# davidepi/glaze

Hardware: AMD Instinct MI355X
Metric: Msamples/s + achieved HBM GB/s, Sponza 1080p, 1/2/4/8xMI355X (higher is better)
Workload: dtype f32; 1 GPU; Sponza-class synthetic atrium (262267 tris, 26 materials, 27 textures) as a .glaze V1 file (2853389 bytes) through parse, 1920x1080, path tracer depth 8, 143 steps = 17.9 spp; materials=26, textures=27, scene=Sponza-class synthetic atrium, width=1920, height=1080, depth=8, triangles=262267

## Files before the change

### glaze_amd/abi.py

```python
import ctypes as C
import os

NAME_MAX = 256

OK, E_IO, E_INVALID_INPUT, E_INVALID_DATA, E_ARG, E_DEVICE, E_UNSUPPORTED = 0, -1, -2, -3, -4, -5, -6

CAMERA_PERSPECTIVE, CAMERA_ORTHOGRAPHIC = 0, 1
MAT_FLAT, MAT_LAMBERT, MAT_MIRROR, MAT_GLASS, MAT_METAL, MAT_FROSTED, MAT_UBER = range(7)
LIGHT_OMNI, LIGHT_SUN, LIGHT_AREA, LIGHT_SKY = range(4)
TEX_GRAY, TEX_RGBA_SRGB, TEX_RGBA_NORM = 1, 2, 3
DIRECT, PATH_TRACE = 0, 1


class Vertex(C.Structure):
    _fields_ = [("vv", C.c_float * 3), ("vn", C.c_float * 3), ("vt", C.c_float * 2)]


class Mesh(C.Structure):
    _fields_ = [("id", C.c_uint16), ("material", C.c_uint16), ("index_offset", C.c_uint32), ("index_count", C.c_uint32)]


class Transform(C.Structure):
    _fields_ = [("m", C.c_float * 16)]

# ... 227 lines not shown
    "glz_renderer_restart": (C.c_int, [_P]),
    "glz_renderer_step": (C.c_int, [_P, C.c_uint32]),
    "glz_renderer_read_rgba8": (C.c_int, [_P, _P]),
    "glz_renderer_set_seed": (C.c_int, [_P, C.c_uint64]),
    "glz_renderer_set_depth": (C.c_int, [_P, C.c_uint32]),
    "glz_renderer_read_hdr": (C.c_int, [_P, _P]),
    "glz_renderer_read_result": (C.c_int, [_P, _P]),
    "glz_renderer_launch_constants": (C.c_int, [_P, C.c_uint32, _P, _P]),
    "glz_renderer_push_constants": (C.c_int, [_P, _P]),
    "glz_renderer_set_partition": (C.c_int, [_P, C.c_uint32, C.c_uint32]),
    "glz_renderer_set_chains": (C.c_int, [_P, C.c_uint32]),
    "glz_renderer_export_device": (C.c_int, [_P, C.c_int, _P]),
    "glz_renderer_packed_pixels": (C.c_uint64, [_P, C.c_uint32, C.c_uint32]),
    "glz_renderer_export_packed": (C.c_int, [_P, C.c_int, _P]),
    "glz_renderer_scatter_packed": (C.c_int, [_P, C.c_uint32, C.c_uint32, _P, _P]),
    "glz_renderer_scatter_packed_all": (C.c_int, [_P, C.c_uint32, _P, C.c_uint64, _P]),
    "glz_renderer_tonemap_device": (C.c_int, [_P, _P, _P]),
    "glz_renderer_enable_counters": (C.c_int, [_P, C.c_int]),
    "glz_renderer_get_stats": (C.c_int, [_P, _P]),
    "glz_debug_trace_closest": (C.c_int, [_P, _P, _P, C.c_uint64, C.c_float, _P, _P, _P, _P, _P]),
    "glz_debug_trace_any": (C.c_int, [_P, _P, _P, _P, C.c_uint64, C.c_float, _P]),
    "glz_debug_read_derivatives": (C.c_int64, [_P, _P, C.c_int64]),
    "glz_debug_read_rt_materials": (C.c_int64, [_P, _P, C.c_int64]),
    "glz_debug_read_rt_lights": (C.c_int64, [_P, _P, C.c_int64]),
    "glz_debug_read_sky": (C.c_int64, [_P, _P, C.c_int64]),
    "glz_debug_read_bvh": (C.c_int64, [_P, _P, C.c_int64, _P, C.c_int64]),
    "glz_debug_read_bvh8": (C.c_int64, [_P, _P, C.c_int64]),
    "glz_host_launch_constants": (C.c_int, [C.c_uint64, C.c_uint32, _P, _P]),
    "glz_host_push_constants": (C.c_int, [_P, C.c_uint32, C.c_uint32, _P]),
    "glz_host_chain_owner": (C.c_int, [C.c_uint32, C.c_uint32, C.c_uint32, C.c_uint32, C.c_uint32, _P]),
    "glz_host_build_sah": (C.c_int, [C.c_uint32, _P, _P, _P, _P]),
    "glz_host_srgb8_thresholds": (C.c_int, [_P]),
    "glz_debug_tonemap": (C.c_int, [_P, _P, C.c_uint64, _P]),
    "glz_debug_sample_texture": (C.c_int, [_P, C.c_uint32, _P, _P, C.c_uint64, _P]),
    "glz_debug_detmath": (C.c_int, [_P, C.c_int, _P, _P, _P, C.c_uint64]),
    "glz_debug_color_to_spec": (C.c_int, [_P, C.c_int, _P, C.c_uint64, _P]),
    "glz_debug_scene_set_spectra": (C.c_int, [_P, C.c_uint32, _P, _P]),
    "glz_debug_bsdf_value": (C.c_int,[_P, C.c_uint32, _P, _P, _P, _P, _P, C.c_uint64, _P, _P]),
    "glz_debug_bsdf_sample": (C.c_int, [_P, C.c_uint32, _P, _P, _P, _P, C.c_uint64, _P, _P, _P]),
    "glz_debug_light_sample": (C.c_int, [_P, C.c_uint32, _P, _P, C.c_uint64, C.c_float, _P, _P, _P, _P]),
    "glz_debug_read_texture_level": (C.c_int64, [_P, C.c_uint32, C.c_uint32, _P, C.c_int64, _P, _P]),
    "glz_host_mip_level": (C.c_int64, [_P, C.c_uint32, _P, C.c_int64, _P, _P]),
    "glz_renderer_set_texture_lod": (C.c_int, [_P, C.c_int]),
    "glz_debug_rccl_selftest": (C.c_int, [_P, C.c_uint64, _P]),
    "glz_instance_set_as_levels": (C.c_int, [_P, C.c_int]),
    "glz_renderer_set_devices": (C.c_int, [_P, _P, C.c_int]),
    "glz_renderer_set_launch_mode": (C.c_int, [_P, C.c_int]),
    "glz_renderer_set_node_width": (C.c_int, [_P, C.c_int]),
    "glz_renderer_node_width": (C.c_int, [_P]),
    "glz_renderer_launch_mode": (C.c_int, [_P]),
    "glz_renderer_device_count": (C.c_int, [_P]),
    "glz_renderer_device_scene_info": (C.c_int, [_P, C.c_int, _P]),
    "glz_rccl_version": (C.c_int, []),
    "glz_host_tile_owner": (C.c_int, [C.c_uint32, C.c_uint32, C.c_uint32, _P]),
    "glz_renderer_read_aov": (C.c_int, [_P, C.c_int, _P]),
    "glz_renderer_set_denoise": (C.c_int, [_P, _P]),
    "glz_renderer_read_denoised": (C.c_int, [_P, _P, _P]),
    "glz_renderer_set_despeckle": (C.c_int, [_P, C.c_int, _P]),
    "glz_renderer_despeckle": (C.c_int, [_P, _P]),
    "glz_renderer_read_despeckled": (C.c_int, [_P, _P, _P]),
    "glz_renderer_read_motion": (C.c_int, [_P, _P, _P, C.c_uint32, _P]),
    "glz_renderer_reproject": (C.c_int, [_P, _P, _P, C.c_uint32, _P, _P, _P, _P, _P]),
    "glz_renderer_read_motion_from": (C.c_int, [_P, _P, _P]),
    "glz_renderer_reproject_from": (C.c_int, [_P, _P, _P, _P, _P, _P, _P]),
    "glz_debug_motion_timing_from": (C.c_int, [_P, _P, _P]),
    "glz_debug_skin_timing": (C.c_int, [_P, _P, C.c_uint32, _P]),
    "glz_host_project_constants": (C.c_int, [_P, C.c_uint32, C.c_uint32, _P]),
    "glz_host_project_points": (C.c_int, [_P, C.c_uint32, C.c_uint32, _P, C.c_uint64, _P]),
    "glz_host_reproject": (C.c_int, [C.c_uint32, C.c_uint32, _P, _P, _P, _P, _P, _P]),
    "glz_debug_project_points": (C.c_int, [_P, _P, C.c_uint32, C.c_uint32, _P, C.c_uint64, _P]),
    "glz_debug_motion_timing": (C.c_int, [_P, _P, _P, C.c_uint32, _P]),
    "glz_debug_reproject": (C.c_int, [_P, C.c_uint32, C.c_uint32, _P, _P, _P, _P, _P, _P, _P]),
    "glz_host_despeckle": (C.c_int, [C.c_uint32, C.c_uint32, _P, _P, _P, _P, _P, C.c_int, _P]),
    "glz_debug_despeckle": (C.c_int, [_P, C.c_uint32, C.c_uint32, _P, _P, _P, _P, _P, C.c_int, _P, _P]),
    "glz_host_denoise": (C.c_int, [C.c_uint32, C.c_uint32, _P, _P, _P, _P, _P]),
    "glz_debug_denoise": (C.c_int, [_P, C.c_uint32, C.c_uint32, _P, _P, _P, _P, _P]),
    "glz_debug_camera_rays": (C.c_int, [_P, C.c_float, C.c_float, _P, _P]),
    "glz_debug_post_timing": (C.c_int, [_P, _P]),
    "glz_renderer_set_guide_mode": (C.c_int, [_P, C.c_int, C.c_uint32]),
    "glz_renderer_guide_mode": (C.c_int, [_P, _P]),
    "glz_debug_guide_chain": (C.c_int, [_P, C.c_uint32, _P, _P, _P]),
    "glz_host_traversal_offsets_fit": (C.c_int, [C.c_uint64] * 6),
    "glz_host_sky_row_pairs": (C.c_int, [_P, _P, C.c_uint64, _P]),
    "glz_host_conductor_finite": (C.c_int, [_P, _P, _P]),
    "glz_host_metal_spectra": (C.c_int, [C.c_uint32, _P, _P]),
}

_LIB = None


def library_path():
    return os.environ.get("GLAZE_HIP_LIB") or os.path.join(os.path.dirname(os.path.abspath(__file__)), "csrc", "libglaze_hip.so")


class GlazeLibraryMissing(ImportError):
    pass


def lib():
    global _LIB
    if _LIB is None:
        path = library_path()
        if not os.path.exists(path):
            raise GlazeLibraryMissing(
                "%s not found: build it with `make -C glaze_amd/csrc` (there is no CPU fallback for the render path)" % path)
        handle = C.CDLL(path)
        for name, (res, args) in PROTOTYPES.items():
            fn = getattr(handle, name)
            fn.restype = res
            fn.argtypes = args
        _LIB = handle
    return _LIB


class GlazeError(IOError):
    def __init__(self, status, message):
        super().__init__("%s (status %d)" % (message, status))
        self.status = status


def last_error():
    l = lib()
    msg = l.glz_last_error()
    return GlazeError(l.glz_last_status(), msg.decode("utf8", "replace") if msg else "unknown error")


def check(status):
    if status < 0:
        raise last_error()
    return status
```

### glaze_amd/csrc/abi_debug.cpp

```cpp
#include <algorithm>
#include <cstring>
#include <string>
#include <vector>

#include "abi_internal.h"
#include "denoise.h"
#include "reproject.h"
#include "skin.h"
#include "morph.h"
#include "normals.h"
#include "mipchain.h"
#include "rccl_dl.h"
#include "tile_map.h"

using namespace glz;
using namespace glz::abi;

namespace {
struct DebugCall {
  hipStream_t st;
  template <class T>
  const T* in(const T* host, size_t n) {
    return host ? static_cast<const T*>(buffer(host, n * sizeof(T), nullptr)) : nullptr;
  }
// ... 603 lines not shown
  const int dev = inst->i->device;
  ncclResult_t r = nc->CommInitAll(&comm, 1, &dev);
  if (r != ncclSuccess) return fail(GLZ_E_DEVICE, (std::string("ncclCommInitAll: ") + nc->GetErrorString(r)).c_str());
  r = nc->Reduce(send.ptr, recv.ptr, n, ncclFloat, ncclSum, 0, comm, st);
  bool ok = r == ncclSuccess;
  std::string msg = ok ? "" : std::string("ncclReduce: ") + nc->GetErrorString(r);
  if (ok) {
    ok = hip_ok(hipMemcpyAsync(back.data(), recv.ptr, n * 4, hipMemcpyDeviceToHost, st), "read back", e) && hip_ok(hipStreamSynchronize(st), "ncclReduce", e);
    if (!ok) msg = e.msg;
  }
  (void)nc->CommDestroy(comm);
  if (!ok) return fail(GLZ_E_DEVICE, msg.c_str());
  if (memcmp(host.data(), back.data(), n * 4) != 0) return fail(GLZ_E_DEVICE, "ncclReduce on a one-rank communicator changed the data");
  return GLZ_OK;
  GLZ_GUARD_END(GLZ_E_IO)
}

int glz_host_launch_constants(uint64_t seed, uint32_t launch, uint32_t* seed_out, float offset[2]) {
  GLZ_GUARD_BEGIN
  if (!seed_out || !offset) return fail(GLZ_E_ARG, "output is null");
  if (!host::launch_constants(seed, launch, seed_out, offset)) return fail(GLZ_E_IO, "WorkScheduler::peek disagrees with next()");
  return GLZ_OK;
  GLZ_GUARD_END(GLZ_E_IO)
}
int glz_host_push_constants(const glz_camera* camera, uint32_t width, uint32_t height, float out32[32]) {
  if (!camera || !out32 || width == 0 || height == 0 || camera->type > GLZ_CAMERA_ORTHOGRAPHIC) return fail(GLZ_E_ARG, "bad argument");
  host::push_constants(*camera, width, height, out32, out32 + 16);
  return GLZ_OK;
}
int glz_host_tile_owner(uint32_t width, uint32_t height, uint32_t world, uint16_t* owner_out) {
  if (!owner_out || world == 0 || world > 65535) return fail(GLZ_E_ARG, "bad argument");
  const TileMap m = make_tile_map(width, height, 0, world);
  for (uint32_t y = 0; y < height; ++y)
    for (uint32_t x = 0; x < width; ++x) owner_out[(size_t)y * width + x] = (uint16_t)tile_owner(tile_of_pixel(m, x, y), world);
  return GLZ_OK;
}
int glz_host_chain_owner(uint32_t width, uint32_t height, uint32_t rank, uint32_t world, uint32_t chains, uint16_t* owner_out) {
  if (world == 0 || rank >= world || chains > 16 || !width || !height) return fail(GLZ_E_ARG, "bad argument");
  const uint32_t S = Renderer::chains_for(width, height, rank, world, chains);
  const TileMap m = make_tile_map(width, height, rank, world);
  if (owner_out)
    for (uint32_t y = 0; y < height; ++y)
      for (uint32_t x = 0; x < width; ++x) {
        const uint32_t t = tile_of_pixel(m, x, y);
        owner_out[(size_t)y * width + x] = tile_owner(t, world) == rank ? (uint16_t)tile_chain(t, world, S) : (uint16_t)0xFFFF;
      }
  return (int)S;
}

int64_t glz_host_mip_level(const glz_texture* t, uint32_t level, uint8_t* out, int64_t cap, uint32_t* width, uint32_t* height) {
  GLZ_GUARD_BEGIN
  if (!t || !t->pixels || !t->width || !t->height || t->format < 1 || t->format > 3) return fail(GLZ_E_ARG, "bad texture");
  std::vector<host::MipLevel> given(1);
  given[0].width = t->width;
  given[0].height = t->height;
  given[0].pixels.assign(t->pixels, t->pixels + (size_t)t->width * t->height * (t->format == GLZ_TEX_GRAY ? 1 : 4));
  const std::vector<host::MipLevel> chain = host::build_mip_chain(t->format, std::move(given));
  if (level >= chain.size()) {
    if (width) *width = 0;
    if (height) *height = 0;
    return 0;
  }
  const host::MipLevel& m = chain[level];
  if (width) *width = m.width;
  if (height) *height = m.height;
  if (out && cap > 0) memcpy(out, m.pixels.data(), (size_t)std::min<int64_t>(cap, (int64_t)m.pixels.size()));
  return (int64_t)m.pixels.size();
  GLZ_GUARD_END(GLZ_E_IO)
}
int glz_host_traversal_offsets_fit(uint64_t n_nodes, uint64_t n_nodes8, uint64_t n_leaves, uint64_t n_instances, uint64_t grid_lanes, uint64_t overflow_depth) {
  const char* what = traversal_offsets_exceeded(TraversalSizes{n_nodes, n_nodes8, n_leaves, n_instances, grid_lanes, overflow_depth});
  return what ? fail(GLZ_E_INVALID_DATA, what) : GLZ_OK;
}
int glz_host_srgb8_thresholds(float thresholds_out[256]) {
  if (!thresholds_out) return fail(GLZ_E_ARG, "output is null");
  host::srgb8_thresholds(thresholds_out);
  return GLZ_OK;
}
int glz_host_sky_row_pairs(const float* marginal_values, const float* conditional_integrals, uint64_t n, float* pairs_out) {
  if (n != 0 && (!marginal_values || !conditional_integrals || !pairs_out)) return fail(GLZ_E_ARG, "glz_host_sky_row_pairs: null array");
  sky_row_pairs(marginal_values, conditional_integrals, (size_t)n, pairs_out);
  return GLZ_OK;
}
int glz_host_conductor_finite(const float ior[16], const float ior2abs2[16], int* flag_out) {
  if (!ior || !ior2abs2 || !flag_out) return fail(GLZ_E_ARG, "glz_host_conductor_finite: null argument");
  *flag_out = conductor_finite(ior, ior2abs2) ? 1 : 0;
  return GLZ_OK;
}
int glz_host_metal_spectra(uint32_t metal, float ior_out[16], float ior2abs2_out[16]) {
  if (!ior_out || !ior2abs2_out || !metal_spectra(metal, ior_out, ior2abs2_out)) return fail(GLZ_E_ARG, "glz_host_metal_spectra: no such metal, or a null output");
  return GLZ_OK;
}

}

int glz_host_build_sah(uint32_t n, const float* box_lo, const float* box_hi, int32_t* children_out, int32_t* parent_out) {
  GLZ_GUARD_BEGIN
  if (n < 2 || !box_lo || !box_hi || !children_out || !parent_out) return fail(GLZ_E_ARG, "glz_host_build_sah: bad argument");
  static_assert(sizeof(float4) == 16 && sizeof(int2) == 8, "layout");
  build_sah_host(n, reinterpret_cast<const float4*>(box_lo), reinterpret_cast<const float4*>(box_hi), reinterpret_cast<int2*>(children_out), parent_out);
  return GLZ_OK;
  GLZ_GUARD_END(GLZ_E_IO)
}
```

### glaze_amd/csrc/device/hit_vertex.h

```cpp
#pragma once
#include "device/shading.h"

namespace glz {
using namespace dev;

struct ShadeRecord { float4 va0, va1, vb0, vb1, vc0, vc1, dn, du; };
struct HitVertex {
  ShadeRecord rec;
  uint32_t xf_bits;
  vec3 point;
  vec2 uv;
  vec3 ng, ns, dpdu;
  MatScalars mat;
};

__device__ __forceinline__ ShadeRecord load_shade_record(const DeviceScene& S, uint32_t leaf) {
  const float4* rec = S.shade_tris + 8u * (size_t)leaf;
  return ShadeRecord{rec[0], rec[1], rec[2], rec[3], rec[4], rec[5], rec[6], rec[7]};
}
__device__ __forceinline__ vec3 hit_point(float4 a, float4 b, float4 c, float4 hr) {
  const float b0 = 1.0f - hr.y - hr.z, b1 = hr.y, b2 = hr.z;
  return (mk3(a.x, a.y, a.z) * b0 + mk3(b.x, b.y, b.z) * b1) + mk3(c.x, c.y, c.z) * b2;
}
__device__ __forceinline__ vec3 hit_point(const ShadeRecord& r, float4 hr) { return hit_point(r.va0, r.vb0, r.vc0, hr); }
struct HitIds { uint32_t material_id, xf; };
template <bool FLAG, class InstOf>
__device__ __forceinline__ HitIds hit_ids(const DeviceScene& S, const ShadeRecord& r, InstOf inst_of) {
  HitIds ids{__float_as_uint(r.dn.w), __float_as_uint(r.du.w)};
  if (!FLAG) ids.xf &= 0x7FFFFFFFu;
  if (S.two_level) {
    const RTInstance in = S.instances[inst_of()];
    ids.material_id = in.material_id;
    ids.xf = in.transform_id;
    if (FLAG) ids.xf = in.transform_id | (S.xf_identity[in.transform_id] ? 0x80000000u : 0u);
  }
  return ids;
}
template <class InstOf>
__device__ __forceinline__ HitVertex load_hit_vertex(const DeviceScene& S, float4 hr, InstOf inst_of) {
  HitVertex v;
  v.rec = load_shade_record(S, __float_as_uint(hr.w));
  const ShadeRecord& r = v.rec;
  const HitIds ids = hit_ids<true>(S, r, inst_of);
  const float b0 = 1.0f - hr.y - hr.z, b1 = hr.y, b2 = hr.z;
  v.point = hit_point(r, hr);
  v.uv = vec2{(r.va1.z * b0 + r.vb1.z * b1) + r.vc1.z * b2, (r.va1.w * b0 + r.vb1.w * b1) + r.vc1.w * b2};
  v.ng = mk3(r.dn.x, r.dn.y, r.dn.z), v.dpdu = mk3(r.du.x, r.du.y, r.du.z);
  v.ns = (mk3(r.va0.w, r.va1.x, r.va1.y) * b0 + mk3(r.vb0.w, r.vb1.x, r.vb1.y) * b1) + mk3(r.vc0.w, r.vc1.x, r.vc1.y) * b2;
  v.mat = load_material(S, ids.material_id);
  v.xf_bits = ids.xf;
  return v;
}
template <bool POINTS>
__device__ __forceinline__ void finish_hit_vertex(const DeviceScene& S, HitVertex& v, const TexFootprint& fp) {
  if (v.mat.normal != 0) {
    const vec4 tx = texture2d_lod(S, v.mat.normal, v.uv.x, v.uv.y, fp);
    Frame old;
    old.s = normalize3(v.dpdu);
    old.n = v.ns;
    old.t = normalize3(cross3(old.n, old.s));
    v.ns = normalize3(to_world(mk3(tx.x * 2.0f - 1.0f, tx.y * 2.0f - 1.0f, tx.z * 2.0f - 1.0f), old));
    v.ns = v.ns * gl_sign(dot3(v.ng, v.ns));
  }
  if (!(v.xf_bits >> 31)) {
    const float4* xq = reinterpret_cast<const float4*>(&S.transforms[v.xf_bits & 0x7FFFFFFFu]);
    const float4 m0 = xq[0], m1 = xq[1], m2 = xq[2], m3 = xq[3], w0 = xq[4], w1 = xq[5], w2 = xq[6];
    const float w2o[12] = {w0.x, w0.y, w0.z, w0.w, w1.x, w1.y, w1.z, w1.w, w2.x, w2.y, w2.z, w2.w};
    if (POINTS) {
      const float o2w[16] = {m0.x, m0.y, m0.z, m0.w, m1.x, m1.y, m1.z, m1.w, m2.x, m2.y, m2.z, m2.w, m3.x, m3.y, m3.z, m3.w};
      v.point = xform_point(o2w, v.point);
      v.dpdu = xform_point(o2w, v.dpdu);
    }
    v.ng = xform_tdir(w2o, v.ng);
    v.ns = xform_tdir(w2o, v.ns);
  }
}
__device__ __forceinline__ SurfacePoint hit_surface_point(const DeviceScene& S, const HitVertex& v, vec3 direction, const TexFootprint& fp) {
  SurfacePoint P;
  P.woW = -direction;
  P.uv = v.uv;
  P.frame = make_frame(v.dpdu, v.ns);
  P.mat = v.mat;
  fetch_material_textures(S, P, fp);
  return P;
}
}
```

### glaze_amd/csrc/device/intersect.h

```cpp
#pragma once
#include <hip/hip_runtime.h>

#include "device/math.h"
#include "device/shading.h"
#include "device/types.h"

namespace glz {
using namespace dev;

typedef float f32x2 __attribute__((ext_vector_type(2)));
struct SlabSel { uint32_t x, y, z; };
constexpr uint32_t kKeyDistanceMask = 0xFFFFFC00u, kKeyChild = 0x100u, kKeyChildMask = 0x300u;
constexpr uint32_t kSlabSelLo = 0x0305040Cu, kSlabSelHi = 0x0307060Cu, kSlabSelFlip = kSlabSelLo ^ kSlabSelHi, kSlabMagic = 0x47000000u;
__device__ __forceinline__ uint32_t slab_sel(float ig) { return ig < 0.0f ? kSlabSelHi : kSlabSelLo; }
constexpr int kKeysNearFirst = 0, kKeysFarFirst = 1, kKeysPerLane = 2;
template <int ORDER>
constexpr uint32_t kKeyMiss = ORDER == kKeysFarFirst ? 0u : 0xFFFFFFFFu;
template <bool CHECK_LINK = true, int ORDER = kKeysNearFirst>
__device__ __forceinline__ uint32_t box_key(uint32_t wx, uint32_t wy, uint32_t wz, uint32_t link, uint32_t k, SlabSel sel, vec3 ig, vec3 cgn, vec3 cgf,
                                            float tmin, float tmax, uint32_t flip = 0u) {
  const float nx = __uint_as_float(__builtin_amdgcn_perm(wx, kSlabMagic, sel.x)), fx = __uint_as_float(__builtin_amdgcn_perm(wx, kSlabMagic, sel.x ^ kSlabSelFlip));
  const float ny = __uint_as_float(__builtin_amdgcn_perm(wy, kSlabMagic, sel.y)), fy = __uint_as_float(__builtin_amdgcn_perm(wy, kSlabMagic, sel.y ^ kSlabSelFlip));
  const float nz = __uint_as_float(__builtin_amdgcn_perm(wz, kSlabMagic, sel.z)), fz = __uint_as_float(__builtin_amdgcn_perm(wz, kSlabMagic, sel.z ^ kSlabSelFlip));
  const f32x2 tx = __builtin_elementwise_fma(f32x2{nx, fx}, f32x2{ig.x, ig.x}, f32x2{cgn.x, cgf.x});
// ... 23 lines not shown
  const float i = 1.0f / d;
  return fabsf(i) <= 1e30f ? i : copysignf(1e30f, i);
}
__device__ __forceinline__ float grid_inv_dir_fast(float d) {
  const float i = __builtin_amdgcn_rcpf(d);
  return fabsf(i) <= 1e30f ? i : copysignf(1e30f, i);
}
__device__ __forceinline__ bool ray_is_finite(vec3 o, vec3 d) {
  const float s = ((o.x + o.y) + o.z) + ((d.x + d.y) + d.z);
  return s - s == 0.0f;
}

struct RayShear {
  bool z_is_x, z_is_y;
  float sx, sy, sz;
};
__device__ __forceinline__ RayShear ray_shear(vec3 d) {
  const float ax = fabsf(d.x), ay = fabsf(d.y), az = fabsf(d.z);
  RayShear r;
  r.z_is_x = (ax >= ay) & (ax >= az);
  r.z_is_y = !r.z_is_x & (ay >= az);
  const float dz = r.z_is_x ? d.x : (r.z_is_y ? d.y : d.z), dx = r.z_is_x ? d.y : (r.z_is_y ? d.z : d.x), dy = r.z_is_x ? d.z : (r.z_is_y ? d.x : d.y);
  r.sz = 1.0f / dz;
  r.sx = dx * r.sz;
  r.sy = dy * r.sz;
  return r;
}
constexpr float kDetNoise = 1.9073486e-6f;

struct QuadHit {
  float t[2], u[2], v[2];
  bool ok[2];
};
__device__ __forceinline__ vec3 shear_point(const RayShear& r, float px, float py, float pz, vec3 o) {
  const vec3 a = mk3(px, py, pz) - o;
  const float az = r.z_is_x ? a.x : (r.z_is_y ? a.y : a.z), ax = r.z_is_x ? a.y : (r.z_is_y ? a.z : a.x), ay = r.z_is_x ? a.z : (r.z_is_y ? a.x : a.y);
  return mk3(fmaf(-r.sx, az, ax), fmaf(-r.sy, az, ay), r.sz * az);
}
__device__ __forceinline__ bool triangle_finish(float U, float V, float W, float Az, float Bz, float Cz, float products, float tmin, float& t, float& u, float& v) {
  const float lo = fminf(fminf(U, V), W), hi = fmaxf(fmaxf(U, V), W);
  const float det = (U + V) + W;
  const float inv = 1.0f / det;
  u = V * inv;
  v = W * inv;
  t = fmaf(W, Cz, fmaf(V, Bz, U * Az)) * inv;
  return !((lo < 0.0f) & (hi > 0.0f)) & (fabsf(det) > products * kDetNoise) & (t > tmin);
}
__device__ __forceinline__ QuadHit ray_quad(const RayShear& rs, float4 r0, float4 r1, float4 r2, float4 r3, bool pair, vec3 o, float tmin) {
  QuadHit h;
  const vec3 S0 = shear_point(rs, r0.x, r0.y, r0.z, o), S2 = shear_point(rs, r2.x, r2.y, r2.z, o);
  const float pv = S0.x * S2.y, qv = S0.y * S2.x;
  {
    const vec3 S1 = shear_point(rs, r1.x, r1.y, r1.z, o);
    const float pu = S2.x * S1.y, qu = S2.y * S1.x, pw = S1.x * S0.y, qw = S1.y * S0.x;
    float U = pu - qu, V = pv - qv, W = pw - qw;
    if (__builtin_expect(__any((U == 0.0f) | (V == 0.0f) | (W == 0.0f)), 0)) {
      if (U == 0.0f) U = fmaf(S2.x, S1.y, -pu) - fmaf(S2.y, S1.x, -qu);
      if (V == 0.0f) V = fmaf(S0.x, S2.y, -pv) - fmaf(S0.y, S2.x, -qv);
      if (W == 0.0f) W = fmaf(S1.x, S0.y, -pw) - fmaf(S1.y, S0.x, -qw);
    }
    h.ok[0] = triangle_finish(U, V, W, S0.z, S1.z, S2.z, (fabsf(pu) + fabsf(pv)) + fabsf(pw), tmin, h.t[0], h.u[0], h.v[0]);
  }
  __builtin_amdgcn_sched_barrier(0);
  {
    const vec3 S3 = shear_point(rs, r3.x, r3.y, r3.z, o);
    const float pu = S3.x * S2.y, qu = S3.y * S2.x, pv2 = S0.x * S3.y, qv2 = S0.y * S3.x;
    float U = pu - qu, V = pv2 - qv2, W = qv - pv;
    if (__builtin_expect(__any(pair & ((U == 0.0f) | (V == 0.0f) | (W == 0.0f))), 0)) {
      if (U == 0.0f) U = fmaf(S3.x, S2.y, -pu) - fmaf(S3.y, S2.x, -qu);
      if (V == 0.0f) V = fmaf(S0.x, S3.y, -pv2) - fmaf(S0.y, S3.x, -qv2);
      if (W == 0.0f) W = fmaf(S2.x, S0.y, -qv) - fmaf(S2.y, S0.x, -pv);
    }
    h.ok[1] = triangle_finish(U, V, W, S0.z, S2.z, S3.z, (fabsf(pu) + fabsf(pv2)) + fabsf(qv), tmin, h.t[1], h.u[1], h.v[1]) & pair;
  }
  return h;
}

__device__ __forceinline__ bool alpha_test(const DeviceScene& S, uint32_t leaf, float u, float v) {
  const float w = 1.0f - u - v;
  const float4* rec = S.alpha_recs + 3u * (size_t)leaf;
  const float4 r0 = rec[0], r1 = rec[1], r2 = rec[2];
  const float tu = (r0.x * w + r0.z * u) + r1.x * v, tv = (r0.y * w + r0.w * u) + r1.y * v;
  const TexDesc t{__float_as_uint(r1.z), __float_as_uint(r1.w), __float_as_uint(r2.x), __float_as_uint(r2.y)};
  return !(bilinear_level(S, t, S.tex_pool, tu, tv).x < 0.5f);
}

__device__ __forceinline__ bool alpha_test_instance(const DeviceScene& S, uint32_t slot, uint32_t instance, float u, float v) {
  const float4* rec = S.shade_tris + 8u * (size_t)slot;
  const float4 a = rec[1], b = rec[3], c = rec[5];
  const uint32_t material_id = S.instances[instance].material_id;
  const float w = 1.0f - u - v;
  const float tu = (a.z * w + b.z * u) + c.z * v, tv = (a.w * w + b.w * u) + c.w * v;
  return !(texture_r(S, S.materials[material_id].opacity, vec2{tu, tv}) < 0.5f);
}

struct HitRecord {
  float t, u, v;
  uint32_t leaf;
  uint32_t inst;
  uint32_t world_id;
};
}
```

### glaze_amd/csrc/device/shade_pixel.h

```cpp
#pragma once
#include <hip/hip_runtime.h>

#include "device/hit_vertex.h"
#include "device/math.h"
#include "device/path_state.h"
#include "device/shading.h"
#include "device/types.h"
#include "kernels.h"

namespace glz {
using namespace dev;

struct SharedQueue {
  const LaunchArgs& A;
  __device__ __forceinline__ uint32_t slot(bool push) { return queue_slot(A.st.queue_count + A.shade_set * kQueueSetWords, A.map.n_local_pixels, push); }
};
#ifdef GLZ_SECTION_TIMES
#define GLZ_SHADE_STAMP(k) out.stamp(k)
#else
#define GLZ_SHADE_STAMP(k) do { } while (0)
#endif
__device__ __forceinline__ uint32_t pixel_rng(const FrameData& F, PixelId px) {
  return pcg(__float_as_uint((float)F.seed) ^ pcg(__float_as_uint((float)px.x) ^ pcg(__float_as_uint((float)px.y))));
}
__device__ __forceinline__ uint32_t light_pick(const FrameData& F, uint32_t& rng) {
  return (uint32_t)gl_min(rand01(rng) * (float)F.lights_no, (float)(F.lights_no - 1u));
}
struct DirectState {
  const LaunchArgs& A;
  static constexpr bool kDeferSkyTexel = false;
  __device__ __forceinline__ void stamp(int) {}
  __device__ __forceinline__ void ray_o(uint32_t lid, float4 v) { A.st.ray_o[lid] = v; }
  __device__ __forceinline__ void ray_d(uint32_t lid, float4 v) { A.st.ray_d[lid] = v; }
  __device__ __forceinline__ void imp(int q, uint32_t lid, float4 v) { A.st.imp[q][lid] = v; }
  __device__ __forceinline__ float4 read_imp(int q, uint32_t lid) const { return A.st.imp[q][lid]; }
  __device__ __forceinline__ float4 reset_origin(uint32_t, float4 ro) const { return ro; }
  __device__ __forceinline__ uint32_t seed_rng(const FrameData& F, PixelId px) const { return pixel_rng(F, px); }
  __device__ __forceinline__ uint32_t pick_light(const FrameData& F, uint32_t& rng) const { return light_pick(F, rng); }
  __device__ __forceinline__ void accumulate(uint32_t lid, vec3 c, bool add, bool update, float mark) { accumulate_shaded(A, lid, c, add && isfinite(c.x + c.y + c.z), update, mark); }
};
struct StagedState {
#ifdef GLZ_SECTION_TIMES
  unsigned long long sec[8] = {0, 0, 0, 0, 0, 0, 0, 0}, sec_last = 0;
  __device__ __forceinline__ void stamp(int k) {
    const unsigned long long now = __builtin_amdgcn_s_memtime();
    sec[k] += now - sec_last;
    sec_last = now;
  }
#else
  __device__ __forceinline__ void stamp(int) {}
#endif
  static constexpr bool kDeferSkyTexel = true;
  float4 ro, rd, im[4];
  uint32_t mask = 0;
  __device__ __forceinline__ void ray_o(uint32_t, float4 v) { ro = v; mask |= 1u; }
  __device__ __forceinline__ void ray_d(uint32_t, float4 v) { rd = v; mask |= 2u; }
  __device__ __forceinline__ void imp(int q, uint32_t, float4 v) { im[q] = v; mask |= 4u; }
  const LaunchArgs* A = nullptr;
  LdsNodePtr lds_imp = nullptr;
  static constexpr uint32_t kShadeBlockPixels = 256;
  __device__ __forceinline__ float4 read_imp(int q, uint32_t) const {
    const u32x4 v = lds_imp[q * kShadeBlockPixels];
    return make_float4(__uint_as_float(v.x), __uint_as_float(v.y), __uint_as_float(v.z), __uint_as_float(v.w));
  }
  __device__ __forceinline__ float4 reset_origin(uint32_t lid, float4) const { return A->st.ray_o[lid]; }
  typedef uint32_t u32x2 __attribute__((ext_vector_type(2)));
  typedef const __attribute__((address_space(3))) u32x2* LdsPickPtr;
  LdsPickPtr lds_pick = nullptr;
  __device__ __forceinline__ uint32_t seed_rng(const FrameData&, PixelId) const { return (*lds_pick).x; }
  __device__ __forceinline__ uint32_t pick_light(const FrameData&, uint32_t&) const { return (*lds_pick).y; }
  __device__ __forceinline__ void accumulate(uint32_t lid, vec3 cc, bool add, bool update, float mark) { accumulate_shaded(*A, lid, cc, add && isfinite(cc.x + cc.y + cc.z), update, mark); }
};
template <bool LOD, class Queue, class State>
__device__ __forceinline__ int shade_pixel_body(const LaunchArgs& A, const DeviceScene& S, const FrameData& F, uint32_t lid, PixelId px, float4 ro, float4 rd, float4 hr, Queue& queue,
                                                State& out, float& end_w) {
  const bool fresh = F.direct_only || ro.w == 0.0f;
  float bounce = F.direct_only ? 0.0f : ro.w;
  const vec3 direction = mk3(rd.x, rd.y, rd.z);
  auto load_importance = [&]() {
    asm volatile("" ::: "memory");
    Spec imp;
    if (fresh) {
      imp = spec_set(1.0f);
    } else {
#pragma unroll
      for (int q = 0; q < 4; ++q) {
        const float4 v = out.read_imp(q, lid);
        imp.w[4 * q] = v.x; imp.w[4 * q + 1] = v.y; imp.w[4 * q + 2] = v.z; imp.w[4 * q + 3] = v.w;
      }
    }
    return imp;
  };
  const uint32_t leaf = __float_as_uint(hr.w);
  if (leaf == 0xFFFFFFFFu) {
    uint32_t flags = 0;
    vec3 c = mk3(0.0f, 0.0f, 0.0f);
    if ((bounce == 0.0f || rd.w == 1.0f) && S.sky.tex_id > 0) {
      const vec3 w = normalize3(xform_dir(S.sky.world2obj, direction));
      const float phi = glz_atan2f(w.y, w.x), theta = glz_acosf(w.z);
      const vec3 texel = texture_rgb(S, S.sky.tex_id, vec2{phi * kInv2Pi, theta * kInvPi});
      c = spec_to_rgb(spec_mul(load_importance(), from_illuminant_color(texel)));
      flags = kFlagUpdate;
    }
    if (flags != 0) out.accumulate(lid, c, true, true, F.update_mark);
    end_w = rd.w;
    return F.direct_only ? 0 : 1;
  }
  HitVertex hv = load_hit_vertex(S, hr, [&]() { return A.st.hit_inst[lid]; });
  const MatScalars mat = hv.mat;
  GLZ_SHADE_STAMP(0);
  TexFootprint fp{kNoLod, 0.0f, 0.0f, 1u};
  float cone_w = 0.0f;
  if constexpr (LOD) {
    const auto& [va0, va1, vb0, vb1, vc0, vc1, dn, du_rec] = hv.rec;
    float cone_in = F.cone_width0;
    asm volatile("" : "+v"(cone_in));
    if (!fresh) cone_in = A.st.cone[lid];
    cone_w = cone_in + F.cone_spread * hr.x;
    vec3 e1 = mk3(vb0.x, vb0.y, vb0.z) - mk3(va0.x, va0.y, va0.z), e2 = mk3(vc0.x, vc0.y, vc0.z) - mk3(va0.x, va0.y, va0.z);
    vec3 n = mk3(dn.x, dn.y, dn.z);
    if (!(hv.xf_bits >> 31)) {
      const TransformPair* xf = &S.transforms[hv.xf_bits & 0x7FFFFFFFu];
      e1 = xform_dir(xf->o2w, e1);
      e2 = xform_dir(xf->o2w, e2);
      n = xform_tdir(xf->w2o, n);
    }
    const vec3 cr = cross3(e1, e2);
    const float area2 = sqrtf(dot3(cr, cr));
    const float uva2 = fabsf((vb1.z - va1.z) * (vc1.w - va1.w) - (vc1.z - va1.z) * (vb1.w - va1.w));
    const float nn = dot3(n, n), nd = dot3(n, direction);
    const float cosv = fabsf(nd) / sqrtf(nn);
    const float x = ((uva2 / area2) * (cone_w * cone_w)) / (cosv * cosv);
    if (x >= 1.17549435e-38f && x <= 3.4e38f) {
      fp.lod_base = 0.5f * glz_log2f(x);
      if (F.lod_mode == 2u) {
        float ratio = 1.0f / cosv;
        ratio = ratio < 16.0f ? ratio : 16.0f;
        const float taps = -glz_floorf(-ratio);
        const vec3 m = direction - n * (nd / nn);
        const float mm = dot3(m, m);
        if (taps > 1.0f && mm > 0.0f) {
          const float g11 = dot3(e1, e1), g12 = dot3(e1, e2), g22 = dot3(e2, e2), r1 = dot3(m, e1), r2 = dot3(m, e2);
          const float det = g11 * g22 - g12 * g12;
          const float ca = (r1 * g22 - r2 * g12) / det, cb = (r2 * g11 - r1 * g12) / det;
          const float len = (cone_w / cosv) / sqrtf(mm);
          const float du = (ca * (vb1.z - va1.z) + cb * (vc1.z - va1.z)) * len;
          const float dv = (ca * (vb1.w - va1.w) + cb * (vc1.w - va1.w)) * len;
          if (fabsf(du) <= 3.4e38f && fabsf(dv) <= 3.4e38f) {
            fp.du = du;
            fp.dv = dv;
            fp.taps = (uint32_t)taps;
            fp.lod_base = fp.lod_base - glz_log2f(taps);
          }
        }
      }
    }
  }
  finish_hit_vertex<true>(S, hv, fp);
  const vec3 point = hv.point, ns = hv.ns;
  uint32_t rng = out.seed_rng(F, px);
  const SurfacePoint P = hit_surface_point(S, hv, direction, fp);
  GLZ_SHADE_STAMP(1);
  float spec_flag;
  float imp_lum = 0.0f;
  bool have_lum = false;
  if (mat.is_specular == 0) {
    const uint32_t li = out.pick_light(F, rng);
    vec3 xi;
    xi.x = rand01(rng); xi.y = rand01(rng); xi.z = rand01(rng);
    LightSample ls;
    ls.pdf = 0.0f;
    sample_light<State::kDeferSkyTexel>(S, li, point, xi, F.scene_radius, ls);
    GLZ_SHADE_STAMP(2);
    vec3 c = mk3(0.0f, 0.0f, 0.0f);
    uint32_t flags = kFlagUpdate;
    vec3 sh_dir = mk3(0.0f, 0.0f, 0.0f);
    float sh_tmax = 0.0f;
    if (ls.pdf > 0.0f) {
      const float xi_b = rand01(rng);
      Spec value = spec_set(0.0f);
      const float bpdf = bsdf_eval(S, P, ls.wiW, xi_b, value);
      if (bpdf > 0.0f) {
        const float w_vis = 1.0f * (fabsf(dot3(ls.wiW, ns)) / ls.pdf);
        const float nl = (float)F.lights_no;
        const Spec emission = light_emission<State::kDeferSkyTexel>(S, ls);
        const Spec importance = load_importance();
        imp_lum = spec_luminance(importance);
        have_lum = true;
        Spec rad;
        GLZ_BINS {
          const float rl = value.w[i] * emission.w[i];
          rad.w[i] = ((rl * w_vis) * nl) * importance.w[i];
        }
        c = spec_to_rgb(rad);
        if (!isfinite(c.x + c.y + c.z)) c = mk3(0.0f, 0.0f, 0.0f);
        flags |= kFlagShadow;
        sh_dir = ls.wiW;
        sh_tmax = ls.distance - 1e-3f;
      }
    }
    if (!(flags & kFlagShadow)) {
      const Spec importance = load_importance();
      imp_lum = spec_luminance(importance);
      have_lum = true;
    }
    const bool push = (flags & kFlagShadow) != 0;
    GLZ_SHADE_STAMP(3);
    const uint32_t slot = queue.slot(push);
    if (push) {
      A.st.sh_o[slot] = make_float4(point.x, point.y, point.z, sh_tmax);
      A.st.sh_d[slot] = make_float4(sh_dir.x, sh_dir.y, sh_dir.z, __uint_as_float(lid));
      A.st.contrib[slot] = make_float4(c.x, c.y, c.z, __uint_as_float(flags));
    } else {
      out.accumulate(lid, c, false, true, F.update_mark);
    }
    spec_flag = 0.0f;
  } else {
    spec_flag = 1.0f;
  }
  if (F.direct_only) return 0;
  GLZ_SHADE_STAMP(4);
  float rr_scale = 1.0f;
  if (bounce > (float)(F.pt_steps / 2u)) {
    const float kill = gl_max(0.05f, 1.0f - (have_lum ? imp_lum : spec_luminance(load_importance())));
    if (rand01(rng) < kill) {
      end_w = spec_flag;
      return 2;
    }
    rr_scale = 1.0f / (1.0f - kill);
  }
  vec3 xi;
  xi.x = rand01(rng); xi.y = rand01(rng); xi.z = rand01(rng);
  Spec value = spec_set(0.0f);
  vec3 wiW = mk3(0.0f, 0.0f, 0.0f);
  const float pdf = bsdf_sample(S, P, xi, value, wiW);
  if (pdf == 0.0f) {
    end_w = spec_flag;
    return 2;
  }
  float weight = fabsf(dot3(wiW, ns));
  weight /= pdf;
  const Spec importance = spec_scale(load_importance(), rr_scale);
#pragma unroll
  for (int q = 0; q < 4; ++q)
    out.imp(q, lid, make_float4(importance.w[4 * q] * (value.w[4 * q] * weight), importance.w[4 * q + 1] * (value.w[4 * q + 1] * weight),
                                importance.w[4 * q + 2] * (value.w[4 * q + 2] * weight), importance.w[4 * q + 3] * (value.w[4 * q + 3] * weight)));
  bounce = bounce < (float)F.pt_steps ? bounce + 1.0f : 0.0f;
  GLZ_SHADE_STAMP(5);
  if constexpr (LOD) A.st.cone[lid] = cone_w;
  if (F.pregen && bounce == 0.0f) {
    end_w = spec_flag;
    return 2;
  }
  out.ray_o(lid, make_float4(point.x, point.y, point.z, bounce));
  out.ray_d(lid, make_float4(wiW.x, wiW.y, wiW.z, spec_flag));
  return 0;
}
template <bool LOD, class Queue, class State>
__device__ __forceinline__ void shade_pixel(const LaunchArgs& A, const DeviceScene& S, const FrameData& F, uint32_t lid, PixelId px, float4 ro, float4 rd, float4 hr, Queue& queue,
                                            State& out) {
  float end_w = 0.0f;
  const int ended = shade_pixel_body<LOD>(A, S, F, lid, px, ro, rd, hr, queue, out, end_w);
  if (ended != 0) {
    if (F.pregen) {
      vec3 co, cd;
      camera_ray(A, F, px, F.next_pixel_offset[0], F.next_pixel_offset[1], co, cd);
      out.ray_o(lid, make_float4(co.x, co.y, co.z, __uint_as_float(kPregenBounceBits)));
      out.ray_d(lid, make_float4(cd.x, cd.y, cd.z, end_w));
    } else {
      const float4 o = out.reset_origin(lid, ro);
      out.ray_o(lid, make_float4(o.x, o.y, o.z, 0.0f));
      if (ended == 2) out.ray_d(lid, make_float4(rd.x, rd.y, rd.z, end_w));
    }
  }
}

constexpr uint32_t kShadeLdsTableBytes = 8192;
constexpr uint32_t kPathTableBytes = 16384;
static_assert(sizeof(MatCompact) % 16 == 0 && sizeof(MetalSpectra) % 16 == 0 && sizeof(RTLight) % 16 == 0 && sizeof(TexDesc) % 16 == 0, "the tables are copied in 16-byte pieces");
struct SceneTables {
  uint32_t qm, qs, ql, qt;
  __host__ __device__ explicit SceneTables(const DeviceScene& s)
      : qm(s.n_materials * (uint32_t)(sizeof(MatCompact) / 16)), qs(s.n_metal_spectra * (uint32_t)(sizeof(MetalSpectra) / 16)), ql(s.n_rt_lights * (uint32_t)(sizeof(RTLight) / 16)), qt(s.n_textures * (uint32_t)(sizeof(TexDesc) / 16)) {}
  __host__ __device__ uint32_t bytes() const { return (qm + qs + ql + qt) * 16u; }
  __device__ __forceinline__ void stage(const DeviceScene& s, uint4* dst, uint32_t block) const {
    const uint4* gm = reinterpret_cast<const uint4*>(s.mat_compact);
    const uint4* gs = reinterpret_cast<const uint4*>(s.metal_spectra);
    const uint4* gl = reinterpret_cast<const uint4*>(s.lights);
    const uint4* gt = reinterpret_cast<const uint4*>(s.tex_desc);
    const uint32_t es = qm + qs, el = es + ql;
    for (uint32_t i = threadIdx.x; i < el + qt; i += block) dst[i] = i < qm ? gm[i] : (i < es ? gs[i - qm] : (i < el ? gl[i - es] : gt[i - el]));
  }
  __device__ __forceinline__ void use(DeviceScene& S, const uint4* copy) const {
    S.mat_compact = reinterpret_cast<const MatCompact*>(copy);
    S.metal_spectra = reinterpret_cast<const MetalSpectra*>(copy + qm);
    S.lights = reinterpret_cast<const RTLight*>(copy + qm + qs);
    S.tex_desc = reinterpret_cast<const TexDesc*>(copy + qm + qs + ql);
  }
};

typedef const __attribute__((address_space(4))) char* KernargPtr;
__device__ __forceinline__ KernargPtr reread_kernarg() {
  KernargPtr p = (KernargPtr)__builtin_amdgcn_kernarg_segment_ptr();
  asm volatile("" : "+s"(p));
  return p;
}
}
```

### glaze_amd/csrc/device/shading.h

```cpp
#pragma once
#include "glaze_abi.h"
#include "glz_tables.h"
#include "math.h"
#include "types.h"

namespace glz {
namespace dev {

struct Spec {
  float w[16];
};
#define GLZ_BINS _Pragma("unroll") for (int i = 0; i < 16; ++i)

GLZ_D Spec spec_set(float f) { Spec s; GLZ_BINS s.w[i] = f; return s; }
GLZ_D Spec spec_scale(const Spec& a, float f) { Spec r; GLZ_BINS r.w[i] = a.w[i] * f; return r; }
GLZ_D Spec spec_mul(const Spec& a, const Spec& b) { Spec r; GLZ_BINS r.w[i] = a.w[i] * b.w[i]; return r; }
GLZ_D Spec spec_div(const Spec& a, float f) { Spec r; GLZ_BINS r.w[i] = a.w[i] / f; return r; }
GLZ_D Spec spec_load(const Spectrum16& g) { Spec r; GLZ_BINS r.w[i] = g.w[i]; return r; }

__device__ static const float kCieX[16] = GLZ_DEV_CIE_X;
__device__ static const float kCieY[16] = GLZ_DEV_CIE_Y;
__device__ static const float kCieZ[16] = GLZ_DEV_CIE_Z;
__device__ static const float kSurf[7][16] = {GLZ_DEV_SURF_WHITE, GLZ_DEV_SURF_CYAN, GLZ_DEV_SURF_MAGENTA, GLZ_DEV_SURF_YELLOW,
                                              GLZ_DEV_SURF_RED, GLZ_DEV_SURF_GREEN, GLZ_DEV_SURF_BLUE};
__device__ static const float kIllum[7][16] = {GLZ_DEV_ILLUM_WHITE, GLZ_DEV_ILLUM_CYAN, GLZ_DEV_ILLUM_MAGENTA, GLZ_DEV_ILLUM_YELLOW,
                                               GLZ_DEV_ILLUM_RED, GLZ_DEV_ILLUM_GREEN, GLZ_DEV_ILLUM_BLUE};
enum { kWhite = 0, kCyan, kMagenta, kYellow, kRed, kGreen, kBlue };

GLZ_D float spec_weighted(const Spec& s, const float* __restrict__ c) {
  float lane[4];
#pragma unroll
  for (int j = 0; j < 4; ++j) lane[j] = ((s.w[j] * c[j] + s.w[4 + j] * c[4 + j]) + s.w[8 + j] * c[8 + j]) + s.w[12 + j] * c[12 + j];
  return ((lane[0] + lane[1]) + lane[2]) + lane[3];
}
GLZ_D float spec_luminance(const Spec& s) { return spec_weighted(s, kCieY) * 0.17557178f; }
GLZ_D vec3 spec_to_rgb(const Spec& s) {
  float X = spec_weighted(s, kCieX) * 0.17557178f;
  float Y = spec_weighted(s, kCieY) * 0.17557178f;
  float Z = spec_weighted(s, kCieZ) * 0.17557178f;
  vec3 r;
  r.x = (3.240479f * X - 1.537150f * Y) - 0.498535f * Z;
  r.y = (-0.969256f * X + 1.875991f * Y) + 0.041556f * Z;
  r.z = (0.055648f * X - 0.204043f * Y) + 1.057311f * Z;
  return r;
}

GLZ_D Spec rgb_to_spec(vec3 c, const float (*__restrict__ basis)[16], float scale) {
  int a, b;
  float k0, k1, k2;
  if (c.x <= c.y && c.x <= c.z) {
    k0 = c.x;
    a = kCyan;
    if (c.y <= c.z) { k1 = c.y - c.x; b = kBlue; k2 = c.z - c.y; } else { k1 = c.z - c.x; b = kGreen; k2 = c.y - c.z; }
  } else if (c.y <= c.x && c.y <= c.z) {
    k0 = c.y;
    a = kMagenta;
    if (c.x <= c.z) { k1 = c.x - c.y; b = kBlue; k2 = c.z - c.x; } else { k1 = c.z - c.y; b = kRed; k2 = c.x - c.z; }
  } else {
    k0 = c.z;
    a = kYellow;
    if (c.x <= c.y) { k1 = c.x - c.z; b = kGreen; k2 = c.y - c.x; } else { k1 = c.y - c.z; b = kRed; k2 = c.x - c.y; }
  }
  Spec r;
  GLZ_BINS r.w[i] = ((basis[kWhite][i] * k0 + basis[a][i] * k1) + basis[b][i] * k2) * scale;
  return r;
}
GLZ_D Spec from_surface_color(vec3 c) { return rgb_to_spec(c, kSurf, 0.94f); }
GLZ_D Spec from_illuminant_color(vec3 c) { return rgb_to_spec(c, kIllum, 0.86445f); }

struct vec4 {
  float x, y, z, w;
};
constexpr uint32_t kTexInline = 0x80u;
GLZ_D vec4 decode_texel(const DeviceScene& S, uint32_t format, uint32_t bits) {
  if (format == GLZ_TEX_GRAY) return vec4{(float)(bits & 0xFFu) / 255.0f, 0.0f, 0.0f, 1.0f};
  const uint32_t r = bits & 0xFFu, g = (bits >> 8) & 0xFFu, b = (bits >> 16) & 0xFFu, a = bits >> 24;
  if (format == GLZ_TEX_RGBA_SRGB) return vec4{S.srgb_lut[r], S.srgb_lut[g], S.srgb_lut[b], (float)a / 255.0f};
  return vec4{(float)r / 255.0f, (float)g / 255.0f, (float)b / 255.0f, (float)a / 255.0f};
}
GLZ_D uint32_t texel_address(const TexDesc& t, uint32_t format, uint32_t ux, uint32_t uy) {
  const uint32_t tiles_x = t.format >> 8;
  if (format == GLZ_TEX_GRAY) return t.offset + ((uy >> 3) * tiles_x + (ux >> 4)) * 128u + (uy & 7u) * 16u + (ux & 15u);
  return t.offset + (((uy >> 2) * tiles_x + (ux >> 3)) * 32u + (uy & 3u) * 8u + (ux & 7u)) * 4u;
}
GLZ_D uint32_t load_texel(const uint8_t* __restrict__ pool, const TexDesc& t, uint32_t format, uint32_t ux, uint32_t uy) {
  const uint32_t addr = texel_address(t, format, ux, uy);
  return format == GLZ_TEX_GRAY ? (uint32_t)pool[addr] : *reinterpret_cast<const uint32_t*>(pool + addr);
}
GLZ_D int wrap_coord(int i, int n) {
  int r = i % n;
  return r < 0 ? r + n : r;
}
GLZ_D int wrap_coord_far(float i, int n) {
  const uint32_t bits = __float_as_uint(i), m = (bits & 0x7FFFFFu) | 0x800000u;
  const int e = (int)((bits >> 23) & 0xFFu) - 150;
  if (e > 104) return 0;
  uint32_t r = 0;
#pragma unroll 1
  for (int k = 23; k >= -e; --k) {
    r = 2u * r + (k >= 0 ? (m >> k) & 1u : 0u);
    r = r >= (uint32_t)n ? r - (uint32_t)n : r;
  }
  return (int)((bits >> 31) && r != 0u ? (uint32_t)n - r : r);
}
GLZ_D float lerp_ab(float a, float b, float t) { return a + (b - a) * t; }
GLZ_D vec4 bilinear_level(const DeviceScene& S, const TexDesc& t, const uint8_t* __restrict__ pool, float u, float v) {
  const uint32_t format = t.format & 0x7Fu;
  float fu = u * (float)t.width - 0.5f, fv = v * (float)t.height - 0.5f;
  float iu = glz_floorf(fu), iv = glz_floorf(fv);
  float ax = fu - iu, ay = fv - iv;
  uint32_t ta, tb, tc, tdx;
  if (t.format & kTexInline) {
    ta = tb = tc = tdx = t.offset;
  } else {
    if (S.tex_counter) {
      S.tex_counter[0] += 1ull;
      S.tex_counter[1] += format == GLZ_TEX_GRAY ? 4ull : 16ull;
    }
    const int x0 = fabsf(iu) < 8388608.0f ? wrap_coord((int)iu, (int)t.width) : wrap_coord_far(iu, (int)t.width);
    const int y0 = fabsf(iv) < 8388608.0f ? wrap_coord((int)iv, (int)t.height) : wrap_coord_far(iv, (int)t.height);
    const int x1 = x0 + 1 == (int)t.width ? 0 : x0 + 1, y1 = y0 + 1 == (int)t.height ? 0 : y0 + 1;
    if (format != GLZ_TEX_GRAY && x1 == x0 + 1 && (x0 & 7) != 7) {
      const uint2 r0 = *reinterpret_cast<const uint2*>(pool + texel_address(t, format, (uint32_t)x0, (uint32_t)y0));
      const uint2 r1 = *reinterpret_cast<const uint2*>(pool + texel_address(t, format, (uint32_t)x0, (uint32_t)y1));
      ta = r0.x; tb = r0.y; tc = r1.x; tdx = r1.y;
    } else {
      ta = load_texel(pool, t, format, (uint32_t)x0, (uint32_t)y0);
      tb = load_texel(pool, t, format, (uint32_t)x1, (uint32_t)y0);
      tc = load_texel(pool, t, format, (uint32_t)x0, (uint32_t)y1);
      tdx = load_texel(pool, t, format, (uint32_t)x1, (uint32_t)y1);
    }
  }
  const vec4 a = decode_texel(S, format, ta), b = decode_texel(S, format, tb), c = decode_texel(S, format, tc), d = decode_texel(S, format, tdx);
  vec4 r;
  r.x = lerp_ab(lerp_ab(a.x, b.x, ax), lerp_ab(c.x, d.x, ax), ay);
  r.y = lerp_ab(lerp_ab(a.y, b.y, ax), lerp_ab(c.y, d.y, ax), ay);
  r.z = lerp_ab(lerp_ab(a.z, b.z, ax), lerp_ab(c.z, d.z, ax), ay);
  r.w = lerp_ab(lerp_ab(a.w, b.w, ax), lerp_ab(c.w, d.w, ax), ay);
  return r;
}
GLZ_D vec4 texture2d(const DeviceScene& S, uint32_t id, float u, float v) {
  const uint4 td = reinterpret_cast<const uint4*>(S.tex_desc)[id];
  return bilinear_level(S, TexDesc{td.x, td.y, td.z, td.w}, S.tex_pool, u, v);
}
constexpr float kNoLod = -1e30f;
struct TexFootprint { float lod_base; float du, dv; uint32_t taps; };
GLZ_D vec4 texture2d_lod(const DeviceScene& S, uint32_t id, float u, float v, const TexFootprint& fp) {
  const uint4 td = reinterpret_cast<const uint4*>(S.tex_desc)[id];
  const TexDesc t0{td.x, td.y, td.z, td.w};
  uint32_t first = 0, l0 = 0, levels_used = 1, probes = 1;
  float frac = 0.0f;
  if (fp.lod_base > -1e29f && S.tex_mip_base != nullptr && !(t0.format & kTexInline)) {
    const uint32_t b = S.tex_mip_base[id];
    const uint32_t levels = b >> 24;
    first = b & 0xFFFFFFu;
    float lam = fp.lod_base + 0.5f * glz_log2f((float)t0.width * (float)t0.height);
    lam = lam > 0.0f ? lam : 0.0f;
    const float top = (float)(levels - 1u);
    lam = lam < top ? lam : top;
    const float fl = glz_floorf(lam);
    l0 = (uint32_t)fl;
    frac = lam - fl;
    levels_used = frac > 0.0f ? 2u : 1u;
    probes = fp.taps;
  }
  vec4 sum{0.0f, 0.0f, 0.0f, 0.0f}, cur{0.0f, 0.0f, 0.0f, 0.0f};
  const uint32_t fetches = probes * levels_used;
#pragma unroll 1
  for (uint32_t k = 0; k < fetches; ++k) {
    const uint32_t probe = levels_used == 2u ? k >> 1 : k, upper = levels_used == 2u ? k & 1u : 0u;
    const uint32_t level = l0 + upper;
    TexDesc t = t0;
    const uint8_t* pool = S.tex_pool;
    if (level != 0u) {
      const uint4 md = reinterpret_cast<const uint4*>(S.tex_mip_desc)[first + level - 1u];
      t = TexDesc{md.x, md.y, md.z, md.w};
      pool = S.tex_mip_pool;
    }
    float uu = u, vv = v;
    if (probes > 1u) {
      const float s = ((float)probe + 0.5f) / (float)probes - 0.5f;
      uu = u + s * fp.du;
      vv = v + s * fp.dv;
    }
    const vec4 r = bilinear_level(S, t, pool, uu, vv);
    if (upper == 0u) {
      cur = r;
    } else {
      cur.x = lerp_ab(cur.x, r.x, frac); cur.y = lerp_ab(cur.y, r.y, frac); cur.z = lerp_ab(cur.z, r.z, frac); cur.w = lerp_ab(cur.w, r.w, frac);
    }
    if (upper + 1u == levels_used) {
      if (probe == 0u) {
        sum = cur;
      } else {
        sum.x += cur.x; sum.y += cur.y; sum.z += cur.z; sum.w += cur.w;
      }
    }
  }
  if (probes > 1u) {
    const float n = (float)probes;
    sum.x = sum.x / n; sum.y = sum.y / n; sum.z = sum.z / n; sum.w = sum.w / n;
  }
  return sum;
}
GLZ_D vec3 texture_rgb(const DeviceScene& S, uint32_t id, vec2 uv) {
  vec4 t = texture2d(S, id, uv.x, uv.y);
  return mk3(t.x, t.y, t.z);
}
GLZ_D float texture_r(const DeviceScene& S, uint32_t id, vec2 uv) { return texture2d(S, id, uv.x, uv.y).x; }

struct Frame {
  vec3 s, t, n;
};
GLZ_D Frame make_frame(vec3 dpdu, vec3 n) {
  Frame f;
  f.s = normalize3(dpdu - n * dot3(n, dpdu));
  f.t = cross3(n, f.s);
  f.n = n;
  return f;
}
GLZ_D vec3 to_world(vec3 v, const Frame& f) {
  return normalize3(mk3((f.s.x * v.x + f.t.x * v.y) + f.n.x * v.z, (f.s.y * v.x + f.t.y * v.y) + f.n.y * v.z,
                        (f.s.z * v.x + f.t.z * v.y) + f.n.z * v.z));
}
GLZ_D vec3 to_local(vec3 w, const Frame& f) {
  return normalize3(mk3(dot3(w, f.s), dot3(w, f.t), dot3(w, f.n)));
}

GLZ_D Spec fresnel_conductor(float c, const Spectrum16& ior, const Spectrum16& ior2abs2) {
  const float c2 = c * c, twoc = c * 2.0f;
  Spec r;
  GLZ_BINS {
    float e = ior.w[i] * twoc;
    float ep = e + c2, epp = e + 1.0f;
    float a = ior2abs2.w[i];
    float perp = (a - ep) / (a + ep);
    float tmp = a * c2;
    float par = (tmp - epp) / (tmp + epp);
    r.w[i] = (perp + par) / 2.0f;
  }
  return r;
}
GLZ_D float fresnel_dielectric(float costi, float etai, float etat) {
  float sin2ti = gl_max(0.0f, 1.0f - costi * costi);
  float sin2tt = etai * etai / (etat * etat) * sin2ti;
  if (sin2tt >= 1.0f) return 1.0f;
  float costt = sqrtf(gl_max(0.0f, 1.0f - sin2tt));
  float tt = etat * costt, ti = etat * costi, ii = etai * costi, it = etai * costt;
  float rparl = (ti - it) / (ti + it);
  float rperp = (ii - tt) / (ii + tt);
  return (rparl * rparl + rperp * rperp) / 2.0f;
}

GLZ_D vec2 ggx_sample_p22(float cost, vec2 r) {
  if (cost > 0.999f) {
    float rr = sqrtf(r.x / (1.0f - r.x));
    float phi = kTwoPi * r.y;
    return vec2{rr * glz_cosf(phi), rr * glz_sinf(phi)};
  }
  float cos2t = cost * cost;
  float sin2t = gl_max(0.0f, 1.0f - cos2t);
  float tan2t = check_inf(sin2t / cos2t);
  float tant = sqrtf(tan2t);
  float a2 = 1.0f / tan2t;
  float G1 = 2.0f / (1.0f + sqrtf(1.0f + 1.0f / a2));
  float A = 2.0f * r.x / G1 - 1.0f;
  float B = tant;
  float invA2m1 = A * A - 1.0f == 0.0f ? 1e10f : 1.0f / (A * A - 1.0f);
  float sq = sqrtf(gl_max(0.0f, B * B * invA2m1 * invA2m1 - (A * A - B * B) * invA2m1));
  float sx1 = B * invA2m1 - sq;
  float sx2 = B * invA2m1 + sq;
  float sx = (A < 0.0f || sx2 > 1.0f / tant) ? sx1 : sx2;
  float stepval = gl_step(0.5f, r.y);
  float s = gl_mix(1.0f, -1.0f, stepval);
  float u = gl_mix(2.0f * (r.y - 0.5f), 2.0f * (0.5f - r.y), stepval);
  float z = (u * (u * (u * -0.3657289f + 0.7902350f) - 0.4249658f) + 0.0001529f) /
            (u * (u * (u * (u * 0.1695078f - 0.3972035f) - 0.2325005f) + 1.0f) - 0.5398259f);
  float sy = s * z * sqrtf(1.0f + sx * sx);
  return vec2{sx, sy};
}
GLZ_D float ggx_d(vec3 wh, vec2 a) {
  float cos2t = wh.z * wh.z;
  float cos4t = cos2t * cos2t;
  float sin2t = gl_max(0.0f, 1.0f - cos2t);
  float tan2t = sin2t / cos2t;
  float cos2p = wh.x * wh.x / sin2t;
  float sin2p = wh.y * wh.y / sin2t;
  float e1 = sin2t == 0.0f ? 1.0f : 1.0f + ((cos2p / (a.x * a.x) + sin2p / (a.y * a.y)) * tan2t);
  float d = 1.0f / (kPi * a.x * a.y * cos4t * e1 * e1);
  return isinf(tan2t) ? 0.0f : d;
}
GLZ_D float ggx_lambda(vec3 v, vec2 a) {
// ... 12 lines not shown
}
GLZ_D vec3 ggx_sample_wh(vec3 wo, vec2 r, vec2 a) {
  float flip = gl_sign(wo.z);
  vec3 wi = flip * wo;
  vec3 ws = normalize3(mk3(wi.x * a.x, wi.y * a.y, wi.z));
  float cost = ws.z;
  vec2 slope = ggx_sample_p22(cost, r);
  float sin2t = gl_max(0.0f, 1.0f - cost * cost);
  float cosp = sin2t == 0.0f ? 1.0f : sqrtf(ws.x * ws.x / sin2t);
  float sinp = sin2t == 0.0f ? 0.0f : sqrtf(ws.y * ws.y / sin2t);
  float sx = cosp * slope.x - sinp * slope.y;
  float sy = sinp * slope.x + cosp * slope.y;
  return flip * normalize3(mk3(-a.x * sx, -a.y * sy, 1.0f));
}
GLZ_D vec2 anisotropic_alpha(float a, float anis) { return vec2{a * (1.0f + anis), a * (1.0f - anis)}; }

struct MatScalars {
  float diffuse_mul[3];
  uint32_t diffuse, roughness, metalness, opacity, normal, bsdf_index;
  float roughness_mul, metalness_mul, anisotropy, ior_dielectric;
  uint32_t is_specular;
  uint32_t spectra;
};
GLZ_D MatScalars load_material(const DeviceScene& S, uint32_t id) {
  const float4* q = reinterpret_cast<const float4*>(&S.mat_compact[id]);
  const float4 a = q[0], b = q[2], c = q[3], d = q[4];
  MatScalars r;
  r.diffuse_mul[0] = a.x; r.diffuse_mul[1] = a.y; r.diffuse_mul[2] = a.z;
  r.diffuse = __float_as_uint(b.x); r.roughness = __float_as_uint(b.y); r.metalness = __float_as_uint(b.z); r.opacity = __float_as_uint(b.w);
  r.normal = __float_as_uint(c.x); r.bsdf_index = __float_as_uint(c.y); r.roughness_mul = c.z; r.metalness_mul = c.w;
  r.anisotropy = d.x; r.ior_dielectric = d.y; r.is_specular = __float_as_uint(d.z);
  r.spectra = __float_as_uint(a.w);
  return r;
}
GLZ_D const MetalSpectra& material_spectra(const DeviceScene& S, const MatScalars& m) { return S.metal_spectra[m.spectra & ~kSpectraConductorFinite]; }

struct SurfacePoint {
  vec3 woW;
  vec2 uv;
  Frame frame;
  MatScalars mat;
  vec3 tint;
  float rough_tex;
  float metal_tex;
};

GLZ_D void dielectric_etas(const MatScalars& m, float woz, float& etai, float& etat) {
  float outside = gl_step(0.0f, woz);
  etai = gl_mix(m.ior_dielectric, kDefaultIor, outside);
  etat = gl_mix(kDefaultIor, m.ior_dielectric, outside);
}

struct Lobe {
  float d, g, pdf, costi, cwo, cwi;
};
GLZ_D Lobe reflect_lobe(vec3 wo, vec3 wi, vec3 wh, vec2 a) {
  Lobe L;
  float owh = dot3(wo, wh), iwh = dot3(wi, wh);
  L.costi = dot3(wi, gl_sign(dot3(wh, mk3(0.0f, 0.0f, 1.0f))) * wh);
  L.cwo = fabsf(wo.z);
  L.cwi = fabsf(wi.z);
  L.d = gl_step(0.0f, wo.z) * ggx_d(wh, a);
  L.g = gl_step(0.0f, owh) * gl_step(0.0f, iwh) * ggx_g(wo, wi, a);
  L.pdf = ggx_pdf(L.d, a, wo, wh) / (4.0f * owh);
  return L;
}

GLZ_D float oren_nayar(float roughness, vec3 wo, vec3 wi) {
  float sigma = roughness * 0.5f;
  float s2 = sigma * sigma;
  float A = 1.0f - s2 / (2.0f * (s2 + 0.33f));
  float B = 0.45f * s2 / (s2 + 0.09f);
  float sinto = sqrtf(gl_max(0.0f, 1.0f - wo.z * wo.z));
  float sinti = sqrtf(gl_max(0.0f, 1.0f - wi.z * wi.z));
  float sinpi = wi.y / sinti, cospi = wi.x / sinti;
  float sinpo = wo.y / sinto, cospo = wo.x / sinto;
  float maxcos = gl_max(0.0f, cospi * cospo + sinpi * sinpo);
  float sel = gl_step(fabsf(wo.z), fabsf(wi.z));
  float sinalpha = gl_mix(sinto, sinti, sel);
  float tanbeta = gl_mix(sinti / fabsf(wi.z), sinto / fabsf(wo.z), sel);
  return kInvPi * (A + B * maxcos * sinalpha * tanbeta);
}

GLZ_D void fetch_material_textures(const DeviceScene& S, SurfacePoint& P, const TexFootprint& fp) {
  const uint32_t kind = P.mat.bsdf_index;
  P.tint = mk3(0.0f, 0.0f, 0.0f);
  P.rough_tex = P.metal_tex = 0.0f;
  if (kind == kBsdfLambert || kind == kBsdfUber) {
    const vec4 tx = texture2d_lod(S, P.mat.diffuse, P.uv.x, P.uv.y, fp);
    P.tint = mk3(tx.x, tx.y, tx.z) * mk3(P.mat.diffuse_mul[0], P.mat.diffuse_mul[1], P.mat.diffuse_mul[2]);
  }
  if (kind == kBsdfMetal || kind == kBsdfFrosted || kind == kBsdfUber) P.rough_tex = texture2d_lod(S, P.mat.roughness, P.uv.x, P.uv.y, fp).x;
  if (kind == kBsdfUber) P.metal_tex = texture2d_lod(S, P.mat.metalness, P.uv.x, P.uv.y, fp).x;
}
GLZ_D vec3 diffuse_tint(const DeviceScene&, const SurfacePoint& P) { return P.tint; }

GLZ_D void uber_specular_value(const DeviceScene& S, const MatScalars& m, float c, float fd, float metalness, float term, Spec& value) {
  if ((m.spectra & kSpectraConductorFinite) != 0u && metalness == 0.0f && fabsf(c) <= 2.0f) {
    const float v = gl_mix(fd, 0.0f, metalness) * term;
    GLZ_BINS value.w[i] = v;
    return;
  }
  const Spec fc = fresnel_conductor(c, material_spectra(S, m).ior, material_spectra(S, m).fresnel);
  GLZ_BINS value.w[i] = gl_mix(fd, fc.w[i], metalness) * term;
}

GLZ_D float bsdf_eval(const DeviceScene& S, const SurfacePoint& P, vec3 wiW, float xi, Spec& value) {
  const MatScalars& m = P.mat;
  const uint32_t kind = m.bsdf_index;
  if (kind == kBsdfMirror || kind == kBsdfGlass) return 0.0f;
  const vec3 wo = to_local(P.woW, P.frame), wi = to_local(wiW, P.frame);
  if (kind == kBsdfLambert) {
    float same = gl_step(0.0f, wo.z * wi.z);
    value = from_surface_color(diffuse_tint(S, P) * kInvPi);
    return same * fabsf(wi.z) * kInvPi;
  }
  if (kind == kBsdfMetal) {
    vec3 wh = normalize3(wo + wi);
    if (!(wo.z * wi.z > 0.0f)) return 0.0f;
    Spec F = fresnel_conductor(dot3(wi, wh), material_spectra(S, m).ior, material_spectra(S, m).fresnel);
    vec2 a = anisotropic_alpha(P.rough_tex * m.roughness_mul, m.anisotropy);
    float d = ggx_d(wh, a);
    float g = ggx_g(wo, wi, a);
    float term = d * g / (4.0f * fabsf(wo.z) * fabsf(wi.z));
    float pdf = ggx_pdf(d, a, wo, wh) / (4.0f * dot3(wo, wh));
    value = spec_scale(F, term);
    return check_nan(pdf);
  }
  if (kind == kBsdfFrosted) {
    vec2 a = anisotropic_alpha(P.rough_tex * m.roughness_mul, m.anisotropy);
    float etai, etat;
    dielectric_etas(m, wo.z, etai, etat);
    float eta = etai / etat;
    if (wo.z * wi.z > 0.0f) {
      vec3 wh = normalize3(wo + wi);
      Lobe L = reflect_lobe(wo, wi, wh, a);
      float f = fresnel_dielectric(L.costi, etai, etat);
      value = spec_set(L.d * L.g * f / (4.0f * L.cwo * L.cwi));
      return check_nan(L.pdf);
    }
    vec3 wh = normalize3(wo + eta * wi);
    wh = wh * gl_sign(wo.z);
    float owh = dot3(wo, wh), iwh = dot3(wi, wh);
    float f = fresnel_dielectric(owh, etai, etat);
    float cwo = fabsf(wo.z), cwi = fabsf(wi.z);
    float denom = owh + eta * iwh;
    float d = ggx_d(wh, a);
    float g = ggx_g(wo, wi, a);
    float pdf = ggx_pdf(d, a, wo, wh) * fabsf(eta * eta * iwh) / (denom * denom);
    value = spec_set(d * g * (1.0f - f) * fabsf(iwh) * fabsf(owh) / (denom * denom * cwo * cwi));
    return check_nan(pdf);
  }
  float roughness = P.rough_tex * m.roughness_mul;
  float same = gl_step(0.0f, wo.z * wi.z);
  if (xi < 0.5f) {
    vec2 a = anisotropic_alpha(roughness * m.roughness_mul, m.anisotropy);
    vec3 wh = normalize3(wo + wi);
    float metalness = P.metal_tex * m.metalness_mul;
    float etai, etat;
    dielectric_etas(m, wo.z, etai, etat);
    Lobe L = reflect_lobe(wo, wi, wh, a);
    float fd = fresnel_dielectric(L.costi, etai, etat);
    float term = L.d * L.g / (4.0f * L.cwo * L.cwi);
    uber_specular_value(S, m, L.costi, fd, metalness, term, value);
    return check_nan(same * 0.5f * L.pdf);
  }
  value = from_surface_color(diffuse_tint(S, P) * oren_nayar(roughness, wo, wi));
  return check_nan(same * 0.5f * fabsf(wi.z) * kInvPi);
}

GLZ_D vec3 cosine_hemisphere(float rx, float ry, float woz) {
  float t = kTwoPi * rx;
  float r = sqrtf(ry);
  vec3 wi;
  wi.x = r * glz_cosf(t);
  wi.y = r * glz_sinf(t);
  wi.z = sqrtf(gl_max(0.0f, 1.0f - wi.x * wi.x - wi.y * wi.y));
  wi.z *= gl_sign(woz);
  return wi;
}

GLZ_D float bsdf_sample(const DeviceScene& S, const SurfacePoint& P, vec3 xi, Spec& value, vec3& wiW) {
  const MatScalars& m = P.mat;
  const uint32_t kind = m.bsdf_index;
  const vec3 wo = to_local(P.woW, P.frame);
  if (kind == kBsdfLambert) {
    vec3 wi = cosine_hemisphere(xi.x, xi.y, wo.z);
    wiW = normalize3(to_world(wi, P.frame));
    value = from_surface_color(diffuse_tint(S, P) * kInvPi);
    return fabsf(wi.z) * kInvPi;
  }
  if (kind == kBsdfMirror) {
    Spec F = fresnel_conductor(wo.z, material_spectra(S, m).ior, material_spectra(S, m).fresnel);
    wiW = normalize3(to_world(mk3(-wo.x, -wo.y, wo.z), P.frame));
    value = spec_div(F, fabsf(wo.z));
    return 1.0f;
  }
  if (kind == kBsdfGlass) {
    float outside = gl_step(0.0f, wo.z);
    float etai = gl_mix(m.ior_dielectric, kDefaultIor, outside);
    float etat = gl_mix(kDefaultIor, m.ior_dielectric, outside);
    float costi = gl_mix(fabsf(wo.z), wo.z, outside);
    float F = fresnel_dielectric(costi, etai, etat);
    vec3 wi;
    float pdf, e;
    if (xi.z < F) {
      wi = mk3(-wo.x, -wo.y, wo.z);
      e = F / fabsf(wi.z);
      pdf = F;
    } else {
      wi = gl_refract(wo, mk3(0.0f, 0.0f, gl_sign(wo.z)), etai / etat);
      e = (1.0f - F) * (etai * etai) / (etat * etat * fabsf(wi.z));
      pdf = 1.0f - F;
    }
    value = spec_set(1.0f * e);
    wiW = to_world(wi, P.frame);
    return pdf;
  }
  if (kind == kBsdfMetal) {
    vec2 a = anisotropic_alpha(P.rough_tex * m.roughness_mul, m.anisotropy);
    vec3 wh = normalize3(ggx_sample_wh(wo, vec2{xi.x, xi.y}, a));
    vec3 wi = -normalize3(gl_reflect(wo, wh));
    if (!(wo.z * wi.z > 0.0f)) return 0.0f;
    float d = ggx_d(wh, a);
    float g = ggx_g(wo, wi, a);
    float gp = ggx_pdf(d, a, wo, wh);
    Spec F = fresnel_conductor(dot3(wi, wh), material_spectra(S, m).ior, material_spectra(S, m).fresnel);
    float term = d * g / (4.0f * fabsf(wo.z) * fabsf(wi.z));
    float pdf = gp / (4.0f * dot3(wo, wh));
    value = spec_scale(F, term);
    wiW = normalize3(to_world(wi, P.frame));
    return check_nan(pdf);
  }
  if (kind == kBsdfFrosted) {
    vec2 a = anisotropic_alpha(P.rough_tex * m.roughness_mul, m.anisotropy);
    vec3 wh = normalize3(ggx_sample_wh(wo, vec2{xi.x, xi.y}, a));
    float etai, etat;
    dielectric_etas(m, wo.z, etai, etat);
    float eta = etai / etat;
    vec3 wi;
    float pdf;
    if (xi.z < 0.5f) {
      wi = -normalize3(gl_reflect(wo, wh));
      Lobe L = reflect_lobe(wo, wi, wh, a);
      float f = fresnel_dielectric(L.costi, etai, etat);
      value = spec_set(L.d * L.g * f / (4.0f * L.cwo * L.cwi));
      pdf = check_nan(0.5f * L.pdf);
    } else {
      wi = normalize3(gl_refract(wo, wh, eta));
      float owh = dot3(wo, wh), iwh = dot3(wi, wh);
      float f = fresnel_dielectric(owh, etai, etat);
      float cwo = fabsf(wo.z), cwi = fabsf(wi.z);
      float denom = owh + eta * iwh;
      float d = ggx_d(wh, a);
      float g = ggx_g(wo, wi, a);
      float p = ggx_pdf(d, a, wo, wh) * fabsf(eta * eta * iwh) / (denom * denom);
      value = spec_set(d * g * (1.0f - f) * fabsf(iwh) * fabsf(owh) / (denom * denom * cwo * cwi));
      pdf = owh * iwh < 0.0f ? check_nan(0.5f * p) : 0.0f;
    }
    wiW = normalize3(to_world(wi, P.frame));
    return pdf;
  }
  float roughness = P.rough_tex * m.roughness_mul;
  vec3 wi;
  float pdf;
  if (xi.z < 0.5f) {
    vec2 a = anisotropic_alpha(roughness * m.roughness_mul, m.anisotropy);
    vec3 wh = normalize3(ggx_sample_wh(wo, vec2{xi.x, xi.y}, a));
    float metalness = P.metal_tex * m.metalness_mul;
    float etai, etat;
    dielectric_etas(m, wo.z, etai, etat);
    wi = -normalize3(gl_reflect(wo, wh));
    Lobe L = reflect_lobe(wo, wi, wh, a);
    float fd = fresnel_dielectric(L.costi, etai, etat);
    float term = L.d * L.g / (4.0f * L.cwo * L.cwi);
    uber_specular_value(S, m, L.costi, fd, metalness, term, value);
    pdf = check_nan(0.5f * L.pdf);
  } else {
    wi = cosine_hemisphere(xi.x, xi.y, wo.z);
    value = from_surface_color(diffuse_tint(S, P) * oren_nayar(roughness, wo, wi));
    pdf = 0.5f * fabsf(wi.z) * kInvPi;
  }
  wiW = normalize3(to_world(wi, P.frame));
  return pdf;
}

struct LightSample {
  vec3 wiW;
  float pdf;
  float distance;
  uint32_t kind;
  const RTLight* light;
  float k;
  vec3 rgb;
  vec2 uv;
};
constexpr uint32_t kLightSampleEmpty = 0xFFFFFFFFu;

GLZ_D float sq_dist(vec3 a, vec3 b) {
  return ((a.x - b.x) * (a.x - b.x) + (a.y - b.y) * (a.y - b.y)) + (a.z - b.z) * (a.z - b.z);
}

template <class Fetch>
GLZ_D float sample_cdf(float xi, int size, Fetch fetch, uint32_t& offset_out) {
  int first = 0, len = size;
  while (len > 0) {
    int half = len >> 1, middle = first + half;
    if (fetch(middle) <= xi) {
      first = middle + 1;
      len -= half + 1;
    } else {
      len = half;
    }
  }
  int off = first - 1;
  off = off < 0 ? 0 : (off > size - 2 ? size - 2 : off);
  float cur = fetch(off), next = fetch(off + 1);
  float du = xi - cur;
  if (next - cur > 0.0f) du /= next - cur;
  offset_out = (uint32_t)off;
  return ((float)off + du) / (float)size;
}

template <bool DEFER_SKY_TEXEL = true>
GLZ_D void sample_light(const DeviceScene& S, uint32_t light_index, vec3 p, vec3 xi, float scene_radius, LightSample& out) {
  const RTLight* L = &S.lights[light_index];
  const uint32_t kind = L->shader;
  if (S.tex_counter) {
    if (kind == kLightOmni || kind == kLightSun || kind == kLightArea) S.tex_counter[2] += 1ull; else S.tex_counter[3] += 1ull;
  }
  out.kind = kind;
  out.light = L;
  out.k = 1.0f;
  out.rgb = mk3(0.0f, 0.0f, 0.0f);
  out.uv = vec2{0.0f, 0.0f};
  if (kind == kLightOmni) {
    vec3 lp = mk3(L->pos[0], L->pos[1], L->pos[2]);
    out.wiW = normalize3(lp - p);
    float d2 = sq_dist(lp, p);
    out.distance = sqrtf(d2);
    out.pdf = 1.0f;
    out.k = d2 / L->intensity;
    return;
  }
  if (kind == kLightSun) {
    out.wiW = mk3(-L->dir[0], -L->dir[1], -L->dir[2]);
    out.pdf = 1.0f;
    out.distance = 2.0f * scene_radius + 1.0f;
    return;
  }
  if (kind == kLightArea) {
    const RTInstance in = S.instances[L->instance_id];
    const uint32_t ntri = in.index_count / 3u;
    uint32_t tri = (uint32_t)gl_min(xi.x * (float)in.index_count / 3.0f, (float)(ntri - 1u));
    tri += in.index_offset / 3u;
    const uint32_t i0 = S.indices[tri * 3u], i1 = S.indices[tri * 3u + 1u], i2 = S.indices[tri * 3u + 2u];
    const float4 a = S.vertices[2u * i0], b = S.vertices[2u * i1], c = S.vertices[2u * i2];
    const float area = 0.5f * 3.0f;
    float su = sqrtf(xi.y);
    float ru = 1.0f - su, rv = xi.z * su;
    vec3 rp = (ru * mk3(a.x, a.y, a.z) + rv * mk3(b.x, b.y, b.z)) + (1.0f - ru - rv) * mk3(c.x, c.y, c.z);
    rp = xform_point(S.transforms[in.transform_id].o2w, rp);
    out.wiW = normalize3(p - rp);
    float d2 = sq_dist(rp, p);
    out.distance = sqrtf(d2);
    const MatCompact* m = &S.mat_compact[in.material_id];
    out.rgb = mk3(m->diffuse_mul[0], m->diffuse_mul[1], m->diffuse_mul[2]);
    out.k = d2 / L->intensity;
    out.pdf = (1.0f / (float)ntri) * (1.0f / area);
    return;
  }
  uint32_t row;
  const float* cdf = S.sky_cdf;
  float v = sample_cdf(xi.y, (int)S.sky_header.marginal_cdf_count, [&](int i) { return cdf[i]; }, row);
  const float2 of_row = S.sky_rows[row];
  float v_pdf = of_row.x / S.sky_header.marginal_integral;
  const float cdf00 = S.sky_header.cond_cdf00;
  const int cond_size = (int)S.sky_header.conditional_cdf_count;
  int cond_off = (cond_size > 0 && cdf00 <= xi.x ? cond_size : 0) - 1;
  cond_off = cond_off < 0 ? 0 : (cond_off > cond_size - 2 ? cond_size - 2 : cond_off);
  float u = ((float)cond_off + (xi.x - cdf00)) / (float)cond_size;
  float u_pdf = S.sky_header.cond_value00 / of_row.y;
  float pdf = u_pdf * v_pdf;
  float theta = v * kPi;
  float sint = glz_sinf(theta);
  if (pdf > 0.0f && sint != 0.0f) {
    float phi = u * kTwoPi;
    float cost = glz_cosf(theta), cosp = glz_cosf(phi), sinp = glz_sinf(phi);
    out.pdf = pdf / (2.0f * kPi * kPi * sint);
    out.wiW = normalize3(xform_dir(S.sky.obj2world, mk3(sint * cosp, sint * sinp, cost)));
    out.distance = 2.0f * scene_radius + 1.0f;
    out.uv = vec2{u, v};
    if (!DEFER_SKY_TEXEL || S.tex_counter) out.rgb = texture_rgb(S, S.sky.tex_id, out.uv) * S.sky.intensity;
  } else {
    out.pdf = 0.0f;
    out.kind = kLightSampleEmpty;
  }
}

template <bool DEFER_SKY_TEXEL = true>
GLZ_D Spec light_emission(const DeviceScene& S, const LightSample& ls) {
  Spec e;
  if (ls.kind == kLightOmni) {
    GLZ_BINS e.w[i] = ls.light->color.w[i] / ls.k;
  } else if (ls.kind == kLightSun) {
    GLZ_BINS e.w[i] = ls.light->color.w[i] * ls.light->intensity;
  } else if (ls.kind == kLightArea) {
    e = spec_div(from_surface_color(ls.rgb), ls.k);
  } else {
    e = from_illuminant_color(!DEFER_SKY_TEXEL || S.tex_counter || ls.kind == kLightSampleEmpty ? ls.rgb : texture_rgb(S, S.sky.tex_id, ls.uv) * S.sky.intensity);
  }
  return e;
}

}
}
```

### glaze_amd/csrc/device/types.h

```cpp
#pragma once
#include <hip/hip_runtime.h>
#include <stdint.h>

namespace glz {

struct Spectrum16 {
  float w[16];
};

struct FrameData {
  uint32_t seed;
  uint32_t lights_no;
  float pixel_offset[2];
  float scene_radius;
  float update_mark;
  float scene_size[2];
  float scene_centre[4];
  uint32_t camera_persp;
  uint32_t pt_steps;
  uint32_t direct_only;
  uint32_t lod_mode;
  float cone_spread;
  float cone_width0;
  float next_pixel_offset[2];
// ... 87 lines not shown
  kBsdfLambert = 4, kBsdfMirror = 6, kBsdfGlass = 8, kBsdfMetal = 10, kBsdfFrosted = 12, kBsdfUber = 14
};

struct TexDesc {
  uint32_t offset;
  uint32_t width, height;
  uint32_t format;
};

struct TransformPair {
  float o2w[16];
  float w2o[16];
};

constexpr uint32_t kTriNonOpaque = 0x80000000u;
constexpr uint32_t kTriHasPartner = 0x40000000u;
constexpr uint32_t kTriPrimMask = 0x3FFFFFFFu;
constexpr float kPairAreaRatio = 0.85f;
struct alignas(16) BvhNode4 {
  uint32_t w[16];
};
struct alignas(128) BvhNode8 {
  uint32_t w[32];
};
constexpr int kBvhEmptyChild = 0x7FFFFFFF;
constexpr int kBvhTopNodes = 21;
constexpr int kBvhTopFlag = 0x40000000;
constexpr uint32_t kBvhGridMax = 32767u;
inline BvhNode4 childless_node4() {
  BvhNode4 nd{};
  for (int k = 0; k < 4; ++k) {
    nd.w[3 * k] = nd.w[3 * k + 1] = nd.w[3 * k + 2] = kBvhGridMax;
    nd.w[12 + k] = (uint32_t)kBvhEmptyChild;
  }
  return nd;
}
struct BvhGrid {
  float lo[3];
  float cell[3];
  float inv_cell[3];
};

struct alignas(16) TlasInstance {
  float w2o[12];
  BvhGrid grid;
  float slack;
  uint32_t node_base;
  float w2o_norm;
  float o2w[16];
  uint32_t tri_base;
  uint32_t world_base;
  uint32_t instance;
  uint32_t non_opaque;
  uint32_t quad_base;
  uint32_t _pad[3];
};
static_assert(sizeof(TlasInstance) == 192, "TlasInstance is 12 x 16 bytes");

struct alignas(16) BvhTri {
  float v0[3]; uint32_t world_id;
  float v1[3]; uint32_t instance;
  float v2[3]; uint32_t prim_flags;
};
static_assert(sizeof(BvhTri) == 48, "BvhTri is 48 bytes");

constexpr uint32_t kQuadSwapped = 0x20000000u;
constexpr uint32_t kQuadPrimMask = 0x1FFFFFFFu;
struct alignas(64) BvhQuad {
  float q0[3]; uint32_t world_id;
  float q1[3]; uint32_t instance;
  float q2[3]; uint32_t prim_flags;
  float q3[3]; uint32_t slot;
};
static_assert(sizeof(BvhQuad) == 64, "BvhQuad is 64 bytes");

struct SkyHeader {
  uint32_t marginal_cdf_count;
  uint32_t conditional_integral_offset;
  uint32_t conditional_cdf_count;
  float marginal_integral;
  float cond_cdf00;
  float cond_value00;
};

struct DeviceScene {
  const float4* vertices;
  const uint32_t* indices;
  const RTInstance* instances;
  const RTMaterial* materials;
  const MatCompact* mat_compact;
  const MetalSpectra* metal_spectra;
  const RTLight* lights;
  const TransformPair* transforms;
  const float4* derivatives;
  const TexDesc* tex_desc;
  const uint8_t* tex_pool;
  const TexDesc* tex_mip_desc;
  const uint32_t* tex_mip_base;
  const uint8_t* tex_mip_pool;
  const float* srgb_lut;
  const BvhNode4* bvh_nodes;
  const BvhNode4* bvh_top;
  const BvhNode8* bvh_nodes8;
  BvhGrid bvh_grid;
  const BvhTri* bvh_tris;
  const BvhQuad* bvh_quads;
  const float4* shade_tris;
  const float4* alpha_recs;
  const BvhNode4* tlas_nodes;
  const TlasInstance* tlas_instances;
  const uint32_t* xf_identity;
  uint32_t two_level;
  uint32_t has_non_opaque;
  uint32_t n_world_tris;
  uint32_t n_textures;
  uint32_t n_materials;
  uint32_t n_metal_spectra;
  uint32_t n_rt_lights;
  RTSky sky;
  SkyHeader sky_header;
  const float* sky_marginal;
  const float* sky_cdf;
  const float2* sky_rows;
  const float* sky_cond_values;
  const float* sky_cond_cdf;
  unsigned long long* tex_counter;
  uint32_t sky_w, sky_h;
};

}
```

### glaze_amd/csrc/kernels_debug.hip

```cpp
#include "device/shading.h"
#include "device/trace_wave.h"
#include "device/trace_wave_tl.h"
#include "launch_geometry.h"

namespace glz {
using namespace dev;

struct DebugSource {
  const float* __restrict__ o3;
  const float* __restrict__ d3;
  const float* __restrict__ tmax_arr;
  float tmin_all;
  __device__ __forceinline__ bool load(uint32_t i, vec3& o, vec3& d, float& tmin, float& tmax) {
    o = mk3(o3[3 * i], o3[3 * i + 1], o3[3 * i + 2]);
    d = mk3(d3[3 * i], d3[3 * i + 1], d3[3 * i + 2]);
    tmin = tmin_all;
    tmax = tmax_arr ? tmax_arr[i] : INFINITY;
    return true;
  }
};
struct DebugClosestSink {
  const DeviceScene& S;
  float* t; uint32_t* tri; uint32_t* inst; float* u; float* v;
  __device__ __forceinline__ void store(uint32_t i, const HitRecord& h) {
// ... 33 lines not shown
  __shared__ float s_top_ray[9 * kBlock];
  stage_top(S, s_top);
  TraceTally tally;
  DebugSource src{o, d, tmax, tmin};
  DebugAnySink sink{out};
  if (S.two_level) trace_wave_tl<true, false>(S, src, sink, &s_stack[threadIdx.x], wave_aux(s_aux, threadIdx.x >> 6), wave_links(s_aux, threadIdx.x >> 6), &s_top_ray[threadIdx.x], (LdsNodePtr)s_top, overflow, overflow_depth, n, wave_index(), wave_count(), tally);
  else trace_wave<true, false>(S, src, sink, &s_stack[threadIdx.x], wave_aux(s_aux, threadIdx.x >> 6), wave_links(s_aux, threadIdx.x >> 6), (LdsNodePtr)s_top, overflow, overflow_depth, n, wave_index(), wave_count(), tally);
}

__global__ void __launch_bounds__(kBlock) k_debug_sample_texture(DeviceScene S, uint32_t id, const float2* __restrict__ uv, const float4* __restrict__ fp,
                                                                 uint32_t n, float4* __restrict__ out) {
  const uint32_t i = blockIdx.x * kBlock + threadIdx.x;
  if (i >= n) return;
  S.tex_counter = nullptr;
  const float2 c = uv[i];
  vec4 r;
  if (fp) {
    const float4 f = fp[i];
    r = texture2d_lod(S, id, c.x, c.y, TexFootprint{f.x, f.y, f.z, (uint32_t)f.w});
  } else {
    r = texture2d(S, id, c.x, c.y);
  }
  out[i] = make_float4(r.x, r.y, r.z, r.w);
}
__global__ void __launch_bounds__(kBlock) k_debug_detmath(int fn, const float* __restrict__ x, const float* __restrict__ y, uint32_t n, float* __restrict__ out) {
  const uint32_t i = blockIdx.x * kBlock + threadIdx.x;
  if (i >= n) return;
  const float a = x[i];
  float r;
  switch (fn) {
    case 0: r = glz_sinf(a); break;
    case 1: r = glz_cosf(a); break;
    case 2: r = glz_acosf(a); break;
    case 3: r = glz_atan2f(y[i], a); break;
    case 4: r = glz_log2f(a); break;
    default: r = glz_floorf(a); break;
  }
  out[i] = r;
}
__global__ void __launch_bounds__(kBlock) k_debug_color_to_spec(int illuminant, const float* __restrict__ rgb3, uint32_t n, float* __restrict__ out16) {
  const uint32_t t = blockIdx.x * kBlock + threadIdx.x;
  if (t >= n) return;
  const vec3 c = mk3(rgb3[3 * t], rgb3[3 * t + 1], rgb3[3 * t + 2]);
  const Spec s = illuminant ? from_illuminant_color(c) : from_surface_color(c);
  GLZ_BINS out16[16 * t + i] = s.w[i];
}

__device__ __forceinline__ SurfacePoint debug_surface_point(const DeviceScene& S, uint32_t material, vec3 wo, const float* __restrict__ uv2,
                                                            const float* __restrict__ frame9) {
  SurfacePoint P;
  P.woW = wo;
  P.uv = vec2{uv2[0], uv2[1]};
  P.frame.s = frame9 ? mk3(frame9[0], frame9[1], frame9[2]) : mk3(1.0f, 0.0f, 0.0f);
  P.frame.t = frame9 ? mk3(frame9[3], frame9[4], frame9[5]) : mk3(0.0f, 1.0f, 0.0f);
  P.frame.n = frame9 ? mk3(frame9[6], frame9[7], frame9[8]) : mk3(0.0f, 0.0f, 1.0f);
  P.mat = load_material(S, material);
  fetch_material_textures(S, P, TexFootprint{kNoLod, 0.0f, 0.0f, 1u});
  return P;
}
__global__ void __launch_bounds__(kBlock) k_debug_bsdf_value(DeviceScene S, uint32_t material, const float* __restrict__ wo3, const float* __restrict__ wi3,
                                                             const float* __restrict__ uv2, const float* __restrict__ rand1, const float* __restrict__ frame9,
                                                             uint32_t n, float* __restrict__ value16, float* __restrict__ pdf) {
  const uint32_t t = blockIdx.x * kBlock + threadIdx.x;
  if (t >= n) return;
  S.tex_counter = nullptr;
  const SurfacePoint P = debug_surface_point(S, material, mk3(wo3[3 * t], wo3[3 * t + 1], wo3[3 * t + 2]), uv2, frame9);
  Spec value = spec_set(0.0f);
  pdf[t] = bsdf_eval(S, P, mk3(wi3[3 * t], wi3[3 * t + 1], wi3[3 * t + 2]), rand1[t], value);
  GLZ_BINS value16[16 * t + i] = value.w[i];
}
__global__ void __launch_bounds__(kBlock) k_debug_bsdf_sample(DeviceScene S, uint32_t material, const float* __restrict__ wo3, const float* __restrict__ uv2,
                                                              const float* __restrict__ rand3, const float* __restrict__ frame9, uint32_t n,
                                                              float* __restrict__ wi3, float* __restrict__ value16, float* __restrict__ pdf) {
  const uint32_t t = blockIdx.x * kBlock + threadIdx.x;
  if (t >= n) return;
  S.tex_counter = nullptr;
  const SurfacePoint P = debug_surface_point(S, material, mk3(wo3[3 * t], wo3[3 * t + 1], wo3[3 * t + 2]), uv2, frame9);
  Spec value = spec_set(0.0f);
  vec3 wi = mk3(0.0f, 0.0f, 0.0f);
  pdf[t] = bsdf_sample(S, P, mk3(rand3[3 * t], rand3[3 * t + 1], rand3[3 * t + 2]), value, wi);
  wi3[3 * t] = wi.x; wi3[3 * t + 1] = wi.y; wi3[3 * t + 2] = wi.z;
  GLZ_BINS value16[16 * t + i] = value.w[i];
}
__global__ void __launch_bounds__(kBlock) k_debug_light_sample(DeviceScene S, uint32_t light, const float* __restrict__ pos3, const float* __restrict__ rand3,
                                                               uint32_t n, float scene_radius, float* __restrict__ wi3, float* __restrict__ dist,
                                                               float* __restrict__ pdf, float* __restrict__ emission16) {
  const uint32_t t = blockIdx.x * kBlock + threadIdx.x;
  if (t >= n) return;
  S.tex_counter = nullptr;
  LightSample ls;
  ls.wiW = mk3(0.0f, 0.0f, 0.0f);
  ls.pdf = 0.0f;
  ls.distance = 0.0f;
  sample_light(S, light, mk3(pos3[3 * t], pos3[3 * t + 1], pos3[3 * t + 2]), mk3(rand3[3 * t], rand3[3 * t + 1], rand3[3 * t + 2]), scene_radius, ls);
  const Spec e = light_emission(S, ls);
  wi3[3 * t] = ls.wiW.x; wi3[3 * t + 1] = ls.wiW.y; wi3[3 * t + 2] = ls.wiW.z;
  dist[t] = ls.distance;
  pdf[t] = ls.pdf;
  GLZ_BINS emission16[16 * t + i] = e.w[i];
}

hipError_t launch_debug_closest(hipStream_t st, const DeviceScene& scene, const float* o, const float* d, uint32_t n, float tmin, float* t,
                                uint32_t* tri, uint32_t* inst, float* u, float* v, uint32_t* overflow, uint32_t overflow_depth) {
  if (n == 0) return hipSuccess;
  hipLaunchKernelGGL(k_debug_closest, persistent_grid(k_debug_closest, n), dim3(kBlock), 0, st, scene, o, d, n, tmin, t, tri, inst, u, v, overflow, overflow_depth);
  return hipGetLastError();
}
hipError_t launch_debug_any(hipStream_t st, const DeviceScene& scene, const float* o, const float* d, const float* tmax, uint32_t n, float tmin,
                            uint8_t* hit, uint32_t* overflow, uint32_t overflow_depth) {
  if (n == 0) return hipSuccess;
  hipLaunchKernelGGL(k_debug_any, persistent_grid(k_debug_any, n), dim3(kBlock), 0, st, scene, o, d, tmax, n, tmin, hit, overflow, overflow_depth);
  return hipGetLastError();
}

hipError_t launch_debug_sample_texture(hipStream_t st, const DeviceScene& scene, uint32_t id, const float* uv2, const float* fp4, uint32_t n, float* rgba) {
  return launch_per_item(st, k_debug_sample_texture, n, scene, id, reinterpret_cast<const float2*>(uv2), reinterpret_cast<const float4*>(fp4), n,
                         reinterpret_cast<float4*>(rgba));
}
hipError_t launch_debug_detmath(hipStream_t st, int fn, const float* x, const float* y, uint32_t n, float* out) {
  return launch_per_item(st, k_debug_detmath, n, fn, x, y, n, out);
}
hipError_t launch_debug_color_to_spec(hipStream_t st, int illuminant, const float* rgb3, uint32_t n, float* out16) {
  return launch_per_item(st, k_debug_color_to_spec, n, illuminant, rgb3, n, out16);
}
hipError_t launch_debug_bsdf_value(hipStream_t st, const DeviceScene& scene, uint32_t material, const float* wo3, const float* wi3, const float* uv2,
                                   const float* rand1, const float* frame9, uint32_t n, float* value16, float* pdf) {
  return launch_per_item(st, k_debug_bsdf_value, n, scene, material, wo3, wi3, uv2, rand1, frame9, n, value16, pdf);
}
hipError_t launch_debug_bsdf_sample(hipStream_t st, const DeviceScene& scene, uint32_t material, const float* wo3, const float* uv2, const float* rand3,
                                    const float* frame9, uint32_t n, float* wi3, float* value16, float* pdf) {
  return launch_per_item(st, k_debug_bsdf_sample, n, scene, material, wo3, uv2, rand3, frame9, n, wi3, value16, pdf);
}
hipError_t launch_debug_light_sample(hipStream_t st, const DeviceScene& scene, uint32_t light, const float* pos3, const float* rand3, uint32_t n,
                                     float scene_radius, float* wi3, float* dist, float* pdf, float* emission16) {
  return launch_per_item(st, k_debug_light_sample, n, scene, light, pos3, rand3, n, scene_radius, wi3, dist, pdf, emission16);
}
}
```

### glaze_amd/csrc/kernels_post.hip

```cpp
#include "denoise.h"
#include "device/hit_vertex.h"
#include "device/path_state.h"
#include "device/shading.h"
#include "device/trace_wave.h"
#include "device/trace_wave_tl.h"
#include "launch_geometry.h"
#include "reproject.h"

namespace glz {
using namespace dev;

struct CentreSource {
  const LaunchArgs& A;
  __device__ __forceinline__ bool load(uint32_t i, vec3& origin, vec3& direction, float& tmin, float& tmax) {
    if (i >= A.map.n_local_pixels) return false;
    const PixelId px = pixel_of(A.map, i);
    if (!px.active) return false;
    camera_ray(A, A.frame, px, 0.5f, 0.5f, origin, direction);
    tmin = 0.0001f;
    tmax = INFINITY;
    return true;
  }
};
template <bool BY_PIXEL>
struct HitSink {
  const LaunchArgs& A;
  float4* hit;
  uint32_t* inst;
  __device__ __forceinline__ void store(uint32_t i, const HitRecord& h) {
    const PixelId px = pixel_of(A.map, i);
    const size_t p = BY_PIXEL ? (size_t)px.y * A.map.width + px.x : i;
    const bool is_hit = h.leaf != 0xFFFFFFFFu;
    hit[p] = pack_hit(h);
    inst[p] = is_hit ? (A.scene.two_level ? h.inst : A.scene.bvh_tris[h.leaf].instance) : 0xFFFFFFFFu;
  }
};
__global__ void __launch_bounds__(kBlock) k_first_hit(const LaunchArgs A, float4* hit, uint32_t* inst) {
  __shared__ int s_stack[kLdsStack * kBlock];
  __shared__ alignas(1024) int s_aux[kAuxPerBlock];
  __shared__ uint4 s_top[kBvhTopNodes * 4];
  __shared__ float s_top_ray[9 * kBlock];
  stage_top(A.scene, s_top);
  TraceTally tally;
  CentreSource src{A};
  HitSink<true> sink{A, hit, inst};
  const uint32_t n = A.map.n_local_pixels;
  if (A.scene.two_level) trace_wave_tl<false, false>(A.scene, src, sink, &s_stack[threadIdx.x], wave_aux(s_aux, threadIdx.x >> 6), wave_links(s_aux, threadIdx.x >> 6), &s_top_ray[threadIdx.x], (LdsNodePtr)s_top, A.st.overflow, A.st.overflow_depth, n, wave_index(), wave_count(), tally);
  else trace_wave<false, false>(A.scene, src, sink, &s_stack[threadIdx.x], wave_aux(s_aux, threadIdx.x >> 6), wave_links(s_aux, threadIdx.x >> 6), (LdsNodePtr)s_top, A.st.overflow, A.st.overflow_depth, n, wave_index(), wave_count(), tally);
}

struct GuideVertex {
  vec3 n, albedo;
  bool go_on;
  vec3 point, wiW;
};
template <bool CHAIN>
__device__ __forceinline__ GuideVertex guide_vertex(const DeviceScene& S, float4 hr, uint32_t hit_inst, vec3 direction) {
  const TexFootprint fp{kNoLod, 0.0f, 0.0f, 1u};
  HitVertex hv = load_hit_vertex(S, hr, [&]() { return hit_inst; });
  finish_hit_vertex<CHAIN>(S, hv, fp);
  const MatScalars& mat = hv.mat;
  GuideVertex v;
  v.n = normalize3(hv.ns);
  if (dot3(v.n, direction) > 0.0f) v.n = -v.n;
  if (!(post::finite1(v.n.x) && post::finite1(v.n.y) && post::finite1(v.n.z))) v.n = mk3(0.0f, 0.0f, 0.0f);
  v.albedo = mk3(1.0f, 1.0f, 1.0f);
  if (mat.bsdf_index == kBsdfLambert || mat.bsdf_index == kBsdfUber) {
    const vec4 tx = texture2d_lod(S, mat.diffuse, hv.uv.x, hv.uv.y, fp);
    v.albedo = mk3(tx.x, tx.y, tx.z) * mk3(mat.diffuse_mul[0], mat.diffuse_mul[1], mat.diffuse_mul[2]);
  }
  v.go_on = false;
  v.point = hv.point;
  v.wiW = mk3(0.0f, 0.0f, 0.0f);
  if (CHAIN && mat.is_specular != 0) {
    const SurfacePoint P = hit_surface_point(S, hv, direction, fp);
    Spec value = spec_set(0.0f);
    const float pdf = bsdf_sample(S, P, mk3(0.0f, 0.0f, 0x1.fffffep-1f), value, v.wiW);
    v.go_on = pdf != 0.0f && post::finite1(v.wiW.x) && post::finite1(v.wiW.y) && post::finite1(v.wiW.z);
  }
  return v;
}

__device__ __forceinline__ void store_miss_planes(float4* __restrict__ aov0, float4* __restrict__ aov1, uint32_t p) {
  aov0[p] = make_float4(0.0f, 0.0f, 0.0f, INFINITY);
  aov1[p] = make_float4(1.0f, 1.0f, 1.0f, __uint_as_float(0xFFFFFFFFu));
}
__device__ __forceinline__ vec3 centre_ray_direction(const LaunchArgs& A, uint32_t p) {
  PixelId px;
  px.x = p % A.map.width;
  px.y = p / A.map.width;
  px.active = true;
  vec3 origin, direction;
  camera_ray(A, A.frame, px, 0.5f, 0.5f, origin, direction);
  return direction;
}
__global__ void __launch_bounds__(kBlock) k_first_hit_attributes(const LaunchArgs A, const float4* __restrict__ hit, const uint32_t* __restrict__ inst,
                                                                 float4* __restrict__ aov0, float4* __restrict__ aov1) {
  const uint32_t p = blockIdx.x * kBlock + threadIdx.x;
  if (p >= A.map.width * A.map.height) return;
  const float4 hr = hit[p];
  if (__float_as_uint(hr.w) == 0xFFFFFFFFu) {
    store_miss_planes(aov0, aov1, p);
    return;
  }
  DeviceScene S = A.scene;
  S.tex_counter = nullptr;
  const uint32_t hit_inst = inst[p];
  const GuideVertex v = guide_vertex<false>(S, hr, hit_inst, centre_ray_direction(A, p));
  aov0[p] = make_float4(v.n.x, v.n.y, v.n.z, hr.x);
  aov1[p] = make_float4(v.albedo.x, v.albedo.y, v.albedo.z, __uint_as_float(hit_inst));
}

__device__ __forceinline__ uint32_t list_slot(uint32_t* count, bool push) {
  const unsigned long long m = __ballot(push);
  uint32_t slot = 0;
  if (push) {
    const int lane = threadIdx.x & 63;
    const int leader = __ffsll((long long)m) - 1;
    uint32_t base = 0;
    if (lane == leader) base = atomicAdd(count, (uint32_t)__popcll(m));
    base = __shfl(base, leader);
    slot = base + (uint32_t)__popcll(m & ((1ull << lane) - 1ull));
  }
  return slot;
}
template <bool FIRST>
__device__ __forceinline__ void guide_continue_ray(const LaunchArgs& A, const DeviceScene& S, uint32_t i, bool live, bool may_push, const float4* __restrict__ hit,
                                                   const uint32_t* __restrict__ inst, const float4* __restrict__ in_o, const float4* __restrict__ in_d,
                                                   float4* __restrict__ out_o, float4* __restrict__ out_d, uint32_t* out_count, float4* __restrict__ aov0,
                                                   float4* __restrict__ aov1) {
  bool push = false;
  uint32_t p = 0;
  float depth = 0.0f;
  vec3 point = mk3(0.0f, 0.0f, 0.0f), wiW = mk3(0.0f, 0.0f, 0.0f);
  if (live) {
    const float4 hr = hit[i];
    vec3 direction;
    float before = 0.0f;
    if (FIRST) {
      p = i;
      direction = centre_ray_direction(A, p);
    } else {
      const float4 ro = in_o[i], rd = in_d[i];
      p = __float_as_uint(rd.w);
      direction = mk3(rd.x, rd.y, rd.z);
      before = ro.w;
    }
    if (__float_as_uint(hr.w) == 0xFFFFFFFFu) {
      if (FIRST) store_miss_planes(aov0, aov1, p);
    } else {
      const uint32_t hit_inst = inst[i];
      const GuideVertex v = guide_vertex<true>(S, hr, hit_inst, direction);
      depth = FIRST ? hr.x : before + hr.x;
      aov0[p] = make_float4(v.n.x, v.n.y, v.n.z, depth);
      aov1[p] = make_float4(v.albedo.x, v.albedo.y, v.albedo.z, __uint_as_float(hit_inst));
      push = may_push && v.go_on;
      point = v.point;
      wiW = v.wiW;
// ... 289 lines not shown
```

### glaze_amd/csrc/kernels_render.hip

```cpp
#include "device/path_state.h"
#include "device/shade_pixel.h"
#include "device/trace_wave.h"
#include "device/trace_wave_tl.h"
#include "launch_geometry.h"
#include "symbol_readers.h"

namespace glz {
using namespace dev;

constexpr uint32_t kSkyLdsFloats = 1088;

constexpr uint32_t kShadeBlock = 256, kShadeWavesPerBlock = kShadeBlock / 64;
#ifdef GLZ_SECTION_TIMES
static __device__ unsigned long long g_shade_sections[16 * 4096];
#endif
__host__ __device__ inline bool shade_tables_fit(const DeviceScene& s) { return SceneTables(s).bytes() <= kShadeLdsTableBytes; }
__host__ __device__ inline bool shade_sky_fits(const DeviceScene& s) { return s.sky_header.marginal_cdf_count > 1u && s.sky_header.marginal_cdf_count <= kSkyLdsFloats; }
template <class T>
__device__ __forceinline__ const T* in_memory(const T* p) { return (const T*)(const __attribute__((address_space(1))) T*)p; }
template <bool COUNT, bool LOD, bool TABLES, bool SKY>
__global__ void __launch_bounds__(kShadeBlock, GLZ_SHADE_WAVES) k_shade(const LaunchArgs A) {
#ifdef GLZ_SECTION_TIMES
  unsigned long long ks[4] = {0, 0, 0, 0}, ks_last = __builtin_amdgcn_s_memtime();
#define GLZ_KS(k) do { const unsigned long long now_ = __builtin_amdgcn_s_memtime(); ks[k] += now_ - ks_last; ks_last = now_; } while (0)
#else
#define GLZ_KS(k) do { } while (0)
#endif
  __shared__ alignas(16) float s_lut[256];
  __shared__ uint4 s_pool[kShadeBlock * 4 + kSkyLdsFloats / 4 + kShadeLdsTableBytes / 16];
  uint4* s_imp = s_pool;
  float* s_sky = reinterpret_cast<float*>(s_pool + kShadeBlock * 4);
  uint4* s_tables = s_pool + kShadeBlock * 4 + kSkyLdsFloats / 4;
  static_assert(6u * kShadeBlock <= kShadeBlock * 4 + kSkyLdsFloats / 4 + kShadeLdsTableBytes / 16, "the staging area of the path state fits the pool");
  __shared__ uint32_t s_bin[kShadeWavesPerBlock * 64];
  __shared__ uint16_t s_perm[kShadeBlock];
  __shared__ float4 s_hit[kShadeBlock];
  __shared__ float s_bounce[kShadeBlock];
  __shared__ uint2 s_pick[kShadeBlock];
  static_assert(kShadeBlock == 256, "pixel_of_block");
  const uint32_t n_sky = A.scene.sky_header.marginal_cdf_count;
  if (threadIdx.x < 64u) reinterpret_cast<float4*>(s_lut)[threadIdx.x] = reinterpret_cast<const float4*>(A.scene.srgb_lut)[threadIdx.x];
  if (SKY)
    for (uint32_t i = threadIdx.x; i < (n_sky + 3u) / 4u; i += kShadeBlock) s_pool[kShadeBlock * 4 + i] = reinterpret_cast<const uint4*>(A.scene.sky_marginal)[i];
  s_bin[threadIdx.x] = 0;
  const SceneTables tables(A.scene);
  if (TABLES) tables.stage(A.scene, s_tables, kShadeBlock);
  __syncthreads();
  GLZ_KS(0);
  DeviceScene S = A.scene;
  unsigned long long tex_tally[4] = {0ull, 0ull, 0ull, 0ull};
  S.tex_counter = COUNT ? tex_tally : nullptr;
  S.srgb_lut = s_lut;
  S.sky_cdf = SKY ? s_sky : in_memory(S.sky_cdf);
  S.sky_rows = in_memory(S.sky_rows);
  if (TABLES) {
    tables.use(S, s_tables);
  } else {
    S.mat_compact = in_memory(S.mat_compact);
    S.metal_spectra = in_memory(S.metal_spectra);
    S.lights = in_memory(S.lights);
    S.tex_desc = in_memory(S.tex_desc);
  }
  const FrameData& F = A.frame;
  uint32_t key = 63u;
  {
    const uint32_t lid0 = blockIdx.x * kShadeBlock + threadIdx.x;
    const PixelId px0 = pixel_of_block(A.map, blockIdx.x, threadIdx.x);
    if (px0.active) {
      const float4 h0 = A.st.hit[lid0];
#pragma unroll
      for (int q = 0; q < 4; ++q) s_imp[q * kShadeBlock + threadIdx.x] = *reinterpret_cast<const uint4*>(&A.st.imp[q][lid0]);
      s_hit[threadIdx.x] = h0;
      s_bounce[threadIdx.x] = A.st.ray_o[lid0].w;
      const uint32_t leaf0 = __float_as_uint(h0.w);
      key = 0u;
      if (leaf0 != 0xFFFFFFFFu) {
        const MatCompact* m0 = &S.mat_compact[S.two_level ? S.instances[A.st.hit_inst[lid0]].material_id : __float_as_uint(S.shade_tris[8u * (size_t)leaf0 + 6u].w)];
        uint32_t light = 4u, rng0 = pixel_rng(F, px0), li0 = 0u;
        if (m0->is_specular == 0) {
          li0 = light_pick(F, rng0);
          if (F.lights_no != 0u) light = S.lights[li0].shader;
        }
        s_pick[threadIdx.x] = make_uint2(rng0, li0);
        key = 1u + (m0->bsdf_index < 6u ? m0->bsdf_index : 5u) * 5u + (light < 4u ? light : 4u);
      }
    }
  }
  GLZ_KS(1);
  uint32_t rank = 0;
  {
    const uint32_t wv = threadIdx.x >> 6, ln = threadIdx.x & 63u;
    unsigned long long todo = __ballot(true);
    while (todo != 0ull) {
      const uint32_t k = (uint32_t)__shfl((int)key, __ffsll((long long)todo) - 1);
      const unsigned long long m = __ballot(key == k);
      if (key == k) {
        rank = (uint32_t)__popcll(m & ((1ull << ln) - 1ull));
        if (rank == 0u) s_bin[wv * 64u + k] = (uint32_t)__popcll(m);
      }
      todo &= ~m;
    }
  }
  __syncthreads();
  if (threadIdx.x < 64) {
    uint32_t c[kShadeWavesPerBlock];
    uint32_t cnt = 0;
#pragma unroll
    for (uint32_t w = 0; w < kShadeWavesPerBlock; ++w) {
      c[w] = s_bin[w * 64u + threadIdx.x];
      cnt += c[w];
    }
    uint32_t incl = cnt;
#pragma unroll
    for (int off = 1; off < 64; off <<= 1) {
      const uint32_t up = __shfl_up(incl, off);
      if ((int)threadIdx.x >= off) incl += up;
    }
    uint32_t at = incl - cnt;
#pragma unroll
    for (uint32_t w = 0; w < kShadeWavesPerBlock; ++w) {
      s_bin[w * 64u + threadIdx.x] = at;
      at += c[w];
    }
  }
  __syncthreads();
  {
    const uint32_t pos = s_bin[(threadIdx.x >> 6) * 64u + key] + rank;
    s_perm[pos] = (uint16_t)threadIdx.x;
  }
  __syncthreads();
  GLZ_KS(2);
  const uint32_t lid = blockIdx.x * kShadeBlock + s_perm[threadIdx.x];
  const PixelId px = pixel_of_block(A.map, blockIdx.x, s_perm[threadIdx.x]);
  StagedState staged;
  if (px.active) {
    const float4 ro = make_float4(0.0f, 0.0f, 0.0f, s_bounce[s_perm[threadIdx.x]]), rd = A.st.ray_d[lid], hr = s_hit[s_perm[threadIdx.x]];
    const LaunchArgs& A2 = *(const LaunchArgs*)reread_kernarg();
    SharedQueue queue{A2};
    staged.A = &A2;
    staged.lds_imp = (LdsNodePtr)(reinterpret_cast<u32x4*>(s_imp) + s_perm[threadIdx.x]);
    staged.lds_pick = (StagedState::LdsPickPtr)(reinterpret_cast<StagedState::u32x2*>(s_pick) + s_perm[threadIdx.x]);
#ifdef GLZ_SECTION_TIMES
    staged.sec_last = __builtin_amdgcn_s_memtime();
#endif
    shade_pixel<LOD>(A2, S, A2.frame, lid, px, ro, rd, hr, queue, staged);
  }
#ifdef GLZ_SECTION_TIMES
  ks_last = __builtin_amdgcn_s_memtime();
#endif
  {
    __syncthreads();
    float4* stage = reinterpret_cast<float4*>(s_pool);
    const uint32_t p = s_perm[threadIdx.x];
    s_bin[p] = staged.mask;
    if (staged.mask & 1u) stage[p] = staged.ro;
    if (staged.mask & 2u) stage[kShadeBlock + p] = staged.rd;
    if (staged.mask & 4u) {
#pragma unroll
      for (int q = 0; q < 4; ++q) stage[(2u + q) * kShadeBlock + p] = staged.im[q];
    }
    __syncthreads();
    const LaunchArgs& A3 = *(const LaunchArgs*)reread_kernarg();
    const uint32_t m = s_bin[threadIdx.x], at = blockIdx.x * kShadeBlock + threadIdx.x;
    if (m & 1u) A3.st.ray_o[at] = stage[threadIdx.x];
    if (m & 2u) A3.st.ray_d[at] = stage[kShadeBlock + threadIdx.x];
    if (m & 4u) {
#pragma unroll
      for (int q = 0; q < 4; ++q) A3.st.imp[q][at] = stage[(2u + q) * kShadeBlock + threadIdx.x];
    }
  }
  if (COUNT) flush_tex_tallies(A.counters->shade_tex, tex_tally);
#ifdef GLZ_SECTION_TIMES
  if (!COUNT) {
    GLZ_KS(3);
    unsigned long long v[10] = {ks[0], ks[1], ks[2], staged.sec[0], staged.sec[1], staged.sec[2], staged.sec[3], staged.sec[4], staged.sec[5], ks[3]};
    const uint32_t w = blockIdx.x * kShadeWavesPerBlock + (threadIdx.x >> 6);
#pragma unroll
    for (int k = 0; k < 10; ++k) {
      unsigned int lo = (unsigned int)v[k], hi = (unsigned int)(v[k] >> 32);
      for (int off = 32; off > 0; off >>= 1) {
        const unsigned int lo2 = __shfl_xor(lo, off), hi2 = __shfl_xor(hi, off);
        const unsigned long long a = ((unsigned long long)hi << 32) | lo, b = ((unsigned long long)hi2 << 32) | lo2;
        if (b > a) { lo = lo2; hi = hi2; }
      }
      if ((threadIdx.x & 63u) == 0u && w < 4096u) g_shade_sections[16u * w + k] += ((unsigned long long)hi << 32) | lo;
    }
    if ((threadIdx.x & 63u) == 0u && w < 4096u) g_shade_sections[16u * w + 15u] += 1ull;
  }
#endif
}

template <bool COUNT, int ALPHA>
__global__ void __launch_bounds__(kBlock, GLZ_TRACE_WAVES) k_trace(const LaunchArgs A) {
  __shared__ int s_stack[kLdsStack * kBlock];
  __shared__ alignas(1024) int s_aux[kAuxPerBlock];
  __shared__ uint4 s_top[kBvhTopNodes * 4];
  static_assert(kBvhTopNodes * 4 <= kBlock, "stage_top copies one 16-byte piece per thread");
  GLZ_WAVE_STAMP(0);
  stage_top(A.scene, s_top);
  int* aux = wave_aux(s_aux, threadIdx.x >> 6);
  int* links = wave_links(s_aux, threadIdx.x >> 6);
  clear_next_queue_set(A);
  unsigned long long tex_tally[4] = {0ull, 0ull, 0ull, 0ull};
  DeviceScene counted_scene;
  if (COUNT) {
    counted_scene = A.scene;
    counted_scene.tex_counter = tex_tally;
  }
  const DeviceScene& TS = COUNT ? counted_scene : A.scene;
  uint32_t split_closest = A.do_closest, split_shadow = A.do_shadow, split_wave_c = wave_index(), split_waves_c = wave_count(), split_wave_s = 0, split_waves_s = 0;
  bool split = false;
  if (!COUNT && A.do_closest && A.do_shadow) {
    const uint32_t* counts0 = A.st.queue_count + (A.shade_set ^ 1u) * kQueueSetWords;
    uint32_t n_sh = 0;
#pragma unroll
    for (uint32_t k = 0; k < kQueueShards; ++k) n_sh += counts0[k * kCounterStride];
    const uint32_t gc = (A.map.n_local_pixels + 63u) / 64u, gs = (n_sh + 63u) / 64u, nw = wave_count();
    if (gc + gs > nw && gs > 0u) {
      split = true;
      uint32_t ws = (uint32_t)(((unsigned long long)nw * gs * GLZ_TRACE_SPLIT_NUM) / ((unsigned long long)gc * GLZ_TRACE_SPLIT_DEN + (unsigned long long)gs * GLZ_TRACE_SPLIT_NUM));
      ws = ws < 1u ? 1u : (ws > nw - 1u ? nw - 1u : ws);
      const uint32_t w = wave_index();
      const uint32_t s_before = (uint32_t)(((unsigned long long)w * ws) / nw), s_after = (uint32_t)(((unsigned long long)(w + 1u) * ws) / nw);
// ... 231 lines not shown
```

### glaze_amd/csrc/shading_tables.cpp

```cpp
#include "shading_tables.h"

#include <cmath>
#include <cstring>
#include <utility>

#include "host_math.h"
#include "instance_boxes.h"

namespace glz {

static uint32_t sbt_callable_index(uint8_t mtype) {
  switch (mtype) {
    case GLZ_MAT_FLAT:
    case GLZ_MAT_LAMBERT: return kBsdfLambert;
    case GLZ_MAT_MIRROR: return kBsdfMirror;
    case GLZ_MAT_GLASS: return kBsdfGlass;
    case GLZ_MAT_METAL: return kBsdfMetal;
    case GLZ_MAT_FROSTED: return kBsdfFrosted;
    default: return kBsdfUber;
  }
}

bool metal_spectra(uint32_t metal, float* ior_out, float* ior2abs2_out) {
  if (metal >= GLZ_METAL_COUNT) return false;
// ... 8 lines not shown
bool conductor_finite(const float* ior, const float* ior2abs2) {
  const double big = 1152921504606846976.0;
  for (int i = 0; i < 16; ++i) {
    const double n = ior[i], a = ior2abs2[i];
    if (!std::isfinite(n) || !std::isfinite(a) || std::fabs(n) > big || std::fabs(a) > big) return false;
    const double need = (std::fabs(a) + 4.0 * std::fabs(n) + 5.0) / 1024.0;
    double lo = std::fmin(a + 4.0 * n + 4.0, a - 4.0 * n + 4.0);
    if (std::fabs(n) <= 2.0) lo = std::fmin(lo, a - n * n);
    if (!(lo >= need)) return false;
    lo = std::fmin(4.0 * a + 4.0 * n + 1.0, 4.0 * a - 4.0 * n + 1.0);
    if (a != 0.0 && std::fabs(n) <= 2.0 * std::fabs(a)) lo = std::fmin(lo, 1.0 - n * n / a);
    if (!(lo >= need)) return false;
  }
  return true;
}

bool ShadingTables::build_materials(hipStream_t st, const std::vector<glz_material>& materials, Error& err) {
  h_materials.clear();
  for (const glz_material& m : materials) {
    RTMaterial r{};
    for (int i = 0; i < 3; ++i) {
      r.diffuse_mul[i] = (float)m.diffuse_mul[i] / 255.0f;
      r.emissive_col[i] = m.has_emissive ? (float)m.emissive_col[i] / 255.0f : 0.0f;
    }
    r.diffuse_mul[3] = r.emissive_col[3] = 1.0f;
    metal_spectra(m.metal < GLZ_METAL_COUNT ? m.metal : 0, r.metal_ior.w, r.metal_fresnel.w);
    r.diffuse = m.diffuse;
    r.roughness = m.roughness;
    r.metalness = m.metalness;
    r.opacity = m.opacity;
    r.normal = m.normal;
    r.bsdf_index = sbt_callable_index(m.mtype);
    r.roughness_mul = m.roughness_mul;
    r.metalness_mul = m.metalness_mul;
    r.anisotropy = m.anisotropy;
    r.ior_dielectric = m.ior;
    r.is_specular = (m.mtype == GLZ_MAT_MIRROR || m.mtype == GLZ_MAT_GLASS) ? 1u : 0u;
    r.is_emissive = m.has_emissive ? 1u : 0u;
    h_materials.push_back(r);
  }
  return upload_materials(st, err);
}

bool ShadingTables::debug_set_spectra(hipStream_t st, uint32_t material, const float* ior, const float* ior2abs2, Error& err) {
  if (material >= h_materials.size()) return err.fail(GLZ_E_ARG, "no such material");
  memcpy(h_materials[material].metal_ior.w, ior, 64);
  memcpy(h_materials[material].metal_fresnel.w, ior2abs2, 64);
  return upload_materials(st, err);
}

bool ShadingTables::upload_materials(hipStream_t st, Error& err) {
  h_mat_compact.clear();
  h_metal_spectra.clear();
  std::vector<uint32_t> finite;
  for (const RTMaterial& r : h_materials) {
    MetalSpectra sp;
    sp.ior = r.metal_ior;
    sp.fresnel = r.metal_fresnel;
    size_t slot = 0;
    while (slot < h_metal_spectra.size() && memcmp(&h_metal_spectra[slot], &sp, sizeof(sp)) != 0) ++slot;
    if (slot == h_metal_spectra.size()) {
      h_metal_spectra.push_back(sp);
      finite.push_back(conductor_finite(sp.ior.w, sp.fresnel.w) ? kSpectraConductorFinite : 0u);
    }
    h_mat_compact.push_back(compact_material(r, (uint32_t)slot | finite[slot]));
  }
  DeviceBuffer<RTMaterial> materials_new;
  DeviceBuffer<MetalSpectra> spectra_new;
  DeviceBuffer<MatCompact> compact_new;
  if (!hip_ok(materials_new.upload(h_materials.data(), h_materials.size(), st), "upload materials", err)) return false;
  if (!hip_ok(spectra_new.upload(h_metal_spectra.data(), h_metal_spectra.size(), st), "upload metal spectra", err)) return false;
  if (!hip_ok(compact_new.upload(h_mat_compact.data(), h_mat_compact.size(), st), "upload compact materials", err)) return false;
  if (!hip_ok(hipStreamSynchronize(st), "materials upload", err)) return false;
  d_materials_ = std::move(materials_new);
  d_metal_spectra_ = std::move(spectra_new);
  d_mat_compact_ = std::move(compact_new);
  return true;
}

void sky_row_pairs(const float* marginal_values, const float* conditional_integrals, size_t n, float* pairs_out) {
  for (size_t y = 0; y < n; ++y) {
    pairs_out[2 * y] = marginal_values[y];
    pairs_out[2 * y + 1] = conditional_integrals[y];
  }
}

bool ShadingTables::has_non_opaque() const {
  for (const RTMaterial& m : h_materials)
    if (m.opacity != 0u) return true;
  return false;
}

bool ShadingTables::build_lights_and_sky(hipStream_t st, const SceneData& data, size_t n_instances, Error& err) {
  std::vector<glz_light> ordered;
  const glz_light* sky = nullptr;
  for (const glz_light& l : data.lights) {
    if (l.ltype > GLZ_LIGHT_SKY) return err.fail(GLZ_E_INVALID_DATA, "Invalid enum value for LightType");
    if (l.ltype == GLZ_LIGHT_SKY) { if (!sky) sky = &l; }
    else ordered.push_back(l);
  }
  const bool has_sky = sky != nullptr;
  if (sky) ordered.push_back(*sky);
  lights_no = (uint32_t)ordered.size();
  h_lights.clear();
  for (const glz_light& l : ordered) {
    RTLight r{};
    memcpy(r.color.w, l.color, 64);
    float dx = l.direction[0], dy = l.direction[1], dz = l.direction[2];
    if (dx == 0.0f && dy == 0.0f && dz == 0.0f) dy = -1.0f;
    r.pos[0] = l.position[0]; r.pos[1] = l.position[1]; r.pos[2] = l.position[2];
    r.dir[0] = dx; r.dir[1] = dy; r.dir[2] = dz;
    r.shader = l.ltype;
    r.instance_id = 0xFFFFFFFFu;
    r.intensity = l.intensity;
    r.delta = (l.ltype == GLZ_LIGHT_OMNI || l.ltype == GLZ_LIGHT_SUN) ? 1u : 0u;
    if (l.ltype == GLZ_LIGHT_AREA) {
      const uint16_t material_id = (uint16_t)l.resource_id;
      std::vector<uint32_t> ids;
      for (size_t i = 0; i < data.instances.size(); ++i) {
        const glz_mesh* found = mesh_by_id(data, data.instances[i].mesh_id);
        if (found && found->material == material_id) ids.push_back((uint32_t)(uint16_t)i);
      }
      if (ids.empty()) ids.push_back(0);
      for (uint32_t id : ids) {
        if (id >= n_instances) return err.fail(GLZ_E_INVALID_DATA, "area light refers to a missing instance");
        r.instance_id = id;
        h_lights.push_back(r);
      }
    } else {
      h_lights.push_back(r);
    }
  }
  if (h_lights.empty()) {
    RTLight r{};
    r.instance_id = 0xFFFFFFFFu;
    r.intensity = 1.0f;
    r.delta = 1u;
    h_lights.push_back(r);
  }
  if (!hip_ok(d_lights_.upload(h_lights.data(), h_lights.size(), st), "upload lights", err)) return false;

  glz_light dflt{};
  dflt.intensity = 1.0f;
  const glz_light& sl = has_sky ? ordered.back() : dflt;
  if (sl.resource_id >= data.textures.size()) return err.fail(GLZ_E_INVALID_DATA, "sky light references a missing texture");
  float rot32[16];
  host::sky_rotation(sl.yaw_deg, sl.pitch_deg, sl.roll_deg).to_f32(rot32);
  host::Mat4d inv;
  if (!host::invert(host::Mat4d::from_f32(rot32), inv)) inv = host::Mat4d::identity();
  memcpy(h_sky.obj2world, rot32, 64);
  inv.to_f32(h_sky.world2obj);
  h_sky.tex_id = sl.resource_id;
  h_sky.intensity = sl.intensity;
  if (sky_distribution_tex_ != h_sky.tex_id) {
    const TextureData& map = data.textures[h_sky.tex_id];
    const uint32_t W = map.info.width, H = map.info.height;
    const size_t bpp = map.info.format == GLZ_TEX_GRAY ? 1 : 4;
    std::vector<float> values((size_t)W * H);
    const float pi = 3.14159265358979323846f;
    for (uint32_t y = 0; y < H; ++y) {
      const float sint = sinf(pi * ((float)y + 0.5f) / (float)H);
      const uint8_t* row = map.level0.data() + (size_t)y * W * bpp;
      for (uint32_t x = 0; x < W; ++x) {
        const uint8_t* p = row + x * bpp;
        const float r = (float)p[0] / 255.0f, g = (float)p[bpp > 1 ? 1 : 0] / 255.0f, b = (float)p[bpp > 1 ? 2 : 0] / 255.0f;
        values[(size_t)y * W + x] = host::illuminant_luminance(r, g, b) * sint;
      }
    }
    std::vector<float> cond_cdf, integrals(H), marginal_cdf;
    cond_cdf.reserve((size_t)(W + 1) * H);
    for (uint32_t y = 0; y < H; ++y) integrals[y] = host::distribution1d(values.data() + (size_t)y * W, W, cond_cdf);
    h_sky_header.marginal_integral = host::distribution1d(integrals.data(), H, marginal_cdf);
    h_sky_header.marginal_cdf_count = H + 1;
    h_sky_header.conditional_integral_offset = H + (H + 1);
    h_sky_header.conditional_cdf_count = W + 1;
    h_sky_marginal = marginal_cdf;
    h_sky_marginal.insert(h_sky_marginal.end(), integrals.begin(), integrals.end());
    h_sky_marginal.insert(h_sky_marginal.end(), integrals.begin(), integrals.end());
    h_sky_header.cond_cdf00 = cond_cdf.empty() ? 0.0f : cond_cdf[0];
    h_sky_header.cond_value00 = values.empty() ? 0.0f : values[0];
    h_sky_rows.resize(2 * (size_t)H);
    sky_row_pairs(h_sky_marginal.data() + h_sky_header.marginal_cdf_count, h_sky_marginal.data() + h_sky_header.conditional_integral_offset, H, h_sky_rows.data());
    if (!hip_ok(d_sky_rows_.upload(reinterpret_cast<const float2*>(h_sky_rows.data()), H, st), "upload sky rows", err)) return false;
    if (!hip_ok(d_sky_marginal_.upload(h_sky_marginal.data(), h_sky_marginal.size(), st), "upload sky marginal", err)) return false;
    if (!hip_ok(d_sky_cond_values_.upload(values.data(), values.size(), st), "upload sky values", err)) return false;
    if (!hip_ok(d_sky_cond_cdf_.upload(cond_cdf.data(), cond_cdf.size(), st), "upload sky cdf", err)) return false;
    if (!hip_ok(hipStreamSynchronize(st), "sky upload", err)) return false;
    sky_w_ = W;
    sky_h_ = H;
    sky_distribution_tex_ = h_sky.tex_id;
  }
  return hip_ok(hipStreamSynchronize(st), "lights upload", err);
}

void ShadingTables::describe(DeviceScene& dev) const {
  dev.materials = d_materials_.ptr;
  dev.mat_compact = d_mat_compact_.ptr;
  dev.metal_spectra = d_metal_spectra_.ptr;
  dev.n_metal_spectra = (uint32_t)d_metal_spectra_.count;
  dev.n_materials = (uint32_t)d_materials_.count;
  dev.has_non_opaque = has_non_opaque() ? 1u : 0u;
  dev.lights = d_lights_.ptr;
  dev.n_rt_lights = (uint32_t)d_lights_.count;
  dev.sky = h_sky;
  dev.sky_header = h_sky_header;
  dev.sky_marginal = d_sky_marginal_.ptr;
  dev.sky_cdf = d_sky_marginal_.ptr;
  dev.sky_rows = d_sky_rows_.ptr;
  dev.sky_cond_values = d_sky_cond_values_.ptr;
  dev.sky_cond_cdf = d_sky_cond_cdf_.ptr;
  dev.sky_w = sky_w_;
  dev.sky_h = sky_h_;
}

}
```

### glaze_amd/csrc/shading_tables.h

```cpp
#pragma once
#include <vector>

#include "hip_util.h"
#include "kernels.h"
#include "parser.h"

namespace glz {

void sky_row_pairs(const float* marginal_values, const float* conditional_integrals, size_t n, float* pairs_out);

bool conductor_finite(const float* ior, const float* ior2abs2);
bool metal_spectra(uint32_t metal, float* ior_out, float* ior2abs2_out);

class ShadingTables {
 public:
  bool build_materials(hipStream_t st, const std::vector<glz_material>& materials, Error& err);
  bool debug_set_spectra(hipStream_t st, uint32_t material, const float* ior, const float* ior2abs2, Error& err);
  bool build_lights_and_sky(hipStream_t st, const SceneData& data, size_t n_instances, Error& err);
  void forget_sky_distribution() { sky_distribution_tex_ = 0xFFFFFFFFu; }
  bool has_non_opaque() const;
  const RTMaterial* materials() const { return d_materials_.ptr; }
  void describe(DeviceScene& dev) const;

  std::vector<RTMaterial> h_materials;
  std::vector<MatCompact> h_mat_compact;
  std::vector<MetalSpectra> h_metal_spectra;
  std::vector<RTLight> h_lights;
  std::vector<float> h_sky_marginal;
  std::vector<float> h_sky_rows;
  SkyHeader h_sky_header{};
  RTSky h_sky{};
  uint32_t lights_no = 0;

 private:
  bool upload_materials(hipStream_t st, Error& err);
  DeviceBuffer<RTMaterial> d_materials_;
  DeviceBuffer<MatCompact> d_mat_compact_;
  DeviceBuffer<MetalSpectra> d_metal_spectra_;
  DeviceBuffer<RTLight> d_lights_;
  DeviceBuffer<float> d_sky_marginal_, d_sky_cond_values_, d_sky_cond_cdf_;
  DeviceBuffer<float2> d_sky_rows_;
  uint32_t sky_distribution_tex_ = 0xFFFFFFFFu;
  uint32_t sky_w_ = 0, sky_h_ = 0;
};

}
```

### glaze_amd/csrc/textures.cpp

```cpp
#include "textures.h"

#include <algorithm>
#include <cstring>
#include <thread>

#include "mipchain.h"

namespace glz {

struct Tiling {
  uint32_t tw, th, bpp, tiles_x, tiles_y;
  Tiling(uint32_t format, uint32_t w, uint32_t h) {
    const bool gray = format == GLZ_TEX_GRAY;
    tw = gray ? 16u : 8u, th = gray ? 8u : 4u, bpp = gray ? 1u : 4u;
    tiles_x = (w + tw - 1) / tw, tiles_y = (h + th - 1) / th;
  }
  size_t bytes() const { return (size_t)tiles_x * tiles_y * 128u; }
};
static TexDesc append_tiled(std::vector<uint8_t>& pool, uint32_t format, uint32_t w, uint32_t h, const uint8_t* px) {
  const Tiling t(format, w, h);
  pool.resize((pool.size() + 127) & ~size_t(127));
  const size_t base = pool.size();
  pool.resize(base + t.bytes(), 0);
  for (uint32_t y = 0; y < h; ++y)
    for (uint32_t x = 0; x < w; ++x) {
      const size_t dst = base + ((size_t)(y / t.th) * t.tiles_x + x / t.tw) * 128u + ((size_t)(y % t.th) * t.tw + x % t.tw) * t.bpp;
      memcpy(&pool[dst], &px[((size_t)y * w + x) * t.bpp], t.bpp);
    }
  return TexDesc{(uint32_t)base, w, h, format | (t.tiles_x << 8)};
}

bool Textures::copy_of(const glz_texture* textures, uint32_t n, std::vector<TextureData>& out, Error& err) {
  if (n == 0 || !textures) return err.fail(GLZ_E_ARG, "the texture list must keep at least the default texture");
  std::vector<TextureData> fresh(n);
  for (uint32_t i = 0; i < n; ++i) {
    const glz_texture& t = textures[i];
    const size_t bytes = (size_t)t.width * t.height * (t.format == GLZ_TEX_GRAY ? 1 : 4);
    if (!t.pixels || !bytes || t.format < 1 || t.format > 3) return err.fail(GLZ_E_INVALID_DATA, "texture has inconsistent dimensions");
    fresh[i].info = t;
    fresh[i].level0.assign(t.pixels, t.pixels + bytes);
  }
  out.swap(fresh);
  for (auto& t : out) t.info.pixels = t.level0.data();
  return true;
}

bool Textures::upload(hipStream_t st, const std::vector<TextureData>& textures, Error& err) {
  std::vector<TexDesc> desc(textures.size());
  std::vector<uint8_t> pool;
  for (size_t i = 0; i < textures.size(); ++i) {
    const TextureData& t = textures[i];
    const size_t bytes = (size_t)t.info.width * t.info.height * (t.info.format == GLZ_TEX_GRAY ? 1 : 4);
    if (t.level0.size() < bytes || t.info.width == 0 || t.info.height == 0 || t.info.format < 1 || t.info.format > 3)
      return err.fail(GLZ_E_INVALID_DATA, "texture has inconsistent dimensions");
    const Tiling tiling(t.info.format, t.info.width, t.info.height);
    if (pool.size() + tiling.bytes() > 0xFFFFFFFFull || tiling.tiles_x >= (1u << 24)) return err.fail(GLZ_E_UNSUPPORTED, "texture pool larger than 4 GiB");
    if (t.info.width == 1 && t.info.height == 1) {
      uint32_t bits = 0;
      memcpy(&bits, t.level0.data(), tiling.bpp);
      desc[i] = TexDesc{bits, 1u, 1u, t.info.format | 0x80u | (1u << 8)};
      continue;
    }
    desc[i] = append_tiled(pool, t.info.format, t.info.width, t.info.height, t.level0.data());
  }
  mips_ready_ = false;
  h_mips_.clear();
  if (!hip_ok(d_desc_.upload(desc.data(), desc.size(), st), "upload texture descriptors", err)) return false;
  if (!hip_ok(d_pool_.upload(pool.data(), pool.size(), st), "upload texture pool", err)) return false;
  return hip_ok(hipStreamSynchronize(st), "texture upload", err);
}

bool Textures::ensure_mips(hipStream_t st, std::vector<TextureData>& textures, Error& err) {
  if (mips_ready_) return true;
  const size_t nt = textures.size();
  h_mips_.assign(nt, {});
  std::vector<std::vector<host::MipLevel>> chains(nt);
  std::vector<std::string> decode_errs(nt);
  auto build_one = [&](size_t i) {
    TextureData& t = textures[i];
    if (!t.decode_more_levels(decode_errs[i])) return;
    std::vector<host::MipLevel> given(1);
    given[0].width = t.info.width;
    given[0].height = t.info.height;
    given[0].pixels = t.level0;
    for (size_t l = 0; l < t.more_levels.size(); ++l) {
      host::MipLevel m;
      m.width = t.more_dims[2 * l];
      m.height = t.more_dims[2 * l + 1];
      m.pixels = t.more_levels[l];
      given.push_back(std::move(m));
    }
    chains[i] = host::build_mip_chain(t.info.format, std::move(given));
  };
  const unsigned workers = (unsigned)std::min<size_t>(nt, std::max(1u, std::min(16u, std::thread::hardware_concurrency())));
  if (workers <= 1) {
    for (size_t i = 0; i < nt; ++i) build_one(i);
  } else {
    std::vector<std::thread> pool;
    std::vector<std::string> failed(workers);
    for (unsigned w = 0; w < workers; ++w)
      pool.emplace_back([&, w] {
        try {
          for (size_t i = w; i < nt; i += workers) build_one(i);
        } catch (const std::exception& ex) {
          failed[w] = ex.what();
        }
      });
    for (auto& th : pool) th.join();
    for (auto& f : failed)
      if (!f.empty()) return err.fail(GLZ_E_IO, "mip chain: " + f);
  }
  for (size_t i = 0; i < nt; ++i)
    if (!decode_errs[i].empty()) return err.fail(GLZ_E_INVALID_DATA, "Corrupted image: " + decode_errs[i]);
  std::vector<uint8_t> pool;
  std::vector<TexDesc> desc;
  std::vector<uint32_t> base(nt, 0);
  for (size_t i = 0; i < nt; ++i) {
    const uint32_t levels = (uint32_t)chains[i].size();
    base[i] = (uint32_t)desc.size() | (levels << 24);
    for (uint32_t l = 1; l < levels; ++l) {
      const host::MipLevel& m = chains[i][l];
      desc.push_back(append_tiled(pool, textures[i].info.format, m.width, m.height, m.pixels.data()));
      h_mips_[i].push_back(m.pixels);
    }
    if (pool.size() > 0xFFFFFFF0ull || desc.size() >= (1u << 24)) return err.fail(GLZ_E_UNSUPPORTED, "mip pool larger than 4 GiB");
  }
  if (!hip_ok(d_mip_desc_.upload(desc.data(), desc.size(), st), "upload mip descriptors", err)) return false;
  if (!hip_ok(d_mip_pool_.upload(pool.data(), pool.size(), st), "upload mip pool", err)) return false;
  if (!hip_ok(d_mip_base_.upload(base.data(), base.size(), st), "upload mip table", err)) return false;
  if (!hip_ok(hipStreamSynchronize(st), "mip upload", err)) return false;
  mips_ready_ = true;
  return true;
}

const std::vector<uint8_t>* Textures::mip_level(uint32_t texture, uint32_t level) const {
  if (!mips_ready_ || texture >= h_mips_.size() || level == 0 || level - 1 >= h_mips_[texture].size()) return nullptr;
  return &h_mips_[texture][level - 1];
}

// ... 12 lines not shown
```

### include/glaze_abi.h

```cpp
#ifndef GLAZE_ABI_H
#define GLAZE_ABI_H

#include <stddef.h>
#include <stdint.h>

#ifdef __cplusplus
extern "C" {
#endif

#define GLZ_OK 0
#define GLZ_E_IO (-1)
#define GLZ_E_INVALID_INPUT (-2)
#define GLZ_E_INVALID_DATA (-3)
#define GLZ_E_ARG (-4)
#define GLZ_E_DEVICE (-5)
#define GLZ_E_UNSUPPORTED (-6)


typedef struct glz_vertex {
  float vv[3];
  float vn[3];
  float vt[2];
} glz_vertex;

// ... 331 lines not shown
int glz_renderer_scatter_packed_all(glz_renderer*, uint32_t world, const void* dev_packed_rgba32f, uint64_t stride_pixels, void* dev_frame_rgba32f);
int glz_renderer_set_chains(glz_renderer*, uint32_t n);
#define GLZ_LAUNCH_AUTO 0
#define GLZ_LAUNCH_TWO_KERNELS 1
#define GLZ_LAUNCH_PATH 2
int glz_renderer_set_launch_mode(glz_renderer*, int mode);
int glz_renderer_launch_mode(glz_renderer*);
int glz_renderer_set_node_width(glz_renderer*, int width);
int glz_renderer_node_width(glz_renderer*);
int glz_renderer_set_devices(glz_renderer*, const int* hip_devices, int n);
int glz_renderer_device_count(glz_renderer*);
int glz_renderer_device_scene_info(glz_renderer*, int i, glz_scene_info* out);
int glz_rccl_version(void);
int glz_renderer_tonemap_device(glz_renderer*, const void* dev_result_rgba32f, uint8_t* rgba8_out);

typedef struct glz_render_stats {
  uint64_t launches;
  uint64_t samples;
  double   render_ms;
  double   trace_closest_ms, shade_ms, trace_shadow_ms, other_ms;
  uint64_t closest_rays, shadow_rays;
  uint64_t closest_nodes, closest_tris, shadow_nodes, shadow_tris, hits;
  uint64_t fresh_paths;
  uint64_t phase[12];
  uint64_t tex_fetches, tex_bytes, alpha_tex_bytes, light_samples, sky_samples;
} glz_render_stats;
int glz_renderer_enable_counters(glz_renderer*, int flags);
int glz_renderer_get_stats(glz_renderer*, glz_render_stats* out);

int glz_debug_trace_closest(glz_scene*, const float* origins3, const float* dirs3, uint64_t n, float tmin,
                            float* t_out, uint32_t* tri_out, uint32_t* inst_out, float* u_out, float* v_out);
int glz_debug_trace_any(glz_scene*, const float* origins3, const float* dirs3, const float* tmax, uint64_t n,
                        float tmin, uint8_t* hit_out);
int64_t glz_debug_read_derivatives(glz_scene*, float* out12, int64_t cap_triangles);
int64_t glz_debug_read_rt_materials(glz_scene*, void* out, int64_t cap_bytes);
int64_t glz_debug_read_rt_lights(glz_scene*, void* out, int64_t cap_bytes);
int64_t glz_debug_read_sky(glz_scene*, float* out, int64_t cap_floats);
int64_t glz_debug_read_bvh(glz_scene*, void* nodes_out, int64_t cap_nodes, void* tris_out, int64_t cap_tris);
int64_t glz_debug_read_bvh8(glz_scene*, void* nodes_out, int64_t cap_nodes);
int64_t glz_debug_read_leaf_records(glz_scene*, void* out, int64_t cap_records);

int64_t glz_debug_read_tlas_instances(glz_scene*, void* out, int64_t cap_bytes);
int64_t glz_debug_instance_boxes(glz_scene*, int on_device, uint64_t budget, float* lo4, float* hi4);
float glz_debug_box_kernel_ms(glz_scene*);
int64_t glz_debug_read_texture_level(glz_scene*, uint32_t texture, uint32_t level, uint8_t* out, int64_t cap, uint32_t* width, uint32_t* height);
int glz_debug_project_points(glz_instance*, const glz_camera* camera, uint32_t width, uint32_t height, const float* points3, uint64_t n, float* out3);
int glz_debug_reproject(glz_instance*, uint32_t w, uint32_t h, const float* motion, const float* prev_color, const float* prev_aov0, const float* prev_aov1,
                        const glz_reproject_params* params_or_null, float* out, float* kernel_ms_out);
int glz_debug_motion_timing(glz_renderer*, const glz_camera* prev_camera, const glz_transform* prev_transforms, uint32_t n_prev_transforms, float* kernel_ms_out);
int glz_debug_motion_timing_from(glz_renderer*, const glz_previous_state*, float* kernel_ms_out);
int glz_debug_skin_timing(glz_renderer*, const glz_pose* pose, uint32_t reps, float* kernel_ms_out);
int glz_debug_morph_timing(glz_renderer*, const glz_animation* one, uint32_t reps, float* kernel_ms_out, uint64_t* bytes_out);
int glz_debug_normals_timing(glz_renderer*, int id, uint32_t reps, float ms_out[2], uint64_t bytes_out[2]);
int glz_debug_tonemap(glz_instance*, const float* rgba32f, uint64_t n_pixels, uint8_t* rgba8_out);
int glz_debug_sample_texture(glz_scene*, uint32_t texture, const float* uv2, const float* footprint4_or_null, uint64_t n, float* rgba_out);
int glz_debug_detmath(glz_instance*, int fn, const float* x, const float* y, float* out, uint64_t n);
int glz_debug_color_to_spec(glz_instance*, int illuminant, const float* rgb3, uint64_t n, float* out16);
int glz_debug_bsdf_value(glz_scene*, uint32_t material_id, const float* wo3, const float* wi3, const float* uv2, const float* rand1,
                         const float* frame9_or_null, uint64_t n, float* value16_out, float* pdf_out);
int glz_debug_bsdf_sample(glz_scene*, uint32_t material_id, const float* wo3, const float* uv2, const float* rand3, const float* frame9_or_null,
                          uint64_t n, float* wi3_out, float* value16_out, float* pdf_out);
int glz_debug_light_sample(glz_scene*, uint32_t light_index, const float* pos3, const float* rand3, uint64_t n, float scene_radius,
                           float* wi3_out, float* dist_out, float* pdf_out, float* emission16_out);
int glz_debug_scene_set_spectra(glz_scene*, uint32_t material_id, const float ior[16], const float ior2abs2[16]);

int glz_debug_denoise(glz_instance*, uint32_t w, uint32_t h, const float* result, const float* aov0, const float* aov1,
                      const glz_denoise_params*, float* out);
int glz_debug_despeckle(glz_instance*, uint32_t w, uint32_t h, const float* result, const float* aov0, const float* aov1,
                        const glz_despeckle_params*, const glz_denoise_params*, int with_filter, float* out, float* kernel_ms_out);
#define GLZ_POST_TIMING_SLOTS (3 + GLZ_DENOISE_MAX_ITERATIONS)
int glz_debug_post_timing(glz_renderer*, float ms_out[GLZ_POST_TIMING_SLOTS]);
int glz_debug_camera_rays(glz_renderer*, float off_x, float off_y, float* origins3, float* dirs3);

int glz_debug_guide_chain(glz_renderer*, uint32_t segment, float* origins3, float* dirs3, uint8_t* alive);

int glz_debug_rccl_selftest(glz_instance*, uint64_t n_floats, int* version_out);

int glz_host_launch_constants(uint64_t seed, uint32_t launch, uint32_t* seed_out, float offset[2]);
int glz_host_push_constants(const glz_camera* camera, uint32_t width, uint32_t height, float out32[32]);
int glz_host_tile_owner(uint32_t width, uint32_t height, uint32_t world, uint16_t* owner_out);
int glz_host_chain_owner(uint32_t width, uint32_t height, uint32_t rank, uint32_t world, uint32_t chains, uint16_t* owner_out);
int glz_host_srgb8_thresholds(float thresholds_out[256]);
int glz_host_sky_row_pairs(const float* marginal_values, const float* conditional_integrals, uint64_t n, float* pairs_out);
int glz_host_conductor_finite(const float ior[16], const float ior2abs2[16], int* flag_out);
int glz_host_metal_spectra(uint32_t metal, float ior_out[16], float ior2abs2_out[16]);
int glz_host_traversal_offsets_fit(uint64_t n_nodes, uint64_t n_nodes8, uint64_t n_leaves, uint64_t n_instances, uint64_t grid_lanes,
                                   uint64_t overflow_depth);
int64_t glz_host_mip_level(const glz_texture* texture, uint32_t level, uint8_t* out, int64_t cap, uint32_t* width, uint32_t* height);
int glz_host_build_sah(uint32_t n, const float* box_lo, const float* box_hi, int32_t* children_out, int32_t* parent_out);
int glz_host_denoise(uint32_t w, uint32_t h, const float* result, const float* aov0, const float* aov1,
                     const glz_denoise_params*, float* out);
int glz_host_despeckle(uint32_t w, uint32_t h, const float* result, const float* aov0, const float* aov1,
                       const glz_despeckle_params*, const glz_denoise_params*, int with_filter, float* out);
int glz_host_project_constants(const glz_camera* camera, uint32_t width, uint32_t height, float out32[32]);
int glz_host_project_points(const glz_camera* camera, uint32_t width, uint32_t height, const float* points3, uint64_t n, float* out3);
int glz_host_reproject(uint32_t w, uint32_t h, const float* motion, const float* prev_color, const float* prev_aov0, const float* prev_aov1,
                       const glz_reproject_params* params_or_null, float* out);
int64_t glz_host_instance_boxes(const glz_scene_desc* desc, uint64_t budget, float* lo4, float* hi4);
int glz_host_skin(const glz_vertex* bind, const uint16_t* joints, const float* weights, uint64_t n, const glz_transform* bones, uint32_t n_bones,
                  glz_vertex* out);
int glz_host_morph(const glz_vertex* base, uint64_t n, const glz_morph_target* targets, uint32_t n_targets, const float* weights, glz_vertex* out);
int glz_host_vertex_normals(const glz_vertex* vertices, uint64_t n_vertices, const uint32_t* indices, uint64_t n_indices, const glz_mesh* meshes, uint64_t n_meshes,
                            uint32_t first_vertex, uint32_t n, const uint32_t* groups_or_null, glz_vertex* out);
int glz_host_weld_groups(const glz_vertex* vertices, uint64_t n, uint32_t* groups_out);

#ifdef __cplusplus
}
#endif
#endif
```

Before: 3213 Msamples/s.

## Bracket sky CDF search, shortcut pow2 texel wrap, reuse Lambert eval in shading

```diff
diff --git a/glaze_amd/abi.py b/glaze_amd/abi.py
--- a/glaze_amd/abi.py
+++ b/glaze_amd/abi.py
@@ -333,6 +333,9 @@
     "glz_debug_guide_chain": (C.c_int, [_P, C.c_uint32, _P, _P, _P]),
     "glz_host_traversal_offsets_fit": (C.c_int, [C.c_uint64] * 6),
     "glz_host_sky_row_pairs": (C.c_int, [_P, _P, C.c_uint64, _P]),
+    "glz_host_sky_bracket_table": (C.c_int, [_P, C.c_uint64, _P]),
+    "glz_host_sky_cdf_search": (C.c_int, [_P, C.c_uint64, _P, _P, C.c_uint64, _P, _P]),
+    "glz_host_texel_wrap": (C.c_int, [_P, C.c_uint64, C.c_int32, _P]),
     "glz_host_conductor_finite": (C.c_int, [_P, _P, _P]),
     "glz_host_metal_spectra": (C.c_int, [C.c_uint32, _P, _P]),
 }
diff --git a/glaze_amd/csrc/abi_debug.cpp b/glaze_amd/csrc/abi_debug.cpp
--- a/glaze_amd/csrc/abi_debug.cpp
+++ b/glaze_amd/csrc/abi_debug.cpp
@@ -709,6 +709,29 @@
   sky_row_pairs(marginal_values, conditional_integrals, (size_t)n, pairs_out);
   return GLZ_OK;
 }
+int glz_host_sky_bracket_table(const float* cdf, uint64_t size, uint16_t* table_out) {
+  if (!table_out || (size != 0 && !cdf) || size > 0xFFFFFFFFull) return fail(GLZ_E_ARG, "glz_host_sky_bracket_table: null array, or a cdf of 2^32 entries");
+  sky_bracket_table(cdf, (uint32_t)size, table_out);
+  return GLZ_OK;
+}
+int glz_host_sky_cdf_search(const float* cdf, uint64_t size, const uint16_t* bracket_or_null, const float* xi, uint64_t n, float* sample_out, uint32_t* offset_out) {
+  if (size < 2 || size > 0x7FFFFFFFull || !cdf) return fail(GLZ_E_ARG, "glz_host_sky_cdf_search: a cdf has two entries at least");
+  if (n != 0 && (!xi || !sample_out || !offset_out)) return fail(GLZ_E_ARG, "glz_host_sky_cdf_search: null array");
+  if (bracket_or_null && bracket_or_null[0] != kSkyBracketFallback)
+    for (uint32_t b = 0; b <= kSkyBracketBuckets; ++b)
+      if (bracket_or_null[b] > size || (b != 0 && bracket_or_null[b] < bracket_or_null[b - 1])) return fail(GLZ_E_ARG, "glz_host_sky_cdf_search: the bracket table does not fit the cdf");
+  for (uint64_t i = 0; i < n; ++i) sample_out[i] = sky_cdf_search(cdf, (uint32_t)size, xi[i], bracket_or_null, &offset_out[i]);
+  return GLZ_OK;
+}
+int glz_host_texel_wrap(const int32_t* i, uint64_t count, int32_t n, int32_t* index_out) {
+  if (n <= 0 || (count != 0 && (!i || !index_out))) return fail(GLZ_E_ARG, "glz_host_texel_wrap: a size below 1, or a null array");
+  const bool pow2 = (n & (n - 1)) == 0;
+  for (uint64_t k = 0; k < count; ++k) {
+    const int32_t r = i[k] % n;
+    index_out[k] = pow2 ? (i[k] & (n - 1)) : (r < 0 ? r + n : r);
+  }
+  return GLZ_OK;
+}
 int glz_host_conductor_finite(const float ior[16], const float ior2abs2[16], int* flag_out) {
   if (!ior || !ior2abs2 || !flag_out) return fail(GLZ_E_ARG, "glz_host_conductor_finite: null argument");
   *flag_out = conductor_finite(ior, ior2abs2) ? 1 : 0;
diff --git a/glaze_amd/csrc/device/hit_vertex.h b/glaze_amd/csrc/device/hit_vertex.h
--- a/glaze_amd/csrc/device/hit_vertex.h
+++ b/glaze_amd/csrc/device/hit_vertex.h
@@ -51,10 +51,10 @@
   v.xf_bits = ids.xf;
   return v;
 }
-template <bool POINTS>
+template <bool POINTS, bool SHORT = true>
 __device__ __forceinline__ void finish_hit_vertex(const DeviceScene& S, HitVertex& v, const TexFootprint& fp) {
   if (v.mat.normal != 0) {
-    const vec4 tx = texture2d_lod(S, v.mat.normal, v.uv.x, v.uv.y, fp);
+    const vec4 tx = texture2d_lod<SHORT>(S, v.mat.normal, v.uv.x, v.uv.y, fp);
     Frame old;
     old.s = normalize3(v.dpdu);
     old.n = v.ns;
@@ -75,13 +75,14 @@
     v.ns = xform_tdir(w2o, v.ns);
   }
 }
+template <bool SHORT = true>
 __device__ __forceinline__ SurfacePoint hit_surface_point(const DeviceScene& S, const HitVertex& v, vec3 direction, const TexFootprint& fp) {
   SurfacePoint P;
   P.woW = -direction;
   P.uv = v.uv;
   P.frame = make_frame(v.dpdu, v.ns);
   P.mat = v.mat;
-  fetch_material_textures(S, P, fp);
+  fetch_material_textures<SHORT>(S, P, fp);
   return P;
 }
 }
diff --git a/glaze_amd/csrc/device/intersect.h b/glaze_amd/csrc/device/intersect.h
--- a/glaze_amd/csrc/device/intersect.h
+++ b/glaze_amd/csrc/device/intersect.h
@@ -129,7 +129,7 @@
   const float4 r0 = rec[0], r1 = rec[1], r2 = rec[2];
   const float tu = (r0.x * w + r0.z * u) + r1.x * v, tv = (r0.y * w + r0.w * u) + r1.y * v;
   const TexDesc t{__float_as_uint(r1.z), __float_as_uint(r1.w), __float_as_uint(r2.x), __float_as_uint(r2.y)};
-  return !(bilinear_level(S, t, S.tex_pool, tu, tv).x < 0.5f);
+  return !(bilinear_level<false>(S, t, S.tex_pool, tu, tv).x < 0.5f);
 }
 
 __device__ __forceinline__ bool alpha_test_instance(const DeviceScene& S, uint32_t slot, uint32_t instance, float u, float v) {
@@ -138,7 +138,7 @@
   const uint32_t material_id = S.instances[instance].material_id;
   const float w = 1.0f - u - v;
   const float tu = (a.z * w + b.z * u) + c.z * v, tv = (a.w * w + b.w * u) + c.w * v;
-  return !(texture_r(S, S.materials[material_id].opacity, vec2{tu, tv}) < 0.5f);
+  return !(texture_r<false>(S, S.materials[material_id].opacity, vec2{tu, tv}) < 0.5f);
 }
 
 struct HitRecord {
diff --git a/glaze_amd/csrc/device/shade_pixel.h b/glaze_amd/csrc/device/shade_pixel.h
--- a/glaze_amd/csrc/device/shade_pixel.h
+++ b/glaze_amd/csrc/device/shade_pixel.h
@@ -29,7 +29,11 @@
 struct DirectState {
   const LaunchArgs& A;
   static constexpr bool kDeferSkyTexel = false;
+  static constexpr bool kHandLambert = false;
   __device__ __forceinline__ void stamp(int) {}
+  __device__ __forceinline__ const uint16_t* sky_bracket(const DeviceScene& S) const {
+    return reinterpret_cast<const uint16_t*>(S.sky_marginal + sky_bracket_offset(S.sky_header.marginal_cdf_count));
+  }
   __device__ __forceinline__ void ray_o(uint32_t lid, float4 v) { A.st.ray_o[lid] = v; }
   __device__ __forceinline__ void ray_d(uint32_t lid, float4 v) { A.st.ray_d[lid] = v; }
   __device__ __forceinline__ void imp(int q, uint32_t lid, float4 v) { A.st.imp[q][lid] = v; }
@@ -51,6 +55,9 @@
   __device__ __forceinline__ void stamp(int) {}
 #endif
   static constexpr bool kDeferSkyTexel = true;
+  static constexpr bool kHandLambert = true;
+  const uint16_t* lds_sky_bracket = nullptr;
+  __device__ __forceinline__ const uint16_t* sky_bracket(const DeviceScene&) const { return lds_sky_bracket; }
   float4 ro, rd, im[4];
   uint32_t mask = 0;
   __device__ __forceinline__ void ray_o(uint32_t, float4 v) { ro = v; mask |= 1u; }
@@ -162,15 +169,15 @@
   const SurfacePoint P = hit_surface_point(S, hv, direction, fp);
   GLZ_SHADE_STAMP(1);
   float spec_flag;
-  float imp_lum = 0.0f;
-  bool have_lum = false;
+  Spec lambert_value = spec_set(0.0f);
+  bool have_lambert = false;
   if (mat.is_specular == 0) {
     const uint32_t li = out.pick_light(F, rng);
     vec3 xi;
     xi.x = rand01(rng); xi.y = rand01(rng); xi.z = rand01(rng);
     LightSample ls;
     ls.pdf = 0.0f;
-    sample_light<State::kDeferSkyTexel>(S, li, point, xi, F.scene_radius, ls);
+    sample_light<State::kDeferSkyTexel>(S, li, point, xi, F.scene_radius, ls, out.sky_bracket(S));
     GLZ_SHADE_STAMP(2);
     vec3 c = mk3(0.0f, 0.0f, 0.0f);
     uint32_t flags = kFlagUpdate;
@@ -180,13 +187,15 @@
       const float xi_b = rand01(rng);
       Spec value = spec_set(0.0f);
       const float bpdf = bsdf_eval(S, P, ls.wiW, xi_b, value);
+      if (State::kHandLambert && mat.bsdf_index == kBsdfLambert) {
+        lambert_value = value;
+        have_lambert = true;
+      }
       if (bpdf > 0.0f) {
         const float w_vis = 1.0f * (fabsf(dot3(ls.wiW, ns)) / ls.pdf);
         const float nl = (float)F.lights_no;
         const Spec emission = light_emission<State::kDeferSkyTexel>(S, ls);
         const Spec importance = load_importance();
-        imp_lum = spec_luminance(importance);
-        have_lum = true;
         Spec rad;
         GLZ_BINS {
           const float rl = value.w[i] * emission.w[i];
@@ -199,11 +208,6 @@
         sh_tmax = ls.distance - 1e-3f;
       }
     }
-    if (!(flags & kFlagShadow)) {
-      const Spec importance = load_importance();
-      imp_lum = spec_luminance(importance);
-      have_lum = true;
-    }
     const bool push = (flags & kFlagShadow) != 0;
     GLZ_SHADE_STAMP(3);
     const uint32_t slot = queue.slot(push);
@@ -222,7 +226,7 @@
   GLZ_SHADE_STAMP(4);
   float rr_scale = 1.0f;
   if (bounce > (float)(F.pt_steps / 2u)) {
-    const float kill = gl_max(0.05f, 1.0f - (have_lum ? imp_lum : spec_luminance(load_importance())));
+    const float kill = gl_max(0.05f, 1.0f - spec_luminance(load_importance()));
     if (rand01(rng) < kill) {
       end_w = spec_flag;
       return 2;
@@ -233,7 +237,7 @@
   xi.x = rand01(rng); xi.y = rand01(rng); xi.z = rand01(rng);
   Spec value = spec_set(0.0f);
   vec3 wiW = mk3(0.0f, 0.0f, 0.0f);
-  const float pdf = bsdf_sample(S, P, xi, value, wiW);
+  const float pdf = bsdf_sample(S, P, xi, value, wiW, &lambert_value, State::kHandLambert && have_lambert);
   if (pdf == 0.0f) {
     end_w = spec_flag;
     return 2;
diff --git a/glaze_amd/csrc/device/shading.h b/glaze_amd/csrc/device/shading.h
--- a/glaze_amd/csrc/device/shading.h
+++ b/glaze_amd/csrc/device/shading.h
@@ -78,13 +78,20 @@
   if (format == GLZ_TEX_RGBA_SRGB) return vec4{S.srgb_lut[r], S.srgb_lut[g], S.srgb_lut[b], (float)a / 255.0f};
   return vec4{(float)r / 255.0f, (float)g / 255.0f, (float)b / 255.0f, (float)a / 255.0f};
 }
+template <bool SHORT = true>
 GLZ_D uint32_t texel_address(const TexDesc& t, uint32_t format, uint32_t ux, uint32_t uy) {
   const uint32_t tiles_x = t.format >> 8;
-  if (format == GLZ_TEX_GRAY) return t.offset + ((uy >> 3) * tiles_x + (ux >> 4)) * 128u + (uy & 7u) * 16u + (ux & 15u);
-  return t.offset + (((uy >> 2) * tiles_x + (ux >> 3)) * 32u + (uy & 3u) * 8u + (ux & 7u)) * 4u;
-}
+  if constexpr (SHORT) {
+    if (format == GLZ_TEX_GRAY) return t.offset + ((uint32_t)__umul24(uy >> 3, tiles_x) + (ux >> 4)) * 128u + (uy & 7u) * 16u + (ux & 15u);
+    return t.offset + (((uint32_t)__umul24(uy >> 2, tiles_x) + (ux >> 3)) * 32u + (uy & 3u) * 8u + (ux & 7u)) * 4u;
+  } else {
+    if (format == GLZ_TEX_GRAY) return t.offset + ((uy >> 3) * tiles_x + (ux >> 4)) * 128u + (uy & 7u) * 16u + (ux & 15u);
+    return t.offset + (((uy >> 2) * tiles_x + (ux >> 3)) * 32u + (uy & 3u) * 8u + (ux & 7u)) * 4u;
+  }
+}
+template <bool SHORT = true>
 GLZ_D uint32_t load_texel(const uint8_t* __restrict__ pool, const TexDesc& t, uint32_t format, uint32_t ux, uint32_t uy) {
-  const uint32_t addr = texel_address(t, format, ux, uy);
+  const uint32_t addr = texel_address<SHORT>(t, format, ux, uy);
   return format == GLZ_TEX_GRAY ? (uint32_t)pool[addr] : *reinterpret_cast<const uint32_t*>(pool + addr);
 }
 GLZ_D int wrap_coord(int i, int n) {
@@ -104,6 +111,7 @@
   return (int)((bits >> 31) && r != 0u ? (uint32_t)n - r : r);
 }
 GLZ_D float lerp_ab(float a, float b, float t) { return a + (b - a) * t; }
+template <bool SHORT = true>
 GLZ_D vec4 bilinear_level(const DeviceScene& S, const TexDesc& t, const uint8_t* __restrict__ pool, float u, float v) {
   const uint32_t format = t.format & 0x7Fu;
   float fu = u * (float)t.width - 0.5f, fv = v * (float)t.height - 0.5f;
@@ -117,18 +125,24 @@
       S.tex_counter[0] += 1ull;
       S.tex_counter[1] += format == GLZ_TEX_GRAY ? 4ull : 16ull;
     }
-    const int x0 = fabsf(iu) < 8388608.0f ? wrap_coord((int)iu, (int)t.width) : wrap_coord_far(iu, (int)t.width);
-    const int y0 = fabsf(iv) < 8388608.0f ? wrap_coord((int)iv, (int)t.height) : wrap_coord_far(iv, (int)t.height);
+    int x0, y0;
+    if (SHORT && (((t.width & (t.width - 1u)) | (t.height & (t.height - 1u))) == 0u) && fabsf(iu) < 8388608.0f && fabsf(iv) < 8388608.0f) {
+      x0 = (int)iu & (int)(t.width - 1u);
+      y0 = (int)iv & (int)(t.height - 1u);
+    } else {
+      x0 = fabsf(iu) < 8388608.0f ? wrap_coord((int)iu, (int)t.width) : wrap_coord_far(iu, (int)t.width);
+      y0 = fabsf(iv) < 8388608.0f ? wrap_coord((int)iv, (int)t.height) : wrap_coord_far(iv, (int)t.height);
+    }
     const int x1 = x0 + 1 == (int)t.width ? 0 : x0 + 1, y1 = y0 + 1 == (int)t.height ? 0 : y0 + 1;
     if (format != GLZ_TEX_GRAY && x1 == x0 + 1 && (x0 & 7) != 7) {
-      const uint2 r0 = *reinterpret_cast<const uint2*>(pool + texel_address(t, format, (uint32_t)x0, (uint32_t)y0));
-      const uint2 r1 = *reinterpret_cast<const uint2*>(pool + texel_address(t, format, (uint32_t)x0, (uint32_t)y1));
+      const uint2 r0 = *reinterpret_cast<const uint2*>(pool + texel_address<SHORT>(t, format, (uint32_t)x0, (uint32_t)y0));
+      const uint2 r1 = *reinterpret_cast<const uint2*>(pool + texel_address<SHORT>(t, format, (uint32_t)x0, (uint32_t)y1));
       ta = r0.x; tb = r0.y; tc = r1.x; tdx = r1.y;
     } else {
-      ta = load_texel(pool, t, format, (uint32_t)x0, (uint32_t)y0);
-      tb = load_texel(pool, t, format, (uint32_t)x1, (uint32_t)y0);
-      tc = load_texel(pool, t, format, (uint32_t)x0, (uint32_t)y1);
-      tdx = load_texel(pool, t, format, (uint32_t)x1, (uint32_t)y1);
+      ta = load_texel<SHORT>(pool, t, format, (uint32_t)x0, (uint32_t)y0);
+      tb = load_texel<SHORT>(pool, t, format, (uint32_t)x1, (uint32_t)y0);
+      tc = load_texel<SHORT>(pool, t, format, (uint32_t)x0, (uint32_t)y1);
+      tdx = load_texel<SHORT>(pool, t, format, (uint32_t)x1, (uint32_t)y1);
     }
   }
   const vec4 a = decode_texel(S, format, ta), b = decode_texel(S, format, tb), c = decode_texel(S, format, tc), d = decode_texel(S, format, tdx);
@@ -139,12 +153,14 @@
   r.w = lerp_ab(lerp_ab(a.w, b.w, ax), lerp_ab(c.w, d.w, ax), ay);
   return r;
 }
+template <bool SHORT = true>
 GLZ_D vec4 texture2d(const DeviceScene& S, uint32_t id, float u, float v) {
   const uint4 td = reinterpret_cast<const uint4*>(S.tex_desc)[id];
-  return bilinear_level(S, TexDesc{td.x, td.y, td.z, td.w}, S.tex_pool, u, v);
+  return bilinear_level<SHORT>(S, TexDesc{td.x, td.y, td.z, td.w}, S.tex_pool, u, v);
 }
 constexpr float kNoLod = -1e30f;
 struct TexFootprint { float lod_base; float du, dv; uint32_t taps; };
+template <bool SHORT = true>
 GLZ_D vec4 texture2d_lod(const DeviceScene& S, uint32_t id, float u, float v, const TexFootprint& fp) {
   const uint4 td = reinterpret_cast<const uint4*>(S.tex_desc)[id];
   const TexDesc t0{td.x, td.y, td.z, td.w};
@@ -183,7 +199,7 @@
       uu = u + s * fp.du;
       vv = v + s * fp.dv;
     }
-    const vec4 r = bilinear_level(S, t, pool, uu, vv);
+    const vec4 r = bilinear_level<SHORT>(S, t, pool, uu, vv);
     if (upper == 0u) {
       cur = r;
     } else {
@@ -207,7 +223,8 @@
   vec4 t = texture2d(S, id, uv.x, uv.y);
   return mk3(t.x, t.y, t.z);
 }
-GLZ_D float texture_r(const DeviceScene& S, uint32_t id, vec2 uv) { return texture2d(S, id, uv.x, uv.y).x; }
+template <bool SHORT = true>
+GLZ_D float texture_r(const DeviceScene& S, uint32_t id, vec2 uv) { return texture2d<SHORT>(S, id, uv.x, uv.y).x; }
 
 struct Frame {
   vec3 s, t, n;
@@ -386,16 +403,17 @@
   return kInvPi * (A + B * maxcos * sinalpha * tanbeta);
 }
 
+template <bool SHORT = true>
 GLZ_D void fetch_material_textures(const DeviceScene& S, SurfacePoint& P, const TexFootprint& fp) {
   const uint32_t kind = P.mat.bsdf_index;
   P.tint = mk3(0.0f, 0.0f, 0.0f);
   P.rough_tex = P.metal_tex = 0.0f;
   if (kind == kBsdfLambert || kind == kBsdfUber) {
-    const vec4 tx = texture2d_lod(S, P.mat.diffuse, P.uv.x, P.uv.y, fp);
+    const vec4 tx = texture2d_lod<SHORT>(S, P.mat.diffuse, P.uv.x, P.uv.y, fp);
     P.tint = mk3(tx.x, tx.y, tx.z) * mk3(P.mat.diffuse_mul[0], P.mat.diffuse_mul[1], P.mat.diffuse_mul[2]);
   }
-  if (kind == kBsdfMetal || kind == kBsdfFrosted || kind == kBsdfUber) P.rough_tex = texture2d_lod(S, P.mat.roughness, P.uv.x, P.uv.y, fp).x;
-  if (kind == kBsdfUber) P.metal_tex = texture2d_lod(S, P.mat.metalness, P.uv.x, P.uv.y, fp).x;
+  if (kind == kBsdfMetal || kind == kBsdfFrosted || kind == kBsdfUber) P.rough_tex = texture2d_lod<SHORT>(S, P.mat.roughness, P.uv.x, P.uv.y, fp).x;
+  if (kind == kBsdfUber) P.metal_tex = texture2d_lod<SHORT>(S, P.mat.metalness, P.uv.x, P.uv.y, fp).x;
 }
 GLZ_D vec3 diffuse_tint(const DeviceScene&, const SurfacePoint& P) { return P.tint; }
 
@@ -484,14 +502,15 @@
   return wi;
 }
 
-GLZ_D float bsdf_sample(const DeviceScene& S, const SurfacePoint& P, vec3 xi, Spec& value, vec3& wiW) {
+GLZ_D float bsdf_sample(const DeviceScene& S, const SurfacePoint& P, vec3 xi, Spec& value, vec3& wiW, const Spec* lambert_value = nullptr, bool have_lambert = false) {
   const MatScalars& m = P.mat;
   const uint32_t kind = m.bsdf_index;
   const vec3 wo = to_local(P.woW, P.frame);
   if (kind == kBsdfLambert) {
     vec3 wi = cosine_hemisphere(xi.x, xi.y, wo.z);
     wiW = normalize3(to_world(wi, P.frame));
-    value = from_surface_color(diffuse_tint(S, P) * kInvPi);
+    if (have_lambert) value = *lambert_value;
+    else value = from_surface_color(diffuse_tint(S, P) * kInvPi);
     return fabsf(wi.z) * kInvPi;
   }
   if (kind == kBsdfMirror) {
@@ -606,8 +625,16 @@
 }
 
 template <class Fetch>
-GLZ_D float sample_cdf(float xi, int size, Fetch fetch, uint32_t& offset_out) {
+GLZ_D float sample_cdf(float xi, int size, Fetch fetch, uint32_t& offset_out, const uint16_t* bracket = nullptr) {
   int first = 0, len = size;
+  if (bracket != nullptr && xi >= 0.0f && xi < 1.0f) {
+    const int b = (int)(xi * (float)kSkyBracketBuckets);
+    const int lo = (int)bracket[b], hi = (int)bracket[b + 1];
+    if (lo != (int)kSkyBracketFallback) {
+      first = lo;
+      len = hi - lo;
+    }
+  }
   while (len > 0) {
     int half = len >> 1, middle = first + half;
     if (fetch(middle) <= xi) {
@@ -627,7 +654,7 @@
 }
 
 template <bool DEFER_SKY_TEXEL = true>
-GLZ_D void sample_light(const DeviceScene& S, uint32_t light_index, vec3 p, vec3 xi, float scene_radius, LightSample& out) {
+GLZ_D void sample_light(const DeviceScene& S, uint32_t light_index, vec3 p, vec3 xi, float scene_radius, LightSample& out, const uint16_t* sky_bracket = nullptr) {
   const RTLight* L = &S.lights[light_index];
   const uint32_t kind = L->shader;
   if (S.tex_counter) {
@@ -676,7 +703,7 @@
   }
   uint32_t row;
   const float* cdf = S.sky_cdf;
-  float v = sample_cdf(xi.y, (int)S.sky_header.marginal_cdf_count, [&](int i) { return cdf[i]; }, row);
+  float v = sample_cdf(xi.y, (int)S.sky_header.marginal_cdf_count, [&](int i) { return cdf[i]; }, row, sky_bracket);
   const float2 of_row = S.sky_rows[row];
   float v_pdf = of_row.x / S.sky_header.marginal_integral;
   const float cdf00 = S.sky_header.cond_cdf00;
diff --git a/glaze_amd/csrc/device/types.h b/glaze_amd/csrc/device/types.h
--- a/glaze_amd/csrc/device/types.h
+++ b/glaze_amd/csrc/device/types.h
@@ -193,6 +193,16 @@
   float cond_cdf00;
   float cond_value00;
 };
+
+constexpr uint32_t kSkyLdsFloats = 1088;
+constexpr uint32_t kSkyBracketBuckets = 256;
+constexpr uint32_t kSkyBracketFallback = 0xFFFFu;
+constexpr uint32_t kSkyBracketFloats = ((kSkyBracketBuckets + 1u) * 2u + 15u) / 16u * 4u;
+inline
+#ifdef __HIPCC__
+__host__ __device__
+#endif
+uint32_t sky_bracket_offset(uint32_t marginal_cdf_count) { return marginal_cdf_count == 0u ? 0u : (3u * (marginal_cdf_count - 1u) + 1u + 3u) / 4u * 4u; }
 
 struct DeviceScene {
   const float4* vertices;
diff --git a/glaze_amd/csrc/kernels_debug.hip b/glaze_amd/csrc/kernels_debug.hip
--- a/glaze_amd/csrc/kernels_debug.hip
+++ b/glaze_amd/csrc/kernels_debug.hip
@@ -139,9 +139,21 @@
   wi3[3 * t] = wi.x; wi3[3 * t + 1] = wi.y; wi3[3 * t + 2] = wi.z;
   GLZ_BINS value16[16 * t + i] = value.w[i];
 }
+template <bool SKY_LDS>
 __global__ void __launch_bounds__(kBlock) k_debug_light_sample(DeviceScene S, uint32_t light, const float* __restrict__ pos3, const float* __restrict__ rand3,
                                                                uint32_t n, float scene_radius, float* __restrict__ wi3, float* __restrict__ dist,
                                                                float* __restrict__ pdf, float* __restrict__ emission16) {
+  __shared__ uint4 s_sky[SKY_LDS ? kSkyLdsFloats / 4 + kSkyBracketFloats / 4 : 1];
+  const uint16_t* bracket = nullptr;
+  if (SKY_LDS) {
+    static_assert(kSkyBracketFloats / 4 <= kBlock, "the bracket table is copied one piece per thread");
+    const uint32_t n_sky = S.sky_header.marginal_cdf_count;
+    for (uint32_t i = threadIdx.x; i < (n_sky + 3u) / 4u; i += kBlock) s_sky[i] = reinterpret_cast<const uint4*>(S.sky_marginal)[i];
+    if (threadIdx.x < kSkyBracketFloats / 4) s_sky[kSkyLdsFloats / 4 + threadIdx.x] = reinterpret_cast<const uint4*>(S.sky_marginal)[sky_bracket_offset(n_sky) / 4u + threadIdx.x];
+    __syncthreads();
+    S.sky_cdf = reinterpret_cast<const float*>(s_sky);
+    bracket = reinterpret_cast<const uint16_t*>(s_sky + kSkyLdsFloats / 4);
+  }
   const uint32_t t = blockIdx.x * kBlock + threadIdx.x;
   if (t >= n) return;
   S.tex_counter = nullptr;
@@ -149,7 +161,7 @@
   ls.wiW = mk3(0.0f, 0.0f, 0.0f);
   ls.pdf = 0.0f;
   ls.distance = 0.0f;
-  sample_light(S, light, mk3(pos3[3 * t], pos3[3 * t + 1], pos3[3 * t + 2]), mk3(rand3[3 * t], rand3[3 * t + 1], rand3[3 * t + 2]), scene_radius, ls);
+  sample_light(S, light, mk3(pos3[3 * t], pos3[3 * t + 1], pos3[3 * t + 2]), mk3(rand3[3 * t], rand3[3 * t + 1], rand3[3 * t + 2]), scene_radius, ls, bracket);
   const Spec e = light_emission(S, ls);
   wi3[3 * t] = ls.wiW.x; wi3[3 * t + 1] = ls.wiW.y; wi3[3 * t + 2] = ls.wiW.z;
   dist[t] = ls.distance;
@@ -190,6 +202,8 @@
 }
 hipError_t launch_debug_light_sample(hipStream_t st, const DeviceScene& scene, uint32_t light, const float* pos3, const float* rand3, uint32_t n,
                                      float scene_radius, float* wi3, float* dist, float* pdf, float* emission16) {
-  return launch_per_item(st, k_debug_light_sample, n, scene, light, pos3, rand3, n, scene_radius, wi3, dist, pdf, emission16);
-}
-}
+  const bool sky_lds = scene.sky_marginal != nullptr && scene.sky_header.marginal_cdf_count > 1u && scene.sky_header.marginal_cdf_count <= kSkyLdsFloats;
+  return sky_lds ? launch_per_item(st, k_debug_light_sample<true>, n, scene, light, pos3, rand3, n, scene_radius, wi3, dist, pdf, emission16)
+                 : launch_per_item(st, k_debug_light_sample<false>, n, scene, light, pos3, rand3, n, scene_radius, wi3, dist, pdf, emission16);
+}
+}
diff --git a/glaze_amd/csrc/kernels_post.hip b/glaze_amd/csrc/kernels_post.hip
--- a/glaze_amd/csrc/kernels_post.hip
+++ b/glaze_amd/csrc/kernels_post.hip
@@ -58,7 +58,7 @@
 __device__ __forceinline__ GuideVertex guide_vertex(const DeviceScene& S, float4 hr, uint32_t hit_inst, vec3 direction) {
   const TexFootprint fp{kNoLod, 0.0f, 0.0f, 1u};
   HitVertex hv = load_hit_vertex(S, hr, [&]() { return hit_inst; });
-  finish_hit_vertex<CHAIN>(S, hv, fp);
+  finish_hit_vertex<CHAIN, false>(S, hv, fp);
   const MatScalars& mat = hv.mat;
   GuideVertex v;
   v.n = normalize3(hv.ns);
@@ -66,14 +66,14 @@
   if (!(post::finite1(v.n.x) && post::finite1(v.n.y) && post::finite1(v.n.z))) v.n = mk3(0.0f, 0.0f, 0.0f);
   v.albedo = mk3(1.0f, 1.0f, 1.0f);
   if (mat.bsdf_index == kBsdfLambert || mat.bsdf_index == kBsdfUber) {
-    const vec4 tx = texture2d_lod(S, mat.diffuse, hv.uv.x, hv.uv.y, fp);
+    const vec4 tx = texture2d_lod<false>(S, mat.diffuse, hv.uv.x, hv.uv.y, fp);
     v.albedo = mk3(tx.x, tx.y, tx.z) * mk3(mat.diffuse_mul[0], mat.diffuse_mul[1], mat.diffuse_mul[2]);
   }
   v.go_on = false;
   v.point = hv.point;
   v.wiW = mk3(0.0f, 0.0f, 0.0f);
   if (CHAIN && mat.is_specular != 0) {
-    const SurfacePoint P = hit_surface_point(S, hv, direction, fp);
+    const SurfacePoint P = hit_surface_point<false>(S, hv, direction, fp);
     Spec value = spec_set(0.0f);
     const float pdf = bsdf_sample(S, P, mk3(0.0f, 0.0f, 0x1.fffffep-1f), value, v.wiW);
     v.go_on = pdf != 0.0f && post::finite1(v.wiW.x) && post::finite1(v.wiW.y) && post::finite1(v.wiW.z);
diff --git a/glaze_amd/csrc/kernels_render.hip b/glaze_amd/csrc/kernels_render.hip
--- a/glaze_amd/csrc/kernels_render.hip
+++ b/glaze_amd/csrc/kernels_render.hip
@@ -8,7 +8,6 @@
 namespace glz {
 using namespace dev;
 
-constexpr uint32_t kSkyLdsFloats = 1088;
 
 constexpr uint32_t kShadeBlock = 256, kShadeWavesPerBlock = kShadeBlock / 64;
 #ifdef GLZ_SECTION_TIMES
@@ -27,11 +26,13 @@
 #define GLZ_KS(k) do { } while (0)
 #endif
   __shared__ alignas(16) float s_lut[256];
-  __shared__ uint4 s_pool[kShadeBlock * 4 + kSkyLdsFloats / 4 + kShadeLdsTableBytes / 16];
+  __shared__ uint4 s_pool[kShadeBlock * 4 + kSkyLdsFloats / 4 + kSkyBracketFloats / 4 + kShadeLdsTableBytes / 16];
   uint4* s_imp = s_pool;
   float* s_sky = reinterpret_cast<float*>(s_pool + kShadeBlock * 4);
-  uint4* s_tables = s_pool + kShadeBlock * 4 + kSkyLdsFloats / 4;
-  static_assert(6u * kShadeBlock <= kShadeBlock * 4 + kSkyLdsFloats / 4 + kShadeLdsTableBytes / 16, "the staging area of the path state fits the pool");
+  uint4* s_bracket = s_pool + kShadeBlock * 4 + kSkyLdsFloats / 4;
+  uint4* s_tables = s_bracket + kSkyBracketFloats / 4;
+  static_assert(6u * kShadeBlock <= kShadeBlock * 4 + kSkyLdsFloats / 4 + kSkyBracketFloats / 4 + kShadeLdsTableBytes / 16, "the staging area of the path state fits the pool");
+  static_assert(kSkyBracketFloats / 4 <= kShadeBlock, "the bracket table is copied one piece per thread");
   __shared__ uint32_t s_bin[kShadeWavesPerBlock * 64];
   __shared__ uint16_t s_perm[kShadeBlock];
   __shared__ float4 s_hit[kShadeBlock];
@@ -40,8 +41,10 @@
   static_assert(kShadeBlock == 256, "pixel_of_block");
   const uint32_t n_sky = A.scene.sky_header.marginal_cdf_count;
   if (threadIdx.x < 64u) reinterpret_cast<float4*>(s_lut)[threadIdx.x] = reinterpret_cast<const float4*>(A.scene.srgb_lut)[threadIdx.x];
-  if (SKY)
+  if (SKY) {
     for (uint32_t i = threadIdx.x; i < (n_sky + 3u) / 4u; i += kShadeBlock) s_pool[kShadeBlock * 4 + i] = reinterpret_cast<const uint4*>(A.scene.sky_marginal)[i];
+    if (threadIdx.x < kSkyBracketFloats / 4) s_bracket[threadIdx.x] = reinterpret_cast<const uint4*>(A.scene.sky_marginal)[sky_bracket_offset(n_sky) / 4u + threadIdx.x];
+  }
   s_bin[threadIdx.x] = 0;
   const SceneTables tables(A.scene);
   if (TABLES) tables.stage(A.scene, s_tables, kShadeBlock);
@@ -139,6 +142,7 @@
     SharedQueue queue{A2};
     staged.A = &A2;
     staged.lds_imp = (LdsNodePtr)(reinterpret_cast<u32x4*>(s_imp) + s_perm[threadIdx.x]);
+    staged.lds_sky_bracket = SKY ? reinterpret_cast<const uint16_t*>(s_bracket) : nullptr;
     staged.lds_pick = (StagedState::LdsPickPtr)(reinterpret_cast<StagedState::u32x2*>(s_pick) + s_perm[threadIdx.x]);
 #ifdef GLZ_SECTION_TIMES
     staged.sec_last = __builtin_amdgcn_s_memtime();
diff --git a/glaze_amd/csrc/shading_tables.cpp b/glaze_amd/csrc/shading_tables.cpp
--- a/glaze_amd/csrc/shading_tables.cpp
+++ b/glaze_amd/csrc/shading_tables.cpp
@@ -114,6 +114,59 @@
   for (size_t y = 0; y < n; ++y) {
     pairs_out[2 * y] = marginal_values[y];
     pairs_out[2 * y + 1] = conditional_integrals[y];
+  }
+}
+
+float sky_cdf_search(const float* cdf, uint32_t size_u, float xi, const uint16_t* bracket, uint32_t* offset_out) {
+  const int size = (int)size_u;
+  int first = 0, len = size;
+  if (bracket != nullptr && xi >= 0.0f && xi < 1.0f) {
+    const int b = (int)(xi * (float)kSkyBracketBuckets);
+    const int lo = (int)bracket[b], hi = (int)bracket[b + 1];
+    if (lo != (int)kSkyBracketFallback) {
+      first = lo;
+      len = hi - lo;
+    }
+  }
+  while (len > 0) {
+    const int half = len >> 1, middle = first + half;
+    if (cdf[middle] <= xi) {
+      first = middle + 1;
+      len -= half + 1;
+    } else {
+      len = half;
+    }
+  }
+  int off = first - 1;
+  off = off < 0 ? 0 : (off > size - 2 ? size - 2 : off);
+  const float cur = cdf[off], next = cdf[off + 1];
+  float du = xi - cur;
+  if (next - cur > 0.0f) du /= next - cur;
+  *offset_out = (uint32_t)off;
+  return ((float)off + du) / (float)size;
+}
+
+void sky_bracket_table(const float* cdf, uint32_t size, uint16_t* table_out) {
+  bool monotone = size < kSkyBracketFallback;
+  for (uint32_t i = 0; monotone && i + 1 < size; ++i) monotone = cdf[i + 1] >= cdf[i];
+  if (monotone && size != 0u) monotone = cdf[0] == cdf[0];
+  for (uint32_t b = 0; b <= kSkyBracketBuckets; ++b) {
+    if (!monotone) {
+      table_out[b] = (uint16_t)kSkyBracketFallback;
+      continue;
+    }
+    const float xi = (float)b / (float)kSkyBracketBuckets;
+    int first = 0, len = (int)size;
+    while (len > 0) {
+      const int half = len >> 1, middle = first + half;
+      if (cdf[middle] <= xi) {
+        first = middle + 1;
+        len -= half + 1;
+      } else {
+        len = half;
+      }
+    }
+    table_out[b] = (uint16_t)first;
   }
 }
 
@@ -214,7 +267,12 @@
     h_sky_rows.resize(2 * (size_t)H);
     sky_row_pairs(h_sky_marginal.data() + h_sky_header.marginal_cdf_count, h_sky_marginal.data() + h_sky_header.conditional_integral_offset, H, h_sky_rows.data());
     if (!hip_ok(d_sky_rows_.upload(reinterpret_cast<const float2*>(h_sky_rows.data()), H, st), "upload sky rows", err)) return false;
-    if (!hip_ok(d_sky_marginal_.upload(h_sky_marginal.data(), h_sky_marginal.size(), st), "upload sky marginal", err)) return false;
+    h_sky_bracket.assign(kSkyBracketFloats * 2u, 0);
+    sky_bracket_table(h_sky_marginal.data(), h_sky_header.marginal_cdf_count, h_sky_bracket.data());
+    std::vector<float> with_bracket(sky_bracket_offset(h_sky_header.marginal_cdf_count) + kSkyBracketFloats, 0.0f);
+    memcpy(with_bracket.data(), h_sky_marginal.data(), h_sky_marginal.size() * sizeof(float));
+    memcpy(with_bracket.data() + sky_bracket_offset(h_sky_header.marginal_cdf_count), h_sky_bracket.data(), h_sky_bracket.size() * sizeof(uint16_t));
+    if (!hip_ok(d_sky_marginal_.upload(with_bracket.data(), with_bracket.size(), st), "upload sky marginal", err)) return false;
     if (!hip_ok(d_sky_cond_values_.upload(values.data(), values.size(), st), "upload sky values", err)) return false;
     if (!hip_ok(d_sky_cond_cdf_.upload(cond_cdf.data(), cond_cdf.size(), st), "upload sky cdf", err)) return false;
     if (!hip_ok(hipStreamSynchronize(st), "sky upload", err)) return false;
diff --git a/glaze_amd/csrc/shading_tables.h b/glaze_amd/csrc/shading_tables.h
--- a/glaze_amd/csrc/shading_tables.h
+++ b/glaze_amd/csrc/shading_tables.h
@@ -8,6 +8,9 @@
 namespace glz {
 
 void sky_row_pairs(const float* marginal_values, const float* conditional_integrals, size_t n, float* pairs_out);
+
+float sky_cdf_search(const float* cdf, uint32_t size, float xi, const uint16_t* bracket, uint32_t* offset_out);
+void sky_bracket_table(const float* cdf, uint32_t size, uint16_t* table_out);
 
 bool conductor_finite(const float* ior, const float* ior2abs2);
 bool metal_spectra(uint32_t metal, float* ior_out, float* ior2abs2_out);
@@ -28,6 +31,7 @@
   std::vector<RTLight> h_lights;
   std::vector<float> h_sky_marginal;
   std::vector<float> h_sky_rows;
+  std::vector<uint16_t> h_sky_bracket;
   SkyHeader h_sky_header{};
   RTSky h_sky{};
   uint32_t lights_no = 0;
diff --git a/glaze_amd/csrc/textures.cpp b/glaze_amd/csrc/textures.cpp
--- a/glaze_amd/csrc/textures.cpp
+++ b/glaze_amd/csrc/textures.cpp
@@ -55,6 +55,7 @@
       return err.fail(GLZ_E_INVALID_DATA, "texture has inconsistent dimensions");
     const Tiling tiling(t.info.format, t.info.width, t.info.height);
     if (pool.size() + tiling.bytes() > 0xFFFFFFFFull || tiling.tiles_x >= (1u << 24)) return err.fail(GLZ_E_UNSUPPORTED, "texture pool larger than 4 GiB");
+    if (tiling.tiles_y >= (1u << 24)) return err.fail(GLZ_E_UNSUPPORTED, "texture of 2^24 tile rows or more");
     if (t.info.width == 1 && t.info.height == 1) {
       uint32_t bits = 0;
       memcpy(&bits, t.level0.data(), tiling.bpp);
diff --git a/include/glaze_abi.h b/include/glaze_abi.h
--- a/include/glaze_abi.h
+++ b/include/glaze_abi.h
@@ -437,6 +437,9 @@
 int glz_host_chain_owner(uint32_t width, uint32_t height, uint32_t rank, uint32_t world, uint32_t chains, uint16_t* owner_out);
 int glz_host_srgb8_thresholds(float thresholds_out[256]);
 int glz_host_sky_row_pairs(const float* marginal_values, const float* conditional_integrals, uint64_t n, float* pairs_out);
+int glz_host_sky_bracket_table(const float* cdf, uint64_t size, uint16_t* table_out);
+int glz_host_sky_cdf_search(const float* cdf, uint64_t size, const uint16_t* bracket_or_null, const float* xi, uint64_t n, float* sample_out, uint32_t* offset_out);
+int glz_host_texel_wrap(const int32_t* i, uint64_t count, int32_t n, int32_t* index_out);
 int glz_host_conductor_finite(const float ior[16], const float ior2abs2[16], int* flag_out);
 int glz_host_metal_spectra(uint32_t metal, float ior_out[16], float ior2abs2_out[16]);
 int glz_host_traversal_offsets_fit(uint64_t n_nodes, uint64_t n_nodes8, uint64_t n_leaves, uint64_t n_instances, uint64_t grid_lanes,
```

Result: faster. 3254 Msamples/s, median of 6 (+1.3%).
